# NVlabs/EdgeRunner

Hardware: AMD Instinct MI355X
Metric: mesh tokens/sec (whole node), ArAE greedy test_num_face=1000 (higher is better)
Workload: dtype f32; 1 GPU; BASELINE configs[1]: ArAE random-init (seeded synthetic checkpoint), batch 1 per GPU, greedy, test_num_face=1000, 4000 new tokens (EOS suppressed until T), 4096-point synthetic cloud; step = the whole LMM.generate(): encode_cond + 2050-token prefill + 4000-token decode + detokenise to a mesh (native meto engine, clean=True); layers=24, hidden=1536, heads=16, batch_per_gpu=1, precision=fp32, parallelism=dp1 (independent samples, full replica per GPU)

## Files before the change

### edgerunner_amd/csrc/er_api.hip

```cpp
#include "../../include/edgerunner_hip.h"

#include <hip/hip_runtime.h>

#include <algorithm>
#include <cstdarg>
#include <cstdio>
#include <cstdlib>
#include <cstring>
#include <map>
#include <memory>
#include <string>
#include <utility>
#include <vector>

#include "er_common.h"
#include "k_attn_decode.h"
#include "k_outproj_merge.h"
#include "k_flash_attn_f16s.h"
#include "k_gemm.h"
#include "k_gemm_stream.h"
#include "k_gemv.h"
#include "k_gemv_mfma.h"
#include "k_head.h"
#include "k_rowops.h"
#include "k_score.h"
#include "k_flash_attn.h"
#include "k_flash_attn_f32.h"
#include "k_fps.h"
#include "k_fidelity.h"
#include "meto_decode.h"
#include "meto_encode.h"
#include "er_queue_host.h"
#include "er_decode_plan.h"
#include "er_decode_proj.h"

using namespace er;

static thread_local char g_err[1024] = "";

static int fail(int code, const char* fmt, ...) {
    va_list ap;
    va_start(ap, fmt);
    vsnprintf(g_err, sizeof(g_err), fmt, ap);
    va_end(ap);
    return code;
}

#define HIPCHK(expr)                                                                          \
    do {                                                                                      \
        hipError_t e_ = (expr);                                                               \
        if (e_ != hipSuccess)                                                                 \
            return fail(ER_ERR_HIP, "%s:%d %s -> %s", __FILE__, __LINE__, #expr, hipGetErrorString(e_)); \
    } while (0)
#define ERCHK(expr)                 \
    do {                            \
        int r_ = (expr);            \
        if (r_ < 0) return r_;      \
    } while (0)

struct LayerW {
    _Float16 *wqkv_h = nullptr, *wo_h = nullptr, *w1_h = nullptr, *w2_h = nullptr;
    void *wqkv_t = nullptr, *wo_t = nullptr, *w1_t = nullptr, *w2_t = nullptr;
    float *wqkv = nullptr, *bqkv = nullptr;
    float *wo = nullptr, *bo = nullptr, *ln1w = nullptr, *ln1b = nullptr;
    float *w1 = nullptr, *b1 = nullptr, *w2 = nullptr, *b2 = nullptr, *ln2w = nullptr, *ln2b = nullptr;
};

#include "er_devbuf.h"
#include "er_weights.h"

struct PointEnc {
    int PH = 0, heads = 0, Lq = 0, LD = 0, freq = 0;
    int mode = ER_PE_EMBED;
    float eps = 1e-5f;
    float *query = nullptr, *basis = nullptr, *mlp_w = nullptr, *mlp_b = nullptr, *ln_w = nullptr, *ln_b = nullptr;
    float *ca_ln1_w = nullptr, *ca_ln1_b = nullptr, *ca_ln2_w = nullptr, *ca_ln2_b = nullptr;
    float *ca_q_w = nullptr, *ca_q_b = nullptr, *ca_k_w = nullptr, *ca_k_b = nullptr, *ca_v_w = nullptr, *ca_v_b = nullptr,
          *ca_o_w = nullptr, *ca_o_b = nullptr;
    float *ff0_w = nullptr, *ff0_b = nullptr, *ff2_w = nullptr, *ff2_b = nullptr, *lin_w = nullptr, *lin_b = nullptr;
    int kpad = 0;
    DevBuf<float> a0, x, k, v, qln, q, sc, att, l, ln, u, g, lat;
    DevBuf<float> q0, fdist;
    DevBuf<int32_t> fidx;
};

static size_t gen_state_ints(size_t b) { return 7 * b + 8; }
static GenState gen_state_carve(int* sb, size_t b) {
    GenState s{};
    s.tok = sb; s.pos = sb + b; s.counter = sb + 2 * b; s.ngen = sb + 3 * b; s.unfinished = sb + 4 * b;
    s.eos_step = sb + 5 * b; s.base_pos = sb + 6 * b; s.n_unfinished = sb + 7 * b; s.error = sb + 7 * b + 1;
    return s;
}

constexpr int SK_SLICES_OUTPROJ = 4, SK_SLICES_FC2 = 16;
static_assert(1536 / (4 * GM_KW) == SK_SLICES_OUTPROJ && 6144 / (4 * GM_KW) == SK_SLICES_FC2 && 6144 / (GM_WAVES * GM_KW) == SK_SLICES_OUTPROJ, "k_gemv_mfma.h");

struct KvMem {
    DecodePlan plan;
    DevBuf<char> kc, vc;
    DevBuf<float> ypre, hbuf, ypre1, h1buf, qbuf, abuf, fbuf, logits;
    DevBuf<float> part, part_ml;
    DevBuf<float> skpart;
    DevBuf<char> xt_h, xt_att, xt_f;
    DevBuf<int> state_block;
    GenState st{};
    DevBuf<DecodeParamsDev> d_params;
    DevBuf<int> d_ids_tmp;
    DevBuf<unsigned int> d_row_stream;
    DevBuf<int> d_row_budget;
    DevBuf<long long> d_out_ids;
    hipGraphExec_t step_exec = nullptr;
    KvMem() = default;
    KvMem(const KvMem&) = delete;
    KvMem& operator=(const KvMem&) = delete;
    ~KvMem() { if (step_exec) hipGraphExecDestroy(step_exec); }
};

struct er_ctx {
    er_config cfg{};
    int device = 0;
    int D = 0;
    hipStream_t own_stream = nullptr;
    std::vector<LayerW> layers;
    float *embd = nullptr, *posemb = nullptr, *lm_head = nullptr, *embed_num_face = nullptr;
    _Float16* lm_head_h = nullptr;
    bool fast = false;
    float *proj_w = nullptr, *proj_b = nullptr, *normc_w = nullptr, *normc_b = nullptr;
    PointEnc pe;
    WeightTable w;
    std::unique_ptr<KvMem> kv = std::make_unique<KvMem>();
    int kv_esz = 4;
    int* h_pinned = nullptr;
    int base_pos = 0;
    bool have_hidden = false;
    DecodeKnobs knobs;
    bool tiled_valid = false;
    int prof_len = 0;
    hipEvent_t ev0 = nullptr, ev1 = nullptr;
    float last_decode_ms = 0.f;
    DevBuf<_Float16> p_hi, p_lo;
    DevBuf<float> p_h, p_q, p_a, p_y, p_f, p_qkv, p_ap, p_aml, e_tmp;
    DevBuf<int> e_ids;
    DevBuf<float> s_lg;
    erq::QueueHost q;
    DevBuf<int> q_stage, q_look;
    int* q_pinned = nullptr;
};

constexpr int ER_MAX_BATCH = 1023;

template <typename Ctx>
static hipStream_t pick(Ctx* c, void* s) { return s ? (hipStream_t)s : c->own_stream; }

static int env_int(const char* name, int dflt) { const char* v = getenv(name); return (v && v[0]) ? atoi(v) : dflt; }
static bool env_is(const char* name, char ch) { const char* v = getenv(name); return v && v[0] == ch; }

static DecodeKnobs read_knobs(bool fast) {
    DecodeKnobs k;
    k.use_graph = !env_is("ER_NO_GRAPH", '1');
    k.nw_qkv = env_int("ER_NW_QKV", fast ? 9 : 6);
    if (k.nw_qkv != 4 && k.nw_qkv != 9) k.nw_qkv = 6;
    k.nw_fc1 = env_int("ER_NW_FC1", fast ? 12 : 4) == 12 ? 12 : 4;
    k.prefill_attn_f16s = env_int("ER_PREFILL_ATTN_F16S", -1);
    if (k.prefill_attn_f16s != 0 && k.prefill_attn_f16s != 1) k.prefill_attn_f16s = -1;
    k.attn_v_batched = env_int("ER_ATTN_V_BATCHED", 0);
    if (k.attn_v_batched != 1 && k.attn_v_batched != 3) k.attn_v_batched = 0;
    k.decode_v = env_int("ER_DECODE_V", 3) == 2 ? 2 : 3;
    const char* rw = getenv("ER_RW_FC2");
    k.rw_fc2 = rw ? atoi(rw) : 6;
    if (fast && k.rw_fc2 != 2 && k.rw_fc2 != 4 && k.rw_fc2 != 6) fprintf(stderr, "[edgerunner_hip] ER_RW_FC2=%s is not 2 / 4 / 6: using 2 rows per fc2 workgroup\n", rw);
    return k;
}

static ReserveKnobs read_reserve_knobs() { return {env_is("ER_FORCE_BATCHED", '1'), env_is("ER_BATCHED_VALU", '1'), !env_is("ER_XT", '0')}; }

extern "C" int er_abi_version(void) { return ER_ABI_VERSION; }
extern "C" const char* er_last_error(void) { return g_err; }

static const char* kKindNames[ER_NUM_KERNEL_KINDS] = {"qkv_gemv", "attn_decode", "attn_combine", "out_proj_gemv",
                                                      "fc1_gemv", "fc2_gemv", "lm_head_gemv", "sample_head"};
extern "C" const char* er_kernel_kind_name(int k) { return (k >= 0 && k < ER_NUM_KERNEL_KINDS) ? kKindNames[k] : "?"; }

static int pe_attach(WeightTable& t, PointEnc& p, int mode, const char* who, const char* before) {
    if (mode != ER_PE_EMBED && mode != ER_PE_DOWNSAMPLE)
        return fail(ER_ERR_INVALID, "%s: %d is neither ER_PE_EMBED nor ER_PE_DOWNSAMPLE", who, mode);
    for (auto& kv : t.keys)
        if (kv.second.loaded && kv.first.rfind(before, 0) == 0)
            return fail(ER_ERR_INVALID, "%s: call it before any '%s*' tensor is loaded", who, before);
    const size_t PH = p.PH, kin = 2 * p.freq + 3;
    p.mode = mode;
    p.kpad = (int)((kin + 15) / 16 * 16);
    const std::string pe = "point_encoder.";
    if (mode == ER_PE_EMBED) t.add(pe + "query_embed", &p.query, (size_t)p.Lq * PH);
    else t.keys.erase(pe + "query_embed");
    t.add(pe + "point_embed.basis", &p.basis, (size_t)3 * p.freq);
    t.lin(pe + "point_embed.mlp", &p.mlp_w, &p.mlp_b, PH, kin).pad(kin, p.kpad);
    t.lin(pe + "ln", &p.ln_w, &p.ln_b, PH, 1);
    t.lin(pe + "cross_att.ln1", &p.ca_ln1_w, &p.ca_ln1_b, PH, 1);
    t.lin(pe + "cross_att.ln2", &p.ca_ln2_w, &p.ca_ln2_b, PH, 1);
    t.lin(pe + "cross_att.att.q_proj", &p.ca_q_w, &p.ca_q_b, PH, PH);
    t.lin(pe + "cross_att.att.k_proj", &p.ca_k_w, &p.ca_k_b, PH, PH);
    t.lin(pe + "cross_att.att.v_proj", &p.ca_v_w, &p.ca_v_b, PH, PH);
    t.lin(pe + "cross_att.att.out_proj", &p.ca_o_w, &p.ca_o_b, PH, PH);
    t.lin(pe + "cross_att.mlp.net.0", &p.ff0_w, &p.ff0_b, 8 * PH, PH);
    t.lin(pe + "cross_att.mlp.net.2", &p.ff2_w, &p.ff2_b, PH, 4 * PH);
    t.lin(pe + "linear", &p.lin_w, &p.lin_b, p.LD, PH);
    return 0;
}

static void register_weights(er_ctx* c) {
    WeightTable& t = c->w;
    const er_config& g = c->cfg;
    const size_t H = g.hidden_dim, I = g.intermediate_dim, V = g.vocab_size;
    t.fp16 = c->fast;
    if (g.cond_mode == ER_COND_POINT) pe_attach(t, c->pe, ER_PE_EMBED, "er_create", "");
    if (g.cond_mode != ER_COND_NONE) {
        t.lin("proj_cond", &c->proj_w, &c->proj_b, H, g.point_latent_dim);
        t.lin("norm_cond", &c->normc_w, &c->normc_b, H, 1);
    }
    if (g.num_face_buckets > 0) t.add("embed_num_face.weight", &c->embed_num_face, (size_t)g.num_face_buckets * H);
    t.add("mesh_decoder.model.embd.weight", &c->embd, V * H);
    t.add("mesh_decoder.model.embed_positions.weight", &c->posemb, (size_t)g.max_positions * H);
    for (int i = 0; i < g.num_layers; ++i) {
        LayerW& L = c->layers[i];
        const std::string p = "mesh_decoder.model.layers." + std::to_string(i) + ".";
        const char* qkv[3] = {"q_proj", "k_proj", "v_proj"};
        for (size_t j = 0; j < 3; ++j) {
            const std::string q = p + "self_attn." + qkv[j];
            t.add(q + ".weight", &L.wqkv, H * H).slice(3 * H * H, j * H * H).half(&L.wqkv_h);
            t.add(q + ".bias", &L.bqkv, H).slice(3 * H, j * H);
        }
        t.lin(p + "self_attn.out_proj", &L.wo, &L.bo, H, H).half(&L.wo_h);
        t.lin(p + "self_attn_layer_norm", &L.ln1w, &L.ln1b, H, 1);
        t.lin(p + "fc1", &L.w1, &L.b1, I, H).half(&L.w1_h);
        t.lin(p + "fc2", &L.w2, &L.b2, H, I).half(&L.w2_h);
        t.lin(p + "final_layer_norm", &L.ln2w, &L.ln2b, H, 1);
    }
    t.add("mesh_decoder.lm_head.weight", &c->lm_head, V * H).half(&c->lm_head_h);
}

extern "C" int er_create(const er_config* cfg, int device, er_ctx** out) {
    if (!cfg || !out) return fail(ER_ERR_INVALID, "er_create: null argument");
    if (cfg->hidden_dim != 1536 || cfg->intermediate_dim != 6144)
        return fail(ER_ERR_UNSUPPORTED, "this build streams hidden_dim=1536 / intermediate_dim=6144 (ArAE, DiT presets); got %d/%d",
                    cfg->hidden_dim, cfg->intermediate_dim);
    if (cfg->num_heads <= 0 || cfg->hidden_dim % cfg->num_heads) return fail(ER_ERR_INVALID, "hidden_dim %% num_heads != 0");
    const int D = cfg->hidden_dim / cfg->num_heads;
    if (D != 96 && D != 64) return fail(ER_ERR_UNSUPPORTED, "head_dim %d not built (96, 64)", D);
    const bool exact = cfg->weight_dtype == ER_F32 && cfg->kv_dtype == ER_F32;
    const bool fast = cfg->weight_dtype == ER_F16 && cfg->kv_dtype == ER_F16;
    if (!exact && !fast)
        return fail(ER_ERR_UNSUPPORTED, "built modes: fp32 weights + fp32 KV (exact) or fp16 weights + fp16 KV (fast)");
    if (cfg->vocab_size > ER_HEAD_MAX_VOCAB) return fail(ER_ERR_UNSUPPORTED, "vocab_size > %d", ER_HEAD_MAX_VOCAB);
    if (cfg->cond_mode == ER_COND_POINT && (cfg->point_hidden_dim != 1024 || cfg->point_hidden_dim % cfg->point_num_heads))
        return fail(ER_ERR_UNSUPPORTED, "point encoder width %d not built (1024)", cfg->point_hidden_dim);
    HIPCHK(hipSetDevice(device));
    er_ctx* c = new er_ctx();
    c->cfg = *cfg;
    c->device = device;
    c->D = D;
    c->fast = fast;
    c->kv_esz = fast ? 2 : 4;
    c->layers.resize(cfg->num_layers);
    c->pe.PH = cfg->point_hidden_dim; c->pe.heads = cfg->point_num_heads; c->pe.Lq = cfg->point_latent_size;
    c->pe.LD = cfg->point_latent_dim; c->pe.freq = cfg->point_freq_dim; c->pe.eps = cfg->ln_eps;
    c->knobs = read_knobs(fast);
    HIPCHK(hipStreamCreateWithFlags(&c->own_stream, hipStreamDefault));
    HIPCHK(hipEventCreate(&c->ev0));
    HIPCHK(hipEventCreate(&c->ev1));
    HIPCHK(hipHostMalloc((void**)&c->h_pinned, 4096, hipHostMallocDefault));
    register_weights(c);
    *out = c;
    return ER_OK;
}

extern "C" int er_destroy(er_ctx* c) {
    if (!c) return ER_OK;
    hipSetDevice(c->device);
    hipDeviceSynchronize();
    if (c->ev0) hipEventDestroy(c->ev0);
    if (c->ev1) hipEventDestroy(c->ev1);
    if (c->h_pinned) hipHostFree(c->h_pinned);
    if (c->q_pinned) hipHostFree(c->q_pinned);
    if (c->own_stream) hipStreamDestroy(c->own_stream);
    delete c;
    return ER_OK;
}

extern "C" int er_load_tensor(er_ctx* c, const char* key, const void* data, int dtype, int ndim, const int64_t* shape,
                              int on_device) {
    if (!c || !key) return fail(ER_ERR_INVALID, "er_load_tensor: bad argument");
    HIPCHK(hipSetDevice(c->device));
    const int rc = weights_load(c->w, c->own_stream, "er_load_tensor", key, data, dtype, ndim, shape, on_device);
    if (rc != 1) c->tiled_valid = false;
    return rc;
}

extern "C" int er_finalize_weights(er_ctx* c) {
    if (!c) return fail(ER_ERR_INVALID, "null ctx");
    return weights_finalize(c->w);
}

template <typename WT>
static int make_tiled(er_ctx* c, const void* src, void** dst, int N, int K) {
    if (!*dst) {
        char* blk = nullptr;
        ERCHK(c->w.alloc(&blk, tiled_weight_bytes<WT>(N, K)));
        *dst = blk;
    }
    hipLaunchKernelGGL((tile_weights_kernel<WT>), dim3(2048), dim3(ER_WG), 0, c->own_stream, reinterpret_cast<const WT*>(src),
                       reinterpret_cast<f32x4*>(*dst), N, K);
    HIPCHK(hipGetLastError());
    return 0;
}
static int make_tiled_weights(er_ctx* c) {
    if (c->tiled_valid || weights_missing(c->w)) return 0;
    const int H = c->cfg.hidden_dim, I = c->cfg.intermediate_dim;
    for (LayerW& L : c->layers) {
        if (c->fast) {
            ERCHK(make_tiled<_Float16>(c, L.wqkv_h, &L.wqkv_t, 3 * H, H));
            ERCHK(make_tiled<_Float16>(c, L.wo_h, &L.wo_t, H, H));
            ERCHK(make_tiled<_Float16>(c, L.w1_h, &L.w1_t, I, H));
            ERCHK(make_tiled<_Float16>(c, L.w2_h, &L.w2_t, H, I));
        } else {
            ERCHK(make_tiled<float>(c, L.wqkv, &L.wqkv_t, 3 * H, H));
            ERCHK(make_tiled<float>(c, L.wo, &L.wo_t, H, H));
            ERCHK(make_tiled<float>(c, L.w1, &L.w1_t, I, H));
            ERCHK(make_tiled<float>(c, L.w2, &L.w2_t, H, I));
        }
    }
    HIPCHK(hipStreamSynchronize(c->own_stream));
    c->tiled_valid = true;
    return 0;
}

static AttnChunking attn_chunking(int heads, bool fast) {
    return {attn3_num_chunks(heads), attn3_num_chunks(heads) * ATTN3_CAP, attn_chunk(ATTN_STEPS_DEFAULT, fast)};
}

extern "C" int er_plan_decode(int batch, int heads, int head_dim, int hidden, int l_cap, er_decode_plan* out) {
    if (!out || batch <= 0 || heads <= 0 || head_dim <= 0 || l_cap <= 0) return fail(ER_ERR_INVALID, "er_plan_decode: bad argument");
    const DecodeKnobs k = read_knobs(false);
    plan_decode(k.decode_v, k.attn_v_batched, read_reserve_knobs().force_batched, batch, heads, head_dim, hidden, (l_cap + 31) / 32 * 32, attn_chunking(heads, false), out);
    return ER_OK;
}

extern "C" int er_ctx_plan(er_ctx* c, er_decode_plan* out) {
    if (!c || !out) return fail(ER_ERR_INVALID, "er_ctx_plan: null argument");
    if (c->kv->plan.B <= 0) return fail(ER_ERR_INVALID, "er_ctx_plan: no cache reserved (call er_kv_reserve)");
    *out = c->kv->plan.sel;
    return ER_OK;
}

extern "C" int er_plan_gemm_tile(int m, int n, int batch) {
    if (m <= 0 || n <= 0 || batch <= 0) return fail(ER_ERR_INVALID, "er_plan_gemm_tile: bad argument");
    return gemm_pick_tile(m, n, batch);
}

static int kv_alloc(er_ctx* c, KvMem& m, int batch, int Lcap);

extern "C" int er_kv_reserve(er_ctx* c, int batch, int max_len) {
    if (!c || batch <= 0 || max_len <= 0) return fail(ER_ERR_INVALID, "er_kv_reserve: bad argument");
    if (batch > ER_MAX_BATCH) return fail(ER_ERR_UNSUPPORTED, "er_kv_reserve: batch %d > %d (host staging buffers are sized for %d rows)", batch, ER_MAX_BATCH, ER_MAX_BATCH);
    HIPCHK(hipSetDevice(c->device));
    const er_config& g = c->cfg;
    if (max_len > g.max_positions)
        return fail(ER_ERR_CAPACITY, "max_len %d exceeds the position table (%d)", max_len, g.max_positions);
    const int Lcap = (max_len + 31) / 32 * 32;
    if (c->kv->plan.B == batch && c->kv->plan.Lcap == Lcap) return ER_OK;
    HIPCHK(hipDeviceSynchronize());
    c->kv = std::make_unique<KvMem>();
    c->have_hidden = false;
    c->q.end();
    auto m = std::make_unique<KvMem>();
    ERCHK(kv_alloc(c, *m, batch, Lcap));
    c->kv = std::move(m);
    return ER_OK;
}

static int kv_alloc(er_ctx* c, KvMem& m, int batch, int Lcap) {
    const er_config& g = c->cfg;
    const int H = g.num_heads, D = c->D, hid = g.hidden_dim;
    m.plan = make_decode_plan(c->knobs, read_reserve_knobs(), c->fast, batch, Lcap, g.num_layers, H, D, hid, attn_chunking(H, c->fast));
    const DecodePlan& p = m.plan;
    const size_t kv_bytes = (size_t)p.kv_lstride * g.num_layers * c->kv_esz;
    ERCHK(m.kc.ensure(kv_bytes));
    ERCHK(m.vc.ensure(kv_bytes));
    const size_t b = (size_t)batch;
    for (DevBuf<float>* w : {&m.ypre, &m.hbuf, &m.ypre1, &m.h1buf, &m.qbuf, &m.abuf}) ERCHK(w->ensure(b * hid));
    ERCHK(m.fbuf.ensure(b * g.intermediate_dim));
    ERCHK(m.logits.ensure(b * g.vocab_size));
    ERCHK(m.part.ensure(b * H * (size_t)std::max(p.S_splits * (D + 2), p.nch3 * D)));
    ERCHK(m.part_ml.ensure(b * H * (size_t)p.nch3 * 2));
    ERCHK(m.state_block.ensure(gen_state_ints(b)));
    m.st = gen_state_carve(m.state_block.p, b);
    ERCHK(m.d_params.ensure(1));
    ERCHK(m.d_ids_tmp.ensure(b));
    ERCHK(m.d_row_stream.ensure(b));
    {
        std::vector<unsigned int> ident(b);
        for (size_t i = 0; i < b; ++i) ident[i] = (unsigned int)i;
        HIPCHK(hipMemcpy(m.d_row_stream.p, ident.data(), b * sizeof(unsigned int), hipMemcpyHostToDevice));
    }
    m.st.row_stream = m.d_row_stream.p;
    ERCHK(m.d_row_budget.ensure(b));
    {
        const std::vector<int> open(b, 0x7fffffff);
        HIPCHK(hipMemcpy(m.d_row_budget.p, open.data(), b * sizeof(int), hipMemcpyHostToDevice));
    }
    m.st.row_budget = m.d_row_budget.p;
    ERCHK(m.d_out_ids.ensure(b * (size_t)Lcap));
    if (p.mfma) ERCHK(make_tiled_weights(c));
    const size_t groups = (b + NBM - 1) / NBM;
    ERCHK(m.skpart.ensure(p.xt ? groups * SK_SLICES_FC2 * NBM * (size_t)hid : (size_t)SK_SLICES_OUTPROJ * NBM * (size_t)std::max(hid, g.vocab_size)));
    if (p.xt) {
        const size_t b_h = groups * (size_t)hid * 128, b_f = groups * (size_t)g.intermediate_dim * 128;
        ERCHK(m.xt_h.ensure(b_h));
        ERCHK(m.xt_att.ensure(b_h));
        ERCHK(m.xt_f.ensure(b_f));
        HIPCHK(hipMemset(m.xt_h.p, 0, b_h));
        HIPCHK(hipMemset(m.xt_att.p, 0, b_h));
        HIPCHK(hipMemset(m.xt_f.p, 0, b_f));
    }
    return ER_OK;
}

static AttnDecArgs attn_args(er_ctx* c, int layer) {
    const DecodePlan& p = c->kv->plan;
    AttnDecArgs a{};
    a.q = c->kv->qbuf.p;
    a.kcache = c->kv->kc.p + (long long)layer * p.kv_lstride * c->kv_esz;
    a.vcache = c->kv->vc.p + (long long)layer * p.kv_lstride * c->kv_esz;
    a.chunk = attn_chunk(ATTN_STEPS_DEFAULT, c->fast);
    a.pos = c->kv->st.pos;
    a.fixed_len = c->prof_len;
    a.len_dev = nullptr;
    a.part = c->kv->part.p;
    a.part_ml = c->kv->part_ml.p;
    a.out = c->kv->abuf.p;
    a.H = c->cfg.num_heads;
    a.l_cap = p.Lcap;
    a.S = p.S_splits;
    a.hidden = c->cfg.hidden_dim;
    a.kv_bstride = p.kv_bstride;
    a.sqrt_d = sqrtf((float)c->D);
    a.out_xt = p.outproj_partials ? c->kv->xt_att.p : nullptr;
    return a;
}

static hipError_t launch_attn_partial(const AttnDecArgs& a, int D, int steps, bool kv_half, int B, hipStream_t st, int ver = 2) {
    return D == 96 ? launch_attn_partial_d<96>(a, steps, kv_half, B, st, ver) : launch_attn_partial_d<64>(a, steps, kv_half, B, st, ver);
}
static hipError_t launch_attn_combine(const AttnDecArgs& a, int D, int B, hipStream_t st) {
    return D == 96 ? launch_attn_combine_d<96>(a, B, st) : launch_attn_combine_d<64>(a, B, st);
}

template <typename WT>
static hipError_t launch_kind_t(er_ctx* c, int kind, int layer, hipStream_t st, long long* out_ids, int out_ld) {
    constexpr bool HALF = sizeof(WT) == 2;
    const er_config& g = c->cfg;
    const DecodePlan& p = c->kv->plan;
    const KvMem& kv = *c->kv;
    const int H = g.hidden_dim, I = g.intermediate_dim, B = p.B;
    const SkPart sk{kv.skpart.p, kv.skpart.n};
    const auto form_of = [&](Proj proj, int l) { return proj_form(p, c->knobs, HALF, proj, l); };
    GemvArgs a{};
    a.eps = g.ln_eps;
    a.hidden = H; a.head_dim = c->D; a.l_cap = p.Lcap; a.kv_bstride = p.kv_bstride; a.kv_half = HALF ? 1 : 0;
    ProjIo io;
    switch (kind) {
        case 0: {
            const LayerW& L = c->layers[layer];
            a.W = HALF ? (const void*)L.wqkv_h : (const void*)L.wqkv; a.bias = L.bqkv; a.N = 3 * H;
            a.hout = kv.hbuf.p; a.pos = kv.st.pos;
            a.q = kv.qbuf.p;
            a.kcache = kv.kc.p + (long long)layer * p.kv_lstride * c->kv_esz;
            a.vcache = kv.vc.p + (long long)layer * p.kv_lstride * c->kv_esz;
            if (layer == 0) {
                io.pro = PRO_EMBED; a.embd = c->embd; a.posemb = c->posemb; a.tok = kv.st.tok;
            } else {
                io.pro = PRO_LN; a.xin = kv.ypre.p; a.ln_w = c->layers[layer - 1].ln2w; a.ln_b = c->layers[layer - 1].ln2b;
                if (form_of(PROJ_FC2, layer - 1).defer) io.rd = {sk.p, c->layers[layer - 1].b2, kv.h1buf.p, SK_SLICES_FC2};
            }
            io.w_tiled = L.wqkv_t; io.x_image = kv.xt_h.p; io.pro_image = p.xt ? kv.xt_h.p : nullptr;
            return run_proj<WT>(PROJ_QKV, form_of(PROJ_QKV, layer), io, a, B, H, sk, st);
        }
        case 1:
            if (p.v3) return launch_attn_partial3_d<96>(attn_args(c, layer), HALF, p.nch3, B, st);
            if (p.stream_attn) return launch_attn_stream_d<96>(attn_args(c, layer), HALF, B, st);
            return launch_attn_partial(attn_args(c, layer), c->D, ATTN_STEPS_DEFAULT, HALF, B, st, p.batched ? 1 : 2);
        case 2:
            if (!p.sel.merge_launch) return hipSuccess;
            return launch_attn_combine(attn_args(c, layer), c->D, B, st);
        case 3: {
            const LayerW& L = c->layers[layer];
            if (p.v3) {
                OutMergeArgs m{};
                m.W = HALF ? (const void*)L.wo_h : (const void*)L.wo; m.bias = L.bo; m.resid = c->kv->hbuf.p; m.out = c->kv->ypre1.p;
                m.part_o = c->kv->part.p; m.part_ml = c->kv->part_ml.p; m.N = H;
                return launch_outproj_merge<WT, 96>(m, p.nch3, st);
            }
            a.W = HALF ? (const void*)L.wo_h : (const void*)L.wo; a.bias = L.bo; a.N = H; a.xin = kv.abuf.p; a.out = kv.ypre1.p; a.resid = kv.hbuf.p;
            io.w_tiled = L.wo_t; io.x_image = kv.xt_att.p;
            return run_proj<WT>(PROJ_OUT, form_of(PROJ_OUT, layer), io, a, B, H, sk, st);
        }
        case 4: {
            const LayerW& L = c->layers[layer];
            a.W = HALF ? (const void*)L.w1_h : (const void*)L.w1; a.bias = L.b1; a.N = I; a.xin = kv.ypre1.p; a.ln_w = L.ln1w; a.ln_b = L.ln1b;
            a.hout = kv.h1buf.p; a.out = kv.fbuf.p;
            io.pro = PRO_LN;
            if (form_of(PROJ_OUT, layer).defer) io.rd = {sk.p, L.bo, kv.hbuf.p, SK_SLICES_OUTPROJ};
            io.w_tiled = L.w1_t; io.x_image = kv.xt_h.p; io.pro_image = p.xt ? kv.xt_h.p : nullptr; io.out_image = kv.xt_f.p;
            return run_proj<WT>(PROJ_FC1, form_of(PROJ_FC1, layer), io, a, B, H, sk, st);
        }
        case 5: {
            const LayerW& L = c->layers[layer];
            a.W = HALF ? (const void*)L.w2_h : (const void*)L.w2; a.bias = L.b2; a.N = H; a.xin = kv.fbuf.p; a.out = kv.ypre.p; a.resid = kv.h1buf.p;
            io.w_tiled = L.w2_t; io.x_image = kv.xt_f.p;
            return run_proj<WT>(PROJ_FC2, form_of(PROJ_FC2, layer), io, a, B, I, sk, st);
        }
        case 6: {
            a.W = HALF ? (const void*)c->lm_head_h : (const void*)c->lm_head; a.bias = nullptr; a.N = g.vocab_size; a.xin = kv.ypre.p;
            a.ln_w = c->layers[p.layers - 1].ln2w; a.ln_b = c->layers[p.layers - 1].ln2b; a.hout = p.batched ? kv.hbuf.p : nullptr; a.out = kv.logits.p;
            io.pro = PRO_LN;
            return run_proj<WT>(PROJ_HEAD, form_of(PROJ_HEAD, layer), io, a, B, H, sk, st);
        }
        case 7:
            hipLaunchKernelGGL(sample_head_kernel, dim3(B), dim3(ER_WG), sample_head_lds(g.vocab_size), st, c->kv->logits.p,
                               c->kv->d_params.p, c->kv->st, out_ids, out_ld);
            return hipGetLastError();
    }
    return hipErrorInvalidValue;
}

static hipError_t launch_kind(er_ctx* c, int kind, int layer, hipStream_t st, long long* out_ids, int out_ld) {
    return c->fast ? launch_kind_t<_Float16>(c, kind, layer, st, out_ids, out_ld)
                   : launch_kind_t<float>(c, kind, layer, st, out_ids, out_ld);
}

static hipError_t enqueue_layers(er_ctx* c, hipStream_t st) {
    for (int l = 0; l < c->cfg.num_layers; ++l)
        for (int k = 0; k <= 5; ++k) {
            hipError_t e = launch_kind(c, k, l, st, nullptr, 0);
            if (e != hipSuccess) return e;
        }
    return hipSuccess;
}

static hipError_t enqueue_step(er_ctx* c, hipStream_t st, long long* out_ids, int out_ld) {
    hipError_t e = launch_kind(c, 6, 0, st, nullptr, 0);
    if (e != hipSuccess) return e;
    e = launch_kind(c, 7, 0, st, out_ids, out_ld);
    if (e != hipSuccess) return e;
    return enqueue_layers(c, st);
}

static hipError_t linear(const float* A, int lda, const float* W, const float* bias, float* C, int ldc, int M, int N, int K,
                         bool relu, const float* resid, int ldr, hipStream_t st) {
    GemmArgs g = gemm_args_default();
    g.A = A; g.B = W; g.C = C; g.bias = bias; g.resid = resid;
    g.M = M; g.N = N; g.K = K; g.lda = lda; g.ldb = K; g.ldc = ldc; g.ldr = ldr;
    g.relu = relu ? 1 : 0;
    return launch_gemm(g, 1, st);
}

static hipError_t linear_h(const float* A, int lda, const _Float16* W, const float* bias, float* C, int ldc, int M, int N, int K,
                           bool relu, const float* resid, int ldr, hipStream_t st) {
    GemmArgs g = gemm_args_default();
    g.A = A; g.B = reinterpret_cast<const float*>(W); g.C = C; g.bias = bias; g.resid = resid;
    g.M = M; g.N = N; g.K = K; g.lda = lda; g.ldb = K; g.ldc = ldc; g.ldr = ldr;
    g.relu = relu ? 1 : 0;
    return launch_gemm_f16s(g, st);
}

static int linear_hs(er_ctx* c, const float* A, int lda, const _Float16* W, const float* bias, float* C, int ldc, int M, int N, int K,
                     bool relu, const float* resid, int ldr, hipStream_t st);

#define HIPRET(expr)                                                                          \
    do {                                                                                      \
        hipError_t e_ = (expr);                                                               \
        if (e_ != hipSuccess)                                                                 \
            return fail(ER_ERR_HIP, "%s:%d %s -> %s", __FILE__, __LINE__, #expr, hipGetErrorString(e_)); \
    } while (0)

static int linear_hs(er_ctx* c, const float* A, int lda, const _Float16* W, const float* bias, float* C, int ldc, int M, int N, int K,
                     bool relu, const float* resid, int ldr, hipStream_t st) {
    constexpr int HS_MAX_ROWS = 4608;
    if (K % XBK != 0 || M > HS_MAX_ROWS) { HIPRET(linear_h(A, lda, W, bias, C, ldc, M, N, K, relu, resid, ldr, st)); return 0; }
    ERCHK(c->p_hi.ensure((size_t)M * K + F16_TAIL));
    ERCHK(c->p_lo.ensure((size_t)M * K + F16_TAIL));
    _Float16 *hi = c->p_hi.p, *lo = c->p_lo.p;
    hipLaunchKernelGGL(split_rows_f16_kernel, split_rows_grid(M, K), dim3(ER_WG), 0, st, A, hi, lo, (long long)M, K, lda);
    HIPRET(hipGetLastError());
    GemmArgs g = gemm_args_default();
    g.A = reinterpret_cast<const float*>(hi); g.a_lo = lo; g.B = reinterpret_cast<const float*>(W); g.C = C; g.bias = bias; g.resid = resid;
    g.M = M; g.N = N; g.K = K; g.lda = K; g.ldb = K; g.ldc = ldc; g.ldr = ldr;
    g.relu = relu ? 1 : 0;
    HIPRET(launch_gemm_hh_split(g, st));
    return 0;
}

static int attention_full(const float* Q, int ldq, const float* Kp, int ldk, long long k_hstride, const float* Vp, int ldv,
                          long long v_hstride, float* out, int ldo, float* sc, int H, int D, int N, int M, bool causal,
                          hipStream_t st) {
    const int ldS = (M + 15) / 16 * 16;
    GemmArgs g = gemm_args_default();
    g.A = Q; g.lda = ldq; g.sA2 = D;
    g.B = Kp; g.ldb = ldk; g.sB2 = k_hstride;
    g.C = sc; g.ldc = ldS; g.sC2 = (long long)N * ldS;
    g.Z2 = H; g.M = N; g.N = M; g.K = D; g.div = sqrtf((float)D);
    g.causal = causal ? 1 : 0; g.causal_off = M - N;
    HIPRET(launch_gemm(g, H, st));
    HIPRET(launch_softmax_rows(sc, N, M, (long long)ldS, ldS, (long long)N * ldS, H, causal ? 1 : 0, M - N, st));
    GemmArgs p = gemm_args_default();
    p.A = sc; p.lda = ldS; p.sA2 = (long long)N * ldS;
    p.B = Vp; p.ldb = ldv; p.sB2 = v_hstride; p.b_is_kn = 1; p.kb_valid = M;
    p.C = out; p.ldc = ldo; p.sC2 = D;
    p.Z2 = H; p.M = N; p.N = D; p.K = ldS;
    p.causal = causal ? 1 : 0; p.causal_off = M - N;
    HIPRET(launch_gemm(p, H, st));
    return 0;
}

constexpr int ENC_CHUNK = 32;
static int point_latent_chunk(PointEnc& p, const float* pts, int nb, int N, hipStream_t st) {
    const int PH = p.PH, Lq = p.Lq, LD = p.LD;
    const int PHh = p.heads > 0 ? p.heads : 1, PD = PH / PHh;
    const bool ds = p.mode == ER_PE_DOWNSAMPLE;
    if (N <= 0) return fail(ER_ERR_INVALID, "n_points must be > 0");
    if (ds && N < Lq)
        return fail(ER_ERR_INVALID, "point_encoder_mode downsample samples point_latent_size = %d points per cloud; the clouds have %d", Lq, N);
    const size_t R = (size_t)nb * N, RQ = (size_t)nb * Lq;
    const size_t QR = ds ? RQ : (size_t)Lq;
    ERCHK(p.a0.ensure(R * p.kpad));
    ERCHK(p.x.ensure(R * PH));
    ERCHK(p.k.ensure(R * PH));
    ERCHK(p.v.ensure(R * PH));
    ERCHK(p.qln.ensure(QR * PH));
    ERCHK(p.q.ensure(QR * PH));
    ERCHK(p.att.ensure(RQ * PH));
    ERCHK(p.l.ensure(RQ * PH));
    ERCHK(p.ln.ensure(RQ * PH));
    ERCHK(p.u.ensure(RQ * 8 * PH));
    ERCHK(p.g.ensure(RQ * 4 * PH));
    ERCHK(p.lat.ensure(RQ * LD));
    int32_t* fidx = nullptr;
    if (ds) {
        ERCHK(p.q0.ensure(RQ * PH));
        ERCHK(p.fidx.ensure(RQ));
        if (N > FPS_REG_MAX) ERCHK(p.fdist.ensure(R));
        fidx = p.fidx.p;
        HIPRET(launch_fps(pts, nb, N, Lq, fidx, p.fdist.p, st));
    }
    hipLaunchKernelGGL(point_embed_kernel, dim3(ew_grid((long long)R * p.kpad)), dim3(ER_WG), 0, st, pts,
                       p.basis, p.a0.p, (long long)R, p.freq, p.kpad);
    HIPRET(hipGetLastError());
    HIPRET(linear(p.a0.p, p.kpad, p.mlp_w, p.mlp_b, p.x.p, PH, (int)R, PH, p.kpad, false, nullptr, 0, st));
    if (ds) {
        hipLaunchKernelGGL(fps_gather_rows_kernel, dim3((unsigned)RQ), dim3(ER_WG), 0, st, p.x.p, fidx, N, Lq, PH, p.q0.p);
        HIPRET(hipGetLastError());
    }
    HIPRET(launch_layernorm(p.x.p, p.ln_w, p.ln_b, p.x.p, (int)R, PH, PH, PH, p.eps, st));
    const float* qsrc = ds ? p.q0.p : p.query;
    HIPRET(launch_layernorm(qsrc, p.ca_ln1_w, p.ca_ln1_b, p.qln.p, (int)QR, PH, PH, PH, p.eps, st));
    HIPRET(linear(p.qln.p, PH, p.ca_q_w, p.ca_q_b, p.q.p, PH, (int)QR, PH, PH, false, nullptr, 0, st));
    HIPRET(linear(p.x.p, PH, p.ca_k_w, p.ca_k_b, p.k.p, PH, (int)R, PH, PH, false, nullptr, 0, st));
    HIPRET(linear(p.x.p, PH, p.ca_v_w, p.ca_v_b, p.v.p, PH, (int)R, PH, PH, false, nullptr, 0, st));
    if (PD == 64 || PD == 96) {
        Flash32Args f{};
        f.Q = p.q.p; f.ldq = PH; f.qs_b = ds ? (long long)Lq * PH : 0; f.qs_h = PD;
        f.K = p.k.p; f.ldk = PH; f.ks_b = (long long)N * PH; f.ks_h = PD;
        f.V = p.v.p; f.ldv = PH; f.vs_b = (long long)N * PH; f.vs_h = PD;
        f.O = p.att.p; f.ldo = PH; f.os_b = (long long)Lq * PH; f.os_h = PD;
        f.N = Lq; f.M = N; f.sqrt_d = sqrtf((float)PD); f.causal_off = 0;
        HIPRET(launch_flash_attn_f32(f, PD, false, PHh, nb, st));
    } else {
        const int ldS = (N + 15) / 16 * 16;
        ERCHK(p.sc.ensure((size_t)PHh * Lq * ldS));
        for (int b = 0; b < nb; ++b)
            ERCHK(attention_full(p.q.p + (ds ? (size_t)b * Lq * PH : 0), PH, p.k.p + (size_t)b * N * PH, PH, PD,
                                 p.v.p + (size_t)b * N * PH, PH, PD, p.att.p + (size_t)b * Lq * PH, PH, p.sc.p, PHh, PD, Lq, N, false, st));
    }
    {
        GemmArgs ga = gemm_args_default();
        ga.A = p.att.p; ga.B = p.ca_o_w; ga.C = p.l.p; ga.bias = p.ca_o_b; ga.resid = qsrc; ga.resid_mod = ds ? 0 : Lq;
        ga.M = (int)RQ; ga.N = PH; ga.K = PH; ga.lda = PH; ga.ldb = PH; ga.ldc = PH; ga.ldr = PH;
        HIPRET(launch_gemm(ga, 1, st));
    }
    HIPRET(launch_layernorm(p.l.p, p.ca_ln2_w, p.ca_ln2_b, p.ln.p, (int)RQ, PH, PH, PH, p.eps, st));
    HIPRET(linear(p.ln.p, PH, p.ff0_w, p.ff0_b, p.u.p, 8 * PH, (int)RQ, 8 * PH, PH, false, nullptr, 0, st));
    hipLaunchKernelGGL(geglu_kernel, dim3(ew_grid((long long)RQ * 4 * PH)), dim3(ER_WG), 0, st, p.u.p, p.g.p,
                       (long long)RQ, 4 * PH);
    HIPRET(hipGetLastError());
    HIPRET(linear(p.g.p, 4 * PH, p.ff2_w, p.ff2_b, p.l.p, PH, (int)RQ, PH, 4 * PH, false, p.l.p, PH, st));
    HIPRET(linear(p.l.p, PH, p.lin_w, p.lin_b, p.lat.p, LD, (int)RQ, LD, PH, false, nullptr, 0, st));
    return 0;
}

static int pe_latent(PointEnc& p, const float* pts, int B, int N, float* latent_out, hipStream_t st, const char* who) {
    const size_t per = (size_t)p.Lq * p.LD;
    if ((long long)B * (long long)per > 0x7fffffffLL) return fail(ER_ERR_CAPACITY, "%s: batch %d too large", who, B);
    for (int b0 = 0; b0 < B; b0 += ENC_CHUNK) {
        const int nb = std::min(ENC_CHUNK, B - b0);
        ERCHK(point_latent_chunk(p, pts + (size_t)b0 * N * 3, nb, N, st));
        HIPCHK(hipMemcpyAsync(latent_out + (size_t)b0 * per, p.lat.p, (size_t)nb * per * 4, hipMemcpyDeviceToDevice, st));
    }
    return 0;
}

extern "C" int er_encode_cond(er_ctx* c, const float* conds, int B, int n_points, const int32_t* face_bucket,
                              float* cond_out, void* stream) {
    if (!c || !cond_out || B <= 0) return fail(ER_ERR_INVALID, "er_encode_cond: bad argument");
    ERCHK(er_finalize_weights(c));
    HIPCHK(hipSetDevice(c->device));
    hipStream_t st = pick(c, stream);
    const er_config& g = c->cfg;
    const int H = g.hidden_dim, C = g.num_cond_tokens, Lq = g.point_latent_size, LD = g.point_latent_dim;
    const int n_lat = (g.cond_mode == ER_COND_NONE) ? 0 : Lq;
    const int n_face = g.num_face_buckets > 0 ? 1 : 0;
    if (n_lat + n_face != C) return fail(ER_ERR_INVALID, "num_cond_tokens %d != latent tokens %d + face token %d", C, n_lat, n_face);
    if (g.cond_mode != ER_COND_NONE && !conds) return fail(ER_ERR_INVALID, "er_encode_cond: conds is null");
    if (LD % 16) return fail(ER_ERR_UNSUPPORTED, "point_latent_dim must be a multiple of 16");
    for (int b0 = 0; b0 < B; b0 += ENC_CHUNK) {
        const int nb = std::min(ENC_CHUNK, B - b0);
        const float* lat = nullptr;
        if (g.cond_mode == ER_COND_POINT) {
            ERCHK(point_latent_chunk(c->pe, conds + (size_t)b0 * n_points * 3, nb, n_points, st));
            lat = c->pe.lat.p;
        } else if (g.cond_mode == ER_COND_POINT_LATENT) {
            lat = conds + (size_t)b0 * Lq * LD;
        }
        if (lat) {
            ERCHK(c->e_tmp.ensure((size_t)nb * Lq * H));
            HIPRET(linear(lat, LD, c->proj_w, c->proj_b, c->e_tmp.p, H, nb * Lq, H, LD, false, nullptr, 0, st));
        }
        for (int b = 0; b < nb; ++b) {
            float* out_b = cond_out + (size_t)(b0 + b) * C * H;
            if (lat) HIPRET(launch_layernorm(c->e_tmp.p + (size_t)b * Lq * H, c->normc_w, c->normc_b, out_b, Lq, H, H, H, g.ln_eps, st));
            if (n_face) {
                const int bucket = face_bucket ? face_bucket[b0 + b] : 0;
                if (bucket < 0 || bucket >= g.num_face_buckets) return fail(ER_ERR_INVALID, "face bucket %d out of range", bucket);
                HIPCHK(hipMemcpyAsync(out_b + (size_t)n_lat * H, c->embed_num_face + (size_t)bucket * H, (size_t)H * 4,
                                      hipMemcpyDeviceToDevice, st));
            }
        }
    }
    return ER_OK;
}

extern "C" int er_embed_tokens(er_ctx* c, const int32_t* ids, int B, int R, float* out, void* stream) {
    if (!c || !ids || !out || B <= 0 || R <= 0) return fail(ER_ERR_INVALID, "er_embed_tokens: bad argument");
    ERCHK(er_finalize_weights(c));
    HIPCHK(hipSetDevice(c->device));
    hipStream_t st = pick(c, stream);
    const int H = c->cfg.hidden_dim;
    const int n = B * R;
    for (int i = 0; i < n; ++i)
        if (ids[i] < 0 || ids[i] >= c->cfg.vocab_size) return fail(ER_ERR_INVALID, "token id %d out of range", ids[i]);
    ERCHK(c->e_ids.ensure((size_t)n));
    int* d_ids = c->e_ids.p;
    HIPCHK(hipMemcpyAsync(d_ids, ids, (size_t)n * sizeof(int), hipMemcpyHostToDevice, st));
    hipLaunchKernelGGL(gather_rows_kernel, dim3(n), dim3(ER_WG), 0, st, c->embd, d_ids, out, n, H, (long long)H);
    HIPRET(hipGetLastError());
    HIPCHK(hipStreamSynchronize(st));
    return ER_OK;
}

static int prefill_tail_rows(const er_ctx* c, int M) {
    const char* v = getenv("ER_PREFILL_TAIL");
    if ((v && atoi(v) == 0) || c->fast) return 0;
    if (c->cfg.hidden_dim != 1536 || c->cfg.intermediate_dim != 6144) return 0;
    const int tail = M % 64;
    if (tail < 1 || tail > 8 || M < 1024) return 0;
    const long long nt = c->cfg.hidden_dim / 64;
    const long long r_all = ((long long)(M / 64 + 1) * nt + 255) / 256, r_main = ((long long)(M / 64) * nt + 255) / 256;
    return r_all > r_main ? tail : 0;
}
template <int KS, int RW, int EPI>
static hipError_t linear_tail(const float* A, const float* W, const float* bias, float* C, const float* resid, int rows, int N, int K,
                              hipStream_t st) {
    GemvArgs t{};
    t.W = W; t.bias = bias; t.N = N; t.xin = A; t.out = C; t.resid = resid;
    return gemv_groups<float, KS, RW, PRO_NONE, EPI>(t, rows, K, st);
}

static int forward_check(er_ctx* c, const char* who, const float* embeds, int B, int S) {
    if (!c || !embeds || B <= 0 || S <= 0) return fail(ER_ERR_INVALID, "%s: bad argument", who);
    if (c->q.active) return fail(ER_ERR_INVALID, "%s: a queue is open on this context (er_queue_end first)", who);
    ERCHK(er_finalize_weights(c));
    if (c->kv->plan.B != B) return fail(ER_ERR_INVALID, "%s: batch %d but KV cache reserved for %d (call er_kv_reserve)", who, B, c->kv->plan.B);
    if (S >= c->kv->plan.Lcap) return fail(ER_ERR_CAPACITY, "prefix length %d does not fit the reserved KV cache (%d)", S, c->kv->plan.Lcap);
    const long long width = std::max({(long long)c->cfg.intermediate_dim, 3LL * c->cfg.hidden_dim, (long long)c->cfg.vocab_size});
    if ((long long)B * S * width > 0x7fffffffLL)
        return fail(ER_ERR_CAPACITY, "%s: %d x %d positions x %lld columns overflows the 32-bit row indexing of the prefill (split the batch)",
                    who, B, S, width);
    return 0;
}

static int prefill_run(er_ctx* c, const float* embeds, int B, int S, hipStream_t st, int row0 = 0, bool in_queue = false) {
    HIPCHK(hipSetDevice(c->device));
    const DecodePlan& p = c->kv->plan;
    if (p.mfma) ERCHK(make_tiled_weights(c));
    const er_config& g = c->cfg;
    const int H = g.hidden_dim, I = g.intermediate_dim, NH = g.num_heads, D = c->D;
    const int M = B * S;
    ERCHK(c->p_h.ensure((size_t)M * H));
    ERCHK(c->p_q.ensure((size_t)M * H));
    ERCHK(c->p_a.ensure((size_t)M * H));
    ERCHK(c->p_y.ensure((size_t)M * H));
    ERCHK(c->p_f.ensure((size_t)M * I));
    float *h = c->p_h.p, *q = c->p_q.p, *a = c->p_a.p, *y = c->p_y.p, *f = c->p_f.p;
    const int tail = prefill_tail_rows(c, M), Mm = M - tail;
    bool attn_ksplit = false;
    if (!c->fast && flash32_ksplit(S, NH, B, D, true)) {
        ERCHK(c->p_ap.ensure(flash32_part_o_floats(B, NH, S, D)));
        ERCHK(c->p_aml.ensure(flash32_part_ml_floats(B, NH, S)));
        attn_ksplit = true;
    }

    hipLaunchKernelGGL(add_pos_kernel, dim3(ew_grid((long long)M * H / 4)), dim3(ER_WG), 0, st, embeds, c->posemb, h, B, S, H, 0);
    HIPRET(hipGetLastError());
    for (int l = 0; l < g.num_layers; ++l) {
        const LayerW& L = c->layers[l];
        char* kc = c->kv->kc.p + ((long long)l * p.kv_lstride + (long long)row0 * p.kv_bstride) * c->kv_esz;
        char* vc = c->kv->vc.p + ((long long)l * p.kv_lstride + (long long)row0 * p.kv_bstride) * c->kv_esz;
        if (!c->fast) {
            GemmArgs qa = gemm_args_default();
            qa.A = h; qa.lda = H; qa.B = L.wqkv; qa.ldb = H; qa.bias = L.bqkv; qa.C = q; qa.ldc = H;
            qa.M = M; qa.N = 3 * H; qa.K = H; qa.epi = GEPI_QKV;
            qa.q = q; qa.kcache = (float*)kc; qa.vcache = (float*)vc; qa.S = S; qa.hidden = H; qa.head_dim = D; qa.l_cap = p.Lcap;
            qa.kv_bstride = p.kv_bstride;
            HIPRET(launch_gemm(qa, 1, st));
            {
                Flash32Args f{};
                f.Q = q; f.ldq = H; f.qs_b = (long long)S * H; f.qs_h = D;
                f.K = (float*)kc; f.ldk = D; f.ks_b = p.kv_bstride; f.ks_h = (long long)p.Lcap * D;
                f.V = (float*)vc; f.ldv = D; f.vs_b = p.kv_bstride; f.vs_h = (long long)p.Lcap * D;
                f.O = a; f.ldo = H; f.os_b = (long long)S * H; f.os_h = D;
                f.N = S; f.M = S; f.sqrt_d = sqrtf((float)D); f.causal_off = 0;
                if (attn_ksplit) { f.part_o = c->p_ap.p; f.part_ml = c->p_aml.p; }
                HIPRET(launch_flash_attn_f32(f, D, true, NH, B, st));
            }
        } else {
            ERCHK(c->p_qkv.ensure((size_t)M * 3 * H));
            float* qkv = c->p_qkv.p;
            ERCHK(linear_hs(c, h, H, L.wqkv_h, L.bqkv, qkv, 3 * H, M, 3 * H, H, false, nullptr, 0, st));
            hipLaunchKernelGGL(kv_scatter_half_kernel, kv_scatter_grid(M, H), dim3(ER_WG), 0, st, qkv,
                               (_Float16*)kc, (_Float16*)vc, M, S, H, D, p.Lcap, p.kv_bstride);
            HIPRET(hipGetLastError());
            {
                Flash32Args f{};
                f.Q = qkv; f.ldq = 3 * H; f.qs_b = (long long)S * 3 * H; f.qs_h = D;
                f.K = qkv + H; f.ldk = 3 * H; f.ks_b = f.qs_b; f.ks_h = D;
                f.V = qkv + 2 * H; f.ldv = 3 * H; f.vs_b = f.qs_b; f.vs_h = D;
                f.O = a; f.ldo = H; f.os_b = (long long)S * H; f.os_h = D;
                f.N = S; f.M = S; f.sqrt_d = sqrtf((float)D); f.causal_off = 0;
                const bool f16s = D == 96 && c->knobs.prefill_attn_f16s != 0;
                if (f16s) HIPRET(launch_flash_attn_f16s(f, D, true, NH, B, st));
                else HIPRET(launch_flash_attn_f32(f, D, true, NH, B, st));
            }
        }
        const bool hs = c->fast;
        if (hs) ERCHK(linear_hs(c, a, H, L.wo_h, L.bo, y, H, M, H, H, false, h, H, st));
        else {
            HIPRET(linear(a, H, L.wo, L.bo, y, H, Mm, H, H, false, h, H, st));
            if (tail) HIPRET((linear_tail<1, 1, EPI_RESID>(a + (size_t)Mm * H, L.wo, L.bo, y + (size_t)Mm * H, h + (size_t)Mm * H, tail, H, H, st)));
        }
        HIPRET(launch_layernorm(y, L.ln1w, L.ln1b, h, M, H, H, H, g.ln_eps, st));
        if (hs) {
            ERCHK(linear_hs(c, h, H, L.w1_h, L.b1, f, I, M, I, H, true, nullptr, 0, st));
            ERCHK(linear_hs(c, f, I, L.w2_h, L.b2, y, H, M, H, I, false, h, H, st));
        } else {
            HIPRET(linear(h, H, L.w1, L.b1, f, I, Mm, I, H, true, nullptr, 0, st));
            if (tail) HIPRET((linear_tail<1, 2, EPI_RELU>(h + (size_t)Mm * H, L.w1, L.b1, f + (size_t)Mm * I, nullptr, tail, I, H, st)));
            HIPRET(linear(f, I, L.w2, L.b2, y, H, Mm, H, I, false, h, H, st));
            if (tail) HIPRET((linear_tail<4, 2, EPI_RESID>(f + (size_t)Mm * I, L.w2, L.b2, y + (size_t)Mm * H, h + (size_t)Mm * H, tail, H, I, st)));
        }
        if (l + 1 < g.num_layers) HIPRET(launch_layernorm(y, L.ln2w, L.ln2b, h, M, H, H, H, g.ln_eps, st));
    }
    for (int b = 0; b < B; ++b)
        HIPCHK(hipMemcpyAsync(c->kv->ypre.p + (size_t)(row0 + b) * H, y + ((size_t)b * S + S - 1) * H, (size_t)H * 4, hipMemcpyDeviceToDevice, st));
    if (in_queue) return ER_OK;
    hipLaunchKernelGGL(init_state_kernel, dim3((B + 63) / 64), dim3(64), 0, st, c->kv->st, B, S);
    HIPRET(hipGetLastError());
    c->base_pos = S;
    c->have_hidden = true;
    return ER_OK;
}

extern "C" int er_prefill(er_ctx* c, const float* embeds, int B, int S, void* stream) {
    ERCHK(forward_check(c, "er_prefill", embeds, B, S));
    return prefill_run(c, embeds, B, S, pick(c, stream));
}

extern "C" int er_score(er_ctx* c, const float* embeds, const int32_t* labels, int B, int S, float* nll_out, int32_t* pred_out,
                        float* logits_out, float* loss_out, void* stream) {
    ERCHK(forward_check(c, "er_score", embeds, B, S));
    if (!labels || !nll_out || !loss_out) return fail(ER_ERR_INVALID, "er_score: labels, nll_out and loss_out are required");
    hipStream_t st = pick(c, stream);
    ERCHK(prefill_run(c, embeds, B, S, st));
    const er_config& g = c->cfg;
    const int H = g.hidden_dim, V = g.vocab_size, M = B * S;
    const LayerW& last = c->layers[g.num_layers - 1];
    HIPRET(launch_layernorm(c->p_y.p, last.ln2w, last.ln2b, c->p_h.p, M, H, H, H, g.ln_eps, st));
    float* lg = logits_out;
    if (!lg) {
        ERCHK(c->s_lg.ensure((size_t)M * V));
        lg = c->s_lg.p;
    }
    if (c->fast) ERCHK(linear_hs(c, c->p_h.p, H, c->lm_head_h, nullptr, lg, V, M, V, H, false, nullptr, 0, st));
    else HIPRET(linear(c->p_h.p, H, c->lm_head, nullptr, lg, V, M, V, H, false, nullptr, 0, st));
    HIPRET(launch_score_rows(lg, labels, M, S, V, nll_out, pred_out, st));
    HIPRET(launch_score_reduce(nll_out, labels, M, S, loss_out, st));
    return ER_OK;
}

extern "C" int er_point_latent(er_ctx* c, const float* conds, int B, int n_points, float* latent_out, float* kl_out, void* stream) {
    if (!c || !conds || !latent_out || B <= 0) return fail(ER_ERR_INVALID, "er_point_latent: bad argument");
    if (c->cfg.cond_mode != ER_COND_POINT) return fail(ER_ERR_UNSUPPORTED, "er_point_latent: the context has no point encoder (cond_mode %d)", c->cfg.cond_mode);
    ERCHK(er_finalize_weights(c));
    HIPCHK(hipSetDevice(c->device));
    hipStream_t st = pick(c, stream);
    ERCHK(pe_latent(c->pe, conds, B, n_points, latent_out, st, "er_point_latent"));
    const size_t n = (size_t)B * c->pe.Lq * c->pe.LD;
    if (kl_out) HIPRET(launch_score_reduce(latent_out, nullptr, (int)n, 0, kl_out, st));
    return ER_OK;
}

extern "C" int er_set_point_encoder_mode(er_ctx* c, int mode) {
    if (!c) return fail(ER_ERR_INVALID, "null ctx");
    if (c->cfg.cond_mode != ER_COND_POINT)
        return fail(ER_ERR_UNSUPPORTED, "er_set_point_encoder_mode: the context has no point encoder (cond_mode %d)", c->cfg.cond_mode);
    return pe_attach(c->w, c->pe, mode, "er_set_point_encoder_mode", "");
}

extern "C" int er_logits(er_ctx* c, float* out, void* stream) {
    if (!c || !out) return fail(ER_ERR_INVALID, "er_logits: bad argument");
    if (!c->have_hidden) return fail(ER_ERR_INVALID, "er_logits: no forward pass has run (call er_prefill)");
    HIPCHK(hipSetDevice(c->device));
    hipStream_t st = pick(c, stream);
    HIPRET(launch_kind(c, 6, 0, st, nullptr, 0));
    HIPCHK(hipMemcpyAsync(out, c->kv->logits.p, (size_t)c->kv->plan.B * c->cfg.vocab_size * 4, hipMemcpyDeviceToDevice, st));
    return ER_OK;
}

static int check_room(er_ctx* c, int extra) {
    HIPCHK(hipMemcpy(c->h_pinned, c->kv->st.ngen, sizeof(int), hipMemcpyDeviceToHost));
    const int used = c->base_pos + c->h_pinned[0];
    if (used + extra > c->kv->plan.Lcap) return fail(ER_ERR_CAPACITY, "KV cache full: %d + %d > %d", used, extra, c->kv->plan.Lcap);
    if (used + extra > c->cfg.max_positions) return fail(ER_ERR_CAPACITY, "position table exhausted (%d)", c->cfg.max_positions);
    return 0;
}

extern "C" int er_feed(er_ctx* c, const int32_t* ids, void* stream) {
    if (!c || !ids) return fail(ER_ERR_INVALID, "er_feed: bad argument");
// ... 13 lines not shown
    HIPRET(enqueue_layers(c, st));
    HIPCHK(hipStreamSynchronize(st));
    return ER_OK;
}

__global__ void fill_i64_kernel(long long* p, long long n, long long v) {
    for (long long i = (long long)blockIdx.x * blockDim.x + threadIdx.x; i < n; i += (long long)gridDim.x * blockDim.x) p[i] = v;
}
__global__ void reset_gen_kernel(GenState st, int B) {
    const int b = blockIdx.x * blockDim.x + threadIdx.x;
    if (b == 0) { *st.n_unfinished = B; *st.error = 0; }
    if (b >= B) return;
    st.counter[b] = 0; st.unfinished[b] = 1; st.eos_step[b] = -1;
}

static int ensure_step_graph(er_ctx* c) {
    if (!c->knobs.use_graph || c->kv->step_exec) return 0;
    const int Lcap = c->kv->plan.Lcap;
    hipGraph_t graph = nullptr;
    HIPCHK(hipStreamBeginCapture(c->own_stream, hipStreamCaptureModeRelaxed));
    hipError_t e = enqueue_step(c, c->own_stream, c->kv->d_out_ids.p, Lcap);
    hipError_t e2 = hipStreamEndCapture(c->own_stream, &graph);
    if (e != hipSuccess || e2 != hipSuccess) {
        if (graph) hipGraphDestroy(graph);
        return fail(ER_ERR_HIP, "graph capture failed: %s / %s", hipGetErrorString(e), hipGetErrorString(e2));
    }
    HIPCHK(hipGraphInstantiate(&c->kv->step_exec, graph, nullptr, nullptr, 0));
    hipGraphDestroy(graph);
    return 0;
}

extern "C" int er_decode(er_ctx* c, const er_decode_params* p, int64_t* out_ids, int32_t* n_steps, void* stream) {
    if (!c || !p || !out_ids || !n_steps) return fail(ER_ERR_INVALID, "er_decode: bad argument");
    if (!c->have_hidden) return fail(ER_ERR_INVALID, "er_decode: call er_prefill first");
    if (p->max_new_tokens <= 0) return fail(ER_ERR_INVALID, "max_new_tokens must be > 0");
    if (p->mode != ER_GREEDY && p->mode != ER_SAMPLE) return fail(ER_ERR_INVALID, "bad mode");
    if (p->grammar < 0 || p->grammar > 2) return fail(ER_ERR_INVALID, "bad grammar");
    if (p->mode == ER_SAMPLE && p->top_k <= 0) return fail(ER_ERR_INVALID, "top_k must be > 0 in sample mode");
    HIPCHK(hipSetDevice(c->device));
    hipStream_t st = pick(c, stream);
    const int B = c->kv->plan.B, Lcap = c->kv->plan.Lcap, T = p->max_new_tokens;
    HIPCHK(hipStreamSynchronize(st));
    ERCHK(check_room(c, T));
    if (c->h_pinned[0] != 0) return fail(ER_ERR_INVALID, "er_decode must directly follow er_prefill (%d tokens already fed)", c->h_pinned[0]);

    DecodeParamsDev dp{};
    dp.mode = p->mode; dp.top_k = p->top_k; dp.grammar = p->grammar; dp.max_new = T; dp.min_new = p->min_new_tokens;
    dp.eos = c->cfg.eos_token_id; dp.pad = c->cfg.pad_token_id; dp.vocab = c->cfg.vocab_size;
    dp.seed_lo = (unsigned int)(p->seed & 0xffffffffu); dp.seed_hi = (unsigned int)(p->seed >> 32);
    HIPCHK(hipMemcpy(c->kv->d_params.p, &dp, sizeof(dp), hipMemcpyHostToDevice));
    hipLaunchKernelGGL(reset_gen_kernel, dim3((B + 63) / 64), dim3(64), 0, st, c->kv->st, B);
    HIPRET(hipGetLastError());
    hipLaunchKernelGGL(fill_i64_kernel, dim3(ew_grid((long long)B * Lcap)), dim3(ER_WG), 0, st, c->kv->d_out_ids.p,
                       (long long)B * Lcap, (long long)dp.pad);
    HIPRET(hipGetLastError());

    ERCHK(ensure_step_graph(c));

    const int check_every = 32;
    int steps_run = 0;
    HIPCHK(hipEventRecord(c->ev0, st));
    for (int t = 0; t < T; ++t) {
        if (c->knobs.use_graph) HIPCHK(hipGraphLaunch(c->kv->step_exec, st));
        else HIPRET(enqueue_step(c, st, c->kv->d_out_ids.p, Lcap));
        steps_run = t + 1;
        if (steps_run >= p->min_new_tokens && steps_run < T && (steps_run % check_every) == 0) {
            HIPCHK(hipMemcpyAsync(c->h_pinned, c->kv->st.n_unfinished, sizeof(int), hipMemcpyDeviceToHost, st));
            HIPCHK(hipStreamSynchronize(st));
            if (c->h_pinned[0] <= 0) break;
        }
    }
    HIPCHK(hipEventRecord(c->ev1, st));
    HIPCHK(hipMemcpy2DAsync(out_ids, (size_t)T * sizeof(long long), c->kv->d_out_ids.p, (size_t)Lcap * sizeof(long long),
                            (size_t)T * sizeof(long long), B, hipMemcpyDeviceToDevice, st));
    HIPCHK(hipMemcpyAsync(c->h_pinned, c->kv->st.eos_step, B * sizeof(int), hipMemcpyDeviceToHost, st));
    HIPCHK(hipMemcpyAsync(c->h_pinned + B, c->kv->st.error, sizeof(int), hipMemcpyDeviceToHost, st));
    HIPCHK(hipStreamSynchronize(st));
    HIPCHK(hipEventElapsedTime(&c->last_decode_ms, c->ev0, c->ev1));
    if (c->h_pinned[B] != 0)
        return fail(ER_ERR_INVALID, "er_decode: a row had no finite candidate score (non-finite logits); HF would raise in multinomial/argmax");
    int last = -1;
    bool finished = true;
    for (int b = 0; b < B; ++b) {
        if (c->h_pinned[b] < 0) finished = false;
        else if (c->h_pinned[b] > last) last = c->h_pinned[b];
    }
    *n_steps = finished ? last + 1 : T;
    if (!finished && steps_run < T) return fail(ER_ERR_INVALID, "internal: stopped early with unfinished rows");
    return ER_OK;
}

extern "C" int er_set_row_streams(er_ctx* c, const uint32_t* ids, int n) {
    if (!c) return fail(ER_ERR_INVALID, "er_set_row_streams: null context");
    const int B = c->kv->plan.B;
    if (B <= 0) return fail(ER_ERR_INVALID, "er_set_row_streams: no cache reserved (call er_kv_reserve)");
    if (ids && n != B) return fail(ER_ERR_INVALID, "er_set_row_streams: %d ids for a batch of %d rows", n, B);
    HIPCHK(hipSetDevice(c->device));
    std::vector<unsigned int> h((size_t)B);
    for (int i = 0; i < B; ++i) h[i] = ids ? ids[i] : (unsigned int)i;
    HIPCHK(hipDeviceSynchronize());
    HIPCHK(hipMemcpy(c->kv->d_row_stream.p, h.data(), h.size() * sizeof(unsigned int), hipMemcpyHostToDevice));
    return ER_OK;
}

__global__ void queue_park_kernel(GenState st, int* budget, int row0, int n) {
    const int i = blockIdx.x * blockDim.x + threadIdx.x;
    if (i >= n) return;
    const int b = row0 + i;
    st.tok[b] = 0; st.pos[b] = 0; st.counter[b] = 0; st.ngen[b] = 0;
    st.unfinished[b] = 0; st.eos_step[b] = -1; st.base_pos[b] = 0;
    budget[b] = 0;
}
__global__ void queue_admit_kernel(GenState st, unsigned int* row_stream, int* budget, const int* stage, int row0, int n, int S) {
    const int i = blockIdx.x * blockDim.x + threadIdx.x;
    if (i >= n) return;
    const int b = row0 + i;
    st.tok[b] = 0; st.pos[b] = S; st.counter[b] = 0; st.ngen[b] = 0;
    st.unfinished[b] = 1; st.eos_step[b] = -1; st.base_pos[b] = S;
    row_stream[b] = (unsigned int)stage[i];
    budget[b] = stage[n + i];
}
__global__ void queue_look_kernel(GenState st, int B, int* look) {
    const int b = blockIdx.x * blockDim.x + threadIdx.x;
    if (b == 0) look[3 * B] = *st.error;
    if (b >= B) return;
    look[b] = st.ngen[b]; look[B + b] = st.unfinished[b]; look[2 * B + b] = st.eos_step[b];
}
__global__ void fill_i32_kernel(int* p, int n, int v) {
    const int i = blockIdx.x * blockDim.x + threadIdx.x;
    if (i < n) p[i] = v;
}

static int queue_open(er_ctx* c, const char* who) {
    if (!c) return fail(ER_ERR_INVALID, "%s: null context", who);
    if (!c->q.active) return fail(ER_ERR_INVALID, "%s: no queue is open (call er_queue_begin)", who);
    HIPCHK(hipSetDevice(c->device));
    return 0;
}

extern "C" int er_queue_begin(er_ctx* c, const er_decode_params* p, int check_every, void* stream) {
    if (!c || !p) return fail(ER_ERR_INVALID, "er_queue_begin: bad argument");
    if (c->q.active) return fail(ER_ERR_INVALID, "er_queue_begin: a queue is already open (er_queue_end first)");
    const int B = c->kv->plan.B, Lcap = c->kv->plan.Lcap;
    if (B <= 0) return fail(ER_ERR_INVALID, "er_queue_begin: no cache reserved (call er_kv_reserve)");
    if (p->max_new_tokens <= 0) return fail(ER_ERR_INVALID, "max_new_tokens must be > 0");
    if (p->mode != ER_GREEDY && p->mode != ER_SAMPLE) return fail(ER_ERR_INVALID, "bad mode");
    if (p->grammar < 0 || p->grammar > 2) return fail(ER_ERR_INVALID, "bad grammar");
    if (p->mode == ER_SAMPLE && p->top_k <= 0) return fail(ER_ERR_INVALID, "top_k must be > 0 in sample mode");
    if (check_every < 0) return fail(ER_ERR_INVALID, "er_queue_begin: check_every %d", check_every);
    ERCHK(er_finalize_weights(c));
    HIPCHK(hipSetDevice(c->device));
    hipStream_t st = pick(c, stream);
    if (c->kv->plan.mfma) ERCHK(make_tiled_weights(c));
    ERCHK(c->q_look.ensure((size_t)3 * B + 1));
    if (c->q_pinned) { hipHostFree(c->q_pinned); c->q_pinned = nullptr; }
    HIPCHK(hipHostMalloc((void**)&c->q_pinned, ((size_t)3 * B + 1) * sizeof(int), hipHostMallocDefault));
    HIPCHK(hipStreamSynchronize(st));

    DecodeParamsDev dp{};
    dp.mode = p->mode; dp.top_k = p->top_k; dp.grammar = p->grammar; dp.max_new = p->max_new_tokens; dp.min_new = p->min_new_tokens;
    dp.eos = c->cfg.eos_token_id; dp.pad = c->cfg.pad_token_id; dp.vocab = c->cfg.vocab_size;
    dp.seed_lo = (unsigned int)(p->seed & 0xffffffffu); dp.seed_hi = (unsigned int)(p->seed >> 32);
    HIPCHK(hipMemcpy(c->kv->d_params.p, &dp, sizeof(dp), hipMemcpyHostToDevice));
    hipLaunchKernelGGL(queue_park_kernel, dim3((B + 63) / 64), dim3(64), 0, st, c->kv->st, c->kv->d_row_budget.p, 0, B);
    HIPRET(hipGetLastError());
    HIPCHK(hipMemsetAsync(c->kv->st.n_unfinished, 0, 2 * sizeof(int), st));
    HIPCHK(hipMemsetAsync(c->kv->ypre.p, 0, (size_t)B * c->cfg.hidden_dim * sizeof(float), st));
    ERCHK(ensure_step_graph(c));
    HIPCHK(hipStreamSynchronize(st));
    c->have_hidden = false;
    c->q.begin(B, Lcap, c->cfg.max_positions, p->max_new_tokens, check_every);
    return ER_OK;
}

extern "C" int er_queue_admit(er_ctx* c, int row0, int n_rows, const float* embeds, int S, const uint32_t* stream_ids,
                              const int32_t* max_new, void* stream) {
    ERCHK(queue_open(c, "er_queue_admit"));
    if (!embeds) return fail(ER_ERR_INVALID, "er_queue_admit: embeds is null");
    const long long width = std::max({(long long)c->cfg.intermediate_dim, 3LL * c->cfg.hidden_dim, (long long)c->cfg.vocab_size});
    const int rc = c->q.check_admit(row0, n_rows, S, max_new, width);
    if (rc < 0) return fail(rc, "%s", c->q.why);
    hipStream_t st = pick(c, stream);
    std::vector<int> stage((size_t)2 * n_rows);
    for (int i = 0; i < n_rows; ++i) {
        stage[(size_t)i] = (int)(stream_ids ? stream_ids[i] : (uint32_t)(row0 + i));
        stage[(size_t)n_rows + i] = c->q.budget_of(max_new, i);
    }
    ERCHK(c->q_stage.ensure(stage.size()));
    HIPCHK(hipMemcpyAsync(c->q_stage.p, stage.data(), stage.size() * sizeof(int), hipMemcpyHostToDevice, st));
    HIPCHK(hipEventRecord(c->ev0, st));
    ERCHK(prefill_run(c, embeds, n_rows, S, st, row0, true));
    hipLaunchKernelGGL(queue_admit_kernel, dim3((n_rows + 63) / 64), dim3(64), 0, st, c->kv->st, c->kv->d_row_stream.p,
                       c->kv->d_row_budget.p, c->q_stage.p, row0, n_rows, S);
    HIPRET(hipGetLastError());
    HIPCHK(hipEventRecord(c->ev1, st));
    HIPCHK(hipStreamSynchronize(st));
    float ms = 0.f;
    HIPCHK(hipEventElapsedTime(&ms, c->ev0, c->ev1));
    c->q.stats.prefill_ms += ms;
    c->q.admit(row0, n_rows, S, max_new);
    return ER_OK;
}

extern "C" int er_queue_run(er_ctx* c, int32_t* done_rows, int32_t* n_done, void* stream) {
    ERCHK(queue_open(c, "er_queue_run"));
    if (!done_rows || !n_done) return fail(ER_ERR_INVALID, "er_queue_run: bad argument");
    *n_done = c->q.list_done(done_rows);
    if (*n_done > 0 || c->q.occupied() == 0) return ER_OK;
    hipStream_t st = pick(c, stream);
    const int B = c->q.slots, Lcap = c->kv->plan.Lcap;
    HIPCHK(hipEventRecord(c->ev0, st));
    while (*n_done == 0) {
        const int burst = c->q.next_burst();
        if (burst <= 0) return fail(ER_ERR_INVALID, "internal: er_queue_run has occupied rows but none is running");
        for (int t = 0; t < burst; ++t) {
            if (c->knobs.use_graph) HIPCHK(hipGraphLaunch(c->kv->step_exec, st));
            else HIPRET(enqueue_step(c, st, c->kv->d_out_ids.p, Lcap));
        }
        c->q.advance(burst);
        hipLaunchKernelGGL(queue_look_kernel, dim3((B + 63) / 64), dim3(64), 0, st, c->kv->st, B, c->q_look.p);
        HIPRET(hipGetLastError());
        HIPCHK(hipMemcpyAsync(c->q_pinned, c->q_look.p, ((size_t)3 * B + 1) * sizeof(int), hipMemcpyDeviceToHost, st));
        HIPCHK(hipStreamSynchronize(st));
        if (c->q_pinned[3 * B] != 0)
            return fail(ER_ERR_INVALID, "er_queue_run: a row had no finite candidate score (non-finite logits); HF would raise in multinomial/argmax");
        const int rc = c->q.collect(c->q_pinned, c->q_pinned + B, c->q_pinned + 2 * B, done_rows, n_done);
        if (rc < 0) return fail(rc, "%s", c->q.why);
    }
    HIPCHK(hipEventRecord(c->ev1, st));
    HIPCHK(hipStreamSynchronize(st));
    float ms = 0.f;
    HIPCHK(hipEventElapsedTime(&ms, c->ev0, c->ev1));
    c->q.stats.decode_ms += ms;
    return ER_OK;
}

extern "C" int er_queue_take(er_ctx* c, int row, int64_t* ids_out, int capacity, int32_t* n_tokens) {
    ERCHK(queue_open(c, "er_queue_take"));
    if (!ids_out || !n_tokens) return fail(ER_ERR_INVALID, "er_queue_take: bad argument");
    const int rc = c->q.check_take(row, capacity);
    if (rc < 0) return fail(rc, "%s", c->q.why);
    const int n = c->q.rows[(size_t)row].n_tokens;
    HIPCHK(hipMemcpy(ids_out, c->kv->d_out_ids.p + (size_t)row * c->kv->plan.Lcap, (size_t)n * sizeof(long long), hipMemcpyDeviceToHost));
    hipLaunchKernelGGL(queue_park_kernel, dim3(1), dim3(64), 0, c->own_stream, c->kv->st, c->kv->d_row_budget.p, row, 1);
    HIPRET(hipGetLastError());
    HIPCHK(hipStreamSynchronize(c->own_stream));
    *n_tokens = n;
    c->q.release(row);
    return ER_OK;
}

extern "C" int er_queue_stats(er_ctx* c, er_queue_counters* out) {
    if (!c || !out) return fail(ER_ERR_INVALID, "er_queue_stats: bad argument");
    if (!c->q.active) return fail(ER_ERR_INVALID, "er_queue_stats: no queue is open");
    *out = c->q.stats;
    return ER_OK;
}

extern "C" int er_queue_end(er_ctx* c) {
    ERCHK(queue_open(c, "er_queue_end"));
    const int B = c->q.slots;
    HIPCHK(hipDeviceSynchronize());
    hipLaunchKernelGGL(fill_i32_kernel, dim3((B + 63) / 64), dim3(64), 0, c->own_stream, c->kv->d_row_budget.p, B, 0x7fffffff);
    HIPRET(hipGetLastError());
    HIPCHK(hipStreamSynchronize(c->own_stream));
    c->q.end();
    c->have_hidden = false;
    if (c->q_pinned) { hipHostFree(c->q_pinned); c->q_pinned = nullptr; }
    return er_set_row_streams(c, nullptr, B);
}

extern "C" int er_last_decode_ms(er_ctx* c, float* ms) {
    if (!c || !ms) return fail(ER_ERR_INVALID, "null");
    *ms = c->last_decode_ms;
    return ER_OK;
}

static int profile_impl(er_ctx* c, int repeats, int use_graph, float* avg_us, double* bytes, void* stream);

extern "C" int er_profile_decode_kernels(er_ctx* c, int repeats, float* avg_us, double* bytes, void* stream) {
    return er_profile_decode_kernels_at(c, repeats, 0, 0, avg_us, bytes, stream);
}

extern "C" int er_profile_decode_kernels_at(er_ctx* c, int repeats, int context_len, int use_graph, float* avg_us, double* bytes,
                                            void* stream) {
    if (!c) return fail(ER_ERR_INVALID, "er_profile_decode_kernels: bad argument");
    if (context_len < 0 || context_len > c->kv->plan.Lcap) return fail(ER_ERR_CAPACITY, "profile: context_len %d outside the reserved cache (%d)", context_len, c->kv->plan.Lcap);
    c->prof_len = context_len;
    const int rc = profile_impl(c, repeats, use_graph, avg_us, bytes, stream);
    c->prof_len = 0;
    return rc;
}

static int profile_impl(er_ctx* c, int repeats, int use_graph, float* avg_us, double* bytes, void* stream) {
    if (!c || !avg_us || !bytes || repeats <= 0) return fail(ER_ERR_INVALID, "er_profile_decode_kernels: bad argument");
    if (!c->have_hidden) return fail(ER_ERR_INVALID, "profile: call er_prefill first");
    HIPCHK(hipSetDevice(c->device));
    hipStream_t st = pick(c, stream);
    const er_config& g = c->cfg;
    const DecodePlan& p = c->kv->plan;
    const int B = p.B, H = g.hidden_dim, I = g.intermediate_dim, nl = g.num_layers, V = g.vocab_size;
    HIPCHK(hipStreamSynchronize(st));
    HIPCHK(hipMemcpy(c->h_pinned, c->kv->st.pos, sizeof(int), hipMemcpyDeviceToHost));
    const double len = c->prof_len > 0 ? (double)c->prof_len : (double)c->h_pinned[0] + 1.0;
    std::vector<float> save_y((size_t)B * H);
    HIPCHK(hipMemcpy(save_y.data(), c->kv->ypre.p, save_y.size() * 4, hipMemcpyDeviceToHost));
    std::vector<int> save_state(gen_state_ints(B));
    HIPCHK(hipMemcpy(save_state.data(), c->kv->state_block.p, save_state.size() * sizeof(int), hipMemcpyDeviceToHost));
    std::vector<int> head_state = save_state;
    for (int b = 0; b < B; ++b) gen_state_carve(head_state.data(), B).ngen[b] = 0;
    DecodeParamsDev dp{};
    dp.mode = 0; dp.top_k = 10; dp.grammar = 2; dp.max_new = 1 << 30; dp.min_new = 0;
    dp.eos = g.eos_token_id; dp.pad = g.pad_token_id; dp.vocab = V;
    HIPCHK(hipMemcpy(c->kv->d_params.p, &dp, sizeof(dp), hipMemcpyHostToDevice));
    DevBuf<long long> dummy;
    ERCHK(dummy.ensure((size_t)B * 8));
    long long* dummy_ids = dummy.p;

    const double w = c->fast ? 2.0 : 4.0;
    bytes[0] = ((double)3 * H * H + 3 * H) * w + (double)B * (H + 3 * H) * w;
    bytes[1] = (double)B * 2.0 * len * H * w;
    bytes[2] = (double)B * g.num_heads * p.S_splits * (c->D + 2) * w + (double)B * H * w;
    bytes[3] = ((double)H * H + H) * w + (double)B * 3 * H * w;
    bytes[4] = ((double)I * H + I) * w + (double)B * (H + I) * w;
    bytes[5] = ((double)I * H + H) * w + (double)B * (I + 2 * H) * w;
    bytes[6] = ((double)V * H) * w + (double)B * (H + V) * w;
    bytes[7] = (double)B * V * w;

    if (p.v3) {
        bytes[3] += (double)g.num_heads * p.nch3 * (c->D + 2) * 4.0;
        bytes[2] = 0.0;
    }
    for (int kind = 0; kind < ER_NUM_KERNEL_KINDS; ++kind) {
        const bool per_layer = kind <= 5;
        if (!p.sel.merge_launch && kind == 2) { avg_us[kind] = 0.f; continue; }
        hipGraphExec_t gexec = nullptr;
        if (use_graph && per_layer) {
            hipGraph_t graph = nullptr;
            HIPCHK(hipStreamBeginCapture(c->own_stream, hipStreamCaptureModeRelaxed));
            hipError_t e = hipSuccess;
            for (int l = 0; l < nl && e == hipSuccess; ++l) e = launch_kind(c, kind, l, c->own_stream, dummy_ids, 8);
            hipError_t e2 = hipStreamEndCapture(c->own_stream, &graph);
            if (e != hipSuccess || e2 != hipSuccess) { if (graph) hipGraphDestroy(graph); return fail(ER_ERR_HIP, "profile: graph capture failed"); }
            HIPCHK(hipGraphInstantiate(&gexec, graph, nullptr, nullptr, 0));
            hipGraphDestroy(graph);
        }
        for (int pass = 0; pass < 2; ++pass) {
            const int reps = pass == 0 ? 1 : repeats;
            if (pass == 1) HIPCHK(hipEventRecord(c->ev0, st));
            int launches = 0;
            for (int r = 0; r < reps; ++r) {
                if (gexec) {
                    HIPCHK(hipGraphLaunch(gexec, st));
                    launches += nl;
                } else if (per_layer) {
                    for (int l = 0; l < nl; ++l) { HIPRET(launch_kind(c, kind, l, st, dummy_ids, 8)); ++launches; }
                } else {
                    for (int l = 0; l < nl; ++l) {
                        if (kind == 7) {
                            HIPCHK(hipMemcpyAsync(c->kv->state_block.p, head_state.data(), head_state.size() * sizeof(int), hipMemcpyHostToDevice, st));
                        }
                        HIPRET(launch_kind(c, kind, 0, st, dummy_ids, 8));
                        ++launches;
                    }
                }
            }
            if (pass == 1) {
                HIPCHK(hipEventRecord(c->ev1, st));
                HIPCHK(hipStreamSynchronize(st));
                float ms = 0.f;
                HIPCHK(hipEventElapsedTime(&ms, c->ev0, c->ev1));
                avg_us[kind] = ms * 1000.0f / (float)launches;
            }
        }
        if (gexec) hipGraphExecDestroy(gexec);
    }
    HIPCHK(hipStreamSynchronize(st));
    HIPCHK(hipMemcpy(c->kv->ypre.p, save_y.data(), save_y.size() * 4, hipMemcpyHostToDevice));
    HIPCHK(hipMemcpy(c->kv->state_block.p, save_state.data(), save_state.size() * sizeof(int), hipMemcpyHostToDevice));
    return ER_OK;
}

template <typename WT>
static int proj_entry(Proj proj, const ProjForm& f, ProjIo io, GemvArgs a, int B, int K, float* part_out, hipStream_t st) {
    const int form = f.form, n = a.N;
    const size_t groups = (size_t)(B + NBM - 1) / NBM;
    const int slices = form == ER_FORM_NARROW || form == ER_FORM_NARROW_DEFER ? K / (4 * GM_KW) : K / (GM_WAVES * GM_KW);
    DevBuf<float> tmp, part;
    DevBuf<char> wt, img;
    SkPart sk{nullptr, 0};
    hipError_t e = hipSuccess;
    if (form != ER_FORM_ROW && form != ER_FORM_ROWS8) {
        if (io.pro != PRO_NONE && !a.hout) { ERCHK(tmp.ensure((size_t)B * K)); a.hout = tmp.p; }
        if (form_mfma(form)) {
            ERCHK(wt.ensure(tiled_weight_bytes<WT>(n, K)));
            if (form != ER_FORM_NARROW_DEFER) ERCHK(part.ensure((size_t)slices * NBM * n));
            sk = form == ER_FORM_NARROW_DEFER ? SkPart{part_out, groups * slices * NBM * (size_t)n} : SkPart{part.p, part.n};
        }
        if (form == ER_FORM_MFMA_XT) {
            if (!io.pro_image) {
                ERCHK(img.ensure(groups * (size_t)K * 128));
                HIPCHK(hipMemsetAsync(img.p, 0, groups * (size_t)K * 128, st));
                io.pro_image = img.p;
            }
            io.x_image = io.pro_image;
        }
        if (form_mfma(form)) {
            hipLaunchKernelGGL((tile_weights_kernel<WT>), dim3(2048), dim3(ER_WG), 0, st, reinterpret_cast<const WT*>(a.W), reinterpret_cast<f32x4*>(wt.p), n, K);
            e = hipGetLastError();
            io.w_tiled = wt.p;
        }
    }
    if (e == hipSuccess) e = form == ER_FORM_PREP ? launch_prologue(io.pro, a, B, io.rd, io.pro_image, st) : run_proj<WT>(proj, f, io, a, B, K, sk, st);
    hipError_t e2 = hipStreamSynchronize(st);
    HIPRET(e);
    HIPRET(e2);
    return ER_OK;
}

extern "C" int er_k_gemv(const float* w, const float* bias, const float* x, const float* ln_w, const float* ln_b,
                         const float* resid, float* y, float* xnorm_out, int B, int n, int k, int relu, float eps, void* stream) {
    hipStream_t st = (hipStream_t)stream;
    GemvArgs a{};
    a.W = w; a.bias = bias; a.N = n; a.xin = x; a.ln_w = ln_w; a.ln_b = ln_b; a.eps = eps; a.hout = xnorm_out;
    a.out = y; a.resid = resid;
    const bool batched = B > 4;
    if (batched && ln_w && k != 1536) return fail(ER_ERR_UNSUPPORTED, "er_k_gemv: LayerNorm prologue needs k=1536");
    Proj proj = PROJ_FC2;
    bool built = k == 6144 && !relu && resid && !ln_w;
    if (k == 1536 && !(relu && resid)) {
        proj = relu ? PROJ_FC1 : resid ? PROJ_OUT : PROJ_HEAD;
        built = batched || (ln_w != nullptr) == (proj != PROJ_OUT);
    }
    if (!built) {
        if (batched) HIPRET(hipErrorInvalidValue);
        if (k != 1536 && k != 6144) return fail(ER_ERR_UNSUPPORTED, "er_k_gemv: k must be 1536 or 6144");
        return fail(ER_ERR_UNSUPPORTED, "er_k_gemv: combination not instantiated for k=%d", k);
    }
    const bool wide = proj == PROJ_FC1 || proj == PROJ_FC2;
    ProjIo io;
    io.pro = ln_w ? PRO_LN : PRO_NONE;
    if (batched) {
        const ProjForm f{wide && !env_is("ER_BATCHED_VALU", '1') ? ER_FORM_MFMA : ER_FORM_VALU, 0, 0, false};
        return proj_entry<float>(proj, f, io, a, B, k, nullptr, st);
    }
    HIPRET(run_proj<float>(proj, ProjForm{ER_FORM_ROW, ER_NWAVES, wide ? 2 : 1, false}, io, a, B, k, SkPart{nullptr, 0}, st));
    return ER_OK;
}

extern "C" int er_k_attn_decode(const float* q, const void* k, const void* v, const int32_t* len_host, float* out, int B,
                                int heads, int head_dim, int l_cap, int steps, int kv_half, int variant, void* stream) {
    if (variant != ER_ATTN_SPLIT1 && variant != ER_ATTN_SPLIT2 && variant != ER_ATTN_STREAM)
        return fail(ER_ERR_INVALID, "er_k_attn_decode: variant must be ER_ATTN_SPLIT1, ER_ATTN_SPLIT2 or ER_ATTN_STREAM");
    if (variant == ER_ATTN_STREAM && head_dim != 96) return fail(ER_ERR_UNSUPPORTED, "the streaming kernel is built for head_dim 96");
    if (head_dim != 96 && head_dim != 64) return fail(ER_ERR_UNSUPPORTED, "head_dim %d", head_dim);
    if (steps != 2 && steps != 4 && steps != 8) return fail(ER_ERR_INVALID, "steps must be 2, 4 or 8 (chunk = 32*steps keys)");
    hipStream_t st = (hipStream_t)stream;
    const int S = attn_num_chunks(l_cap, attn_chunk(steps, kv_half != 0));
    DevBuf<int> len_dev;
    DevBuf<float> part;
    ERCHK(len_dev.ensure(B));
    ERCHK(part.ensure((size_t)B * heads * S * (head_dim + 2)));
    HIPCHK(hipMemcpy(len_dev.p, len_host, B * sizeof(int), hipMemcpyHostToDevice));
    AttnDecArgs a{};
    a.q = q; a.kcache = k; a.vcache = v; a.len_dev = len_dev.p; a.part = part.p; a.out = out;
    a.H = heads; a.l_cap = l_cap; a.S = S; a.hidden = heads * head_dim; a.chunk = attn_chunk(steps, kv_half != 0);
    a.kv_bstride = (long long)heads * l_cap * head_dim; a.sqrt_d = sqrtf((float)head_dim);
    hipError_t e;
    if (variant == ER_ATTN_STREAM) {
        e = launch_attn_stream_d<96>(a, kv_half != 0, B, st);
    } else {
        e = launch_attn_partial(a, head_dim, steps, kv_half != 0, B, st, variant == ER_ATTN_SPLIT1 ? 1 : 2);
        if (e == hipSuccess) e = launch_attn_combine(a, head_dim, B, st);
    }
    hipError_t e2 = hipStreamSynchronize(st);
    HIPRET(e);
    HIPRET(e2);
    return ER_OK;
}

extern "C" int er_k_attn_stream_xt(const float* q, const void* k, const void* v, const int32_t* len_host, float* out, void* out_xt, int B,
                                   int heads, int l_cap, int kv_half, void* stream) {
    constexpr int D = 96;
    if (!q || !k || !v || !len_host || !out || B < 1 || heads < 1 || l_cap < 1) return fail(ER_ERR_INVALID, "er_k_attn_stream_xt: bad argument");
    for (int b = 0; b < B; ++b)
        if (len_host[b] < 1 || len_host[b] > l_cap) return fail(ER_ERR_CAPACITY, "er_k_attn_stream_xt: len[%d] = %d / l_cap %d", b, len_host[b], l_cap);
    hipStream_t st = (hipStream_t)stream;
    DevBuf<int> len_dev;
    ERCHK(len_dev.ensure(B));
    HIPCHK(hipMemcpy(len_dev.p, len_host, B * sizeof(int), hipMemcpyHostToDevice));
    AttnDecArgs a{};
    a.q = q; a.kcache = k; a.vcache = v; a.len_dev = len_dev.p; a.out = out; a.out_xt = out_xt;
    a.H = heads; a.l_cap = l_cap; a.hidden = heads * D; a.kv_bstride = (long long)heads * l_cap * D; a.sqrt_d = sqrtf((float)D);
    hipError_t e = launch_attn_stream_d<D>(a, kv_half != 0, B, st);
    hipError_t e2 = hipStreamSynchronize(st);
    HIPRET(e);
    HIPRET(e2);
    return ER_OK;
}

static int gemv_form_check(const er_k_gemv_form_args& f, Proj* proj_out) {
    const int B = f.batch, n = f.n, k = f.k, pro = f.prologue, epi = f.epilogue, form = f.form;
    const bool half = f.w_half != 0;
    if (B < 1 || B > ER_MAX_BATCH || n < 1) return fail(ER_ERR_INVALID, "er_k_gemv_form: batch %d, n %d", B, n);
    if (k != 1536 && k != 6144) return fail(ER_ERR_UNSUPPORTED, "er_k_gemv_form: k must be 1536 or 6144");
    Proj proj = PROJ_QKV;
    const bool prep = form == ER_FORM_PREP;
    if (prep) {
        if (k != 1536 || pro == ER_PRO_NONE) return fail(ER_ERR_UNSUPPORTED, "er_k_gemv_form: the prologue launch is built for k=1536 and LN / EMBED");
        if (!f.xnorm_out) return fail(ER_ERR_INVALID, "er_k_gemv_form: ER_FORM_PREP needs xnorm_out");
    } else {
        if (!f.w) return fail(ER_ERR_INVALID, "er_k_gemv_form: null weights");
        if (epi == ER_EPI_QKV && k == 1536 && pro != ER_PRO_NONE) proj = PROJ_QKV;
        else if (epi == ER_EPI_RELU && k == 1536 && (pro == ER_PRO_LN || pro == ER_PRO_LN_SK)) proj = PROJ_FC1;
        else if (epi == ER_EPI_RESID && pro == ER_PRO_NONE) proj = k == 1536 ? PROJ_OUT : PROJ_FC2;
        else if (epi == ER_EPI_STORE && k == 1536 && pro == ER_PRO_LN) proj = PROJ_HEAD;
        else return fail(ER_ERR_UNSUPPORTED, "er_k_gemv_form: no decode projection has k=%d, prologue %d, epilogue %d", k, pro, epi);
    }
    if (pro == ER_PRO_NONE && !f.x) return fail(ER_ERR_INVALID, "er_k_gemv_form: null x");
    if (pro == ER_PRO_LN && (!f.x || !f.ln_w || !f.ln_b)) return fail(ER_ERR_INVALID, "er_k_gemv_form: PRO_LN needs x, ln_w, ln_b");
    if (pro == ER_PRO_EMBED && (!f.embd || !f.posemb || !f.tok || !f.pos)) return fail(ER_ERR_INVALID, "er_k_gemv_form: PRO_EMBED needs embd, posemb, tok, pos");
    if (pro == ER_PRO_LN_SK) {
        if (!f.sk_part || !f.sk_bias || !f.sk_resid || !f.ln_w || !f.ln_b) return fail(ER_ERR_INVALID, "er_k_gemv_form: PRO_LN_SK needs sk_part, sk_bias, sk_resid, ln_w, ln_b");
        if (!half || form == ER_FORM_ROW || form == ER_FORM_ROWS8) return fail(ER_ERR_UNSUPPORTED, "er_k_gemv_form: a deferred finish is read by the fast-mode batched prologue only");
        const int want = prep ? f.sk_slices : proj == PROJ_QKV ? SK_SLICES_FC2 : proj == PROJ_FC1 ? SK_SLICES_OUTPROJ : f.sk_slices;
        if ((f.sk_slices != SK_SLICES_OUTPROJ && f.sk_slices != SK_SLICES_FC2) || f.sk_slices != want)
            return fail(ER_ERR_UNSUPPORTED, "er_k_gemv_form: sk_slices %d (qkv reads 16, fc1 reads 4)", f.sk_slices);
    }
    if (!prep && proj == PROJ_QKV) {
        if (!f.q_out || !f.kcache || !f.vcache || !f.pos) return fail(ER_ERR_INVALID, "er_k_gemv_form: EPI_QKV needs q_out, kcache, vcache, pos");
        if (f.heads < 1 || f.head_dim < 1 || f.l_cap < 1 || f.heads * f.head_dim != k || n != 3 * k)
            return fail(ER_ERR_INVALID, "er_k_gemv_form: EPI_QKV needs heads * head_dim == k and n == 3 k");
    } else if (!prep) {
        if (!f.y && !(form == ER_FORM_MFMA_XT && proj == PROJ_FC1) && form != ER_FORM_NARROW_DEFER) return fail(ER_ERR_INVALID, "er_k_gemv_form: null y");
        if (epi == ER_EPI_RESID && !f.resid && form != ER_FORM_NARROW_DEFER) return fail(ER_ERR_INVALID, "er_k_gemv_form: EPI_RESID needs resid");
    }
    if (f.prep_xt_out && !(half && pro != ER_PRO_NONE && (form == ER_FORM_MFMA_XT || form == ER_FORM_PREP)))
        return fail(ER_ERR_UNSUPPORTED, "er_k_gemv_form: prep_xt_out is written in front of the tiled fp16 forms only");
    if (form != ER_FORM_ROW && form != ER_FORM_ROWS8 && B <= 4) return fail(ER_ERR_UNSUPPORTED, "er_k_gemv_form: the batched forms run at batch > 4");
    if (form < ER_FORM_ROW || form > ER_FORM_PREP) return fail(ER_ERR_INVALID, "er_k_gemv_form: form %d", form);
    if (!prep && !proj_form_legal(proj, ProjForm{form, f.nw, f.rw, form == ER_FORM_NARROW_DEFER}, half, B))
        return fail(ER_ERR_UNSUPPORTED, "er_k_gemv_form: the decode step never launches projection %d in form %d (%d waves x %d rows) with %s weights at batch %d",
                    (int)proj, form, f.nw, f.rw, half ? "fp16" : "fp32", B);
    if (form == ER_FORM_MFMA_XT && proj == PROJ_FC1 && (!f.xt_out || n % 4)) return fail(ER_ERR_INVALID, "er_k_gemv_form: the tiled fc1 writes xt_out (n a multiple of 4)");
    if (form == ER_FORM_NARROW_DEFER && !f.part_out) return fail(ER_ERR_INVALID, "er_k_gemv_form: ER_FORM_NARROW_DEFER needs part_out");
    *proj_out = proj;
    return ER_OK;
}

template <typename WT>
static int gemv_form_t(const er_k_gemv_form_args& f, Proj proj, hipStream_t st) {
    GemvArgs a{};
    a.W = f.w; a.bias = f.bias; a.N = f.n; a.xin = f.x; a.ln_w = f.ln_w; a.ln_b = f.ln_b; a.eps = f.eps; a.hout = f.xnorm_out;
    a.embd = f.embd; a.posemb = f.posemb; a.tok = f.tok; a.pos = f.pos;
    a.out = f.y; a.resid = f.resid; a.q = f.q_out; a.kcache = f.kcache; a.vcache = f.vcache; a.kv_half = f.kv_half ? 1 : 0;
    a.hidden = f.form != ER_FORM_PREP && proj == PROJ_QKV ? f.heads * f.head_dim : 1536; a.head_dim = f.head_dim; a.l_cap = f.l_cap;
    a.kv_bstride = (long long)f.heads * f.l_cap * f.head_dim;
    ProjIo io;
    io.pro = f.prologue == ER_PRO_NONE ? PRO_NONE : f.prologue == ER_PRO_EMBED ? PRO_EMBED : PRO_LN;
    if (f.prologue == ER_PRO_LN_SK) io.rd = {f.sk_part, f.sk_bias, f.sk_resid, f.sk_slices};
    io.pro_image = f.prep_xt_out; io.x_image = f.x; io.out_image = f.xt_out;
    return proj_entry<WT>(proj, ProjForm{f.form, f.nw, f.rw, f.form == ER_FORM_NARROW_DEFER}, io, a, f.batch, f.k, f.part_out, st);
}

extern "C" int er_k_gemv_form(const er_k_gemv_form_args* f, void* stream) {
    if (!f) return fail(ER_ERR_INVALID, "er_k_gemv_form: null args");
    Proj proj = PROJ_QKV;
    ERCHK(gemv_form_check(*f, &proj));
    return f->w_half ? gemv_form_t<_Float16>(*f, proj, (hipStream_t)stream) : gemv_form_t<float>(*f, proj, (hipStream_t)stream);
}

extern "C" int er_k_attn_outproj3(const float* q, const void* k, const void* v, int len, const void* wo, const float* bo,
                                  const float* resid, float* y, int l_cap, int kv_half, int w_half, void* stream) {
    constexpr int H = 16, D = 96;
    if (len <= 0 || len > l_cap || !attn3_fits(l_cap, H)) return fail(ER_ERR_CAPACITY, "er_k_attn_outproj3: len %d / l_cap %d (<= %d)", len, l_cap, attn3_num_chunks(H) * ATTN3_CAP);
    hipStream_t st = (hipStream_t)stream;
    const int nch = attn3_num_chunks(H);
    DevBuf<float> blk;
    ERCHK(blk.ensure((size_t)H * nch * (D + 2)));
    float *part = blk.p, *part_ml = part + (size_t)H * nch * D;
    AttnDecArgs a{};
    a.q = q; a.kcache = k; a.vcache = v; a.fixed_len = len; a.part = part; a.part_ml = part_ml;
    a.H = H; a.l_cap = l_cap; a.hidden = H * D; a.kv_bstride = (long long)H * l_cap * D; a.sqrt_d = sqrtf((float)D);
    hipError_t e = launch_attn_partial3_d<D>(a, kv_half != 0, nch, 1, st);
    OutMergeArgs m{};
    m.W = wo; m.bias = bo; m.resid = resid; m.out = y; m.part_o = part; m.part_ml = part_ml; m.N = H * D;
    if (e == hipSuccess) e = w_half ? launch_outproj_merge<_Float16, D>(m, nch, st) : launch_outproj_merge<float, D>(m, nch, st);
    hipError_t e2 = hipStreamSynchronize(st);
    HIPRET(e);
    HIPRET(e2);
    return ER_OK;
}

extern "C" int er_k_gemm(const float* a, const float* b, const float* bias, const float* resid, float* cc, int m, int n, int k,
                         int lda, int ldb, int ldc, int b_is_kn, int relu, float div, void* stream) {
    if (k % 16) return fail(ER_ERR_INVALID, "er_k_gemm: k must be a multiple of 16");
    GemmArgs g = gemm_args_default();
    g.A = a; g.B = b; g.C = cc; g.bias = bias; g.resid = resid; g.M = m; g.N = n; g.K = k;
    g.lda = lda; g.ldb = ldb; g.ldc = ldc; g.ldr = ldc; g.b_is_kn = b_is_kn; g.kb_valid = k; g.relu = relu; g.div = div;
    HIPRET(launch_gemm(g, 1, (hipStream_t)stream));
    return ER_OK;
}

extern "C" int er_k_gemm_f16(const float* a, const void* w, const float* bias, const float* resid, float* cc, int m, int n, int k,
                             int lda, int ldb, int ldc, int relu, void* stream) {
    if (k % 32) return fail(ER_ERR_INVALID, "er_k_gemm_f16: k must be a multiple of 32");
    GemmArgs g = gemm_args_default();
    g.A = a; g.B = reinterpret_cast<const float*>(w); g.C = cc; g.bias = bias; g.resid = resid; g.M = m; g.N = n; g.K = k;
    g.lda = lda; g.ldb = ldb; g.ldc = ldc; g.ldr = ldc; g.relu = relu;
    HIPRET(launch_gemm_f16(g, (hipStream_t)stream));
    return ER_OK;
}

extern "C" int er_k_gemm_hh(const float* a, const void* w, const float* bias, const float* resid, float* cc, void* c16_out, int m,
                            int n, int k, int lda, int ldb, int ldc, int relu, void* stream) {
    if (k % 64 || (ldb & 7)) return fail(ER_ERR_INVALID, "er_k_gemm_hh: k must be a multiple of 64, ldb of 8");
    hipStream_t st = (hipStream_t)stream;
    DevBuf<_Float16> a16b;
    ERCHK(a16b.ensure((size_t)m * k));
    _Float16* a16 = a16b.p;
    hipLaunchKernelGGL(cvt_rows_f16_kernel, dim3(ew_grid((long long)m * k)), dim3(ER_WG), 0, st, a, a16, (long long)m, k, lda, k);
    GemmArgs g = gemm_args_default();
    g.A = reinterpret_cast<const float*>(a16); g.B = reinterpret_cast<const float*>(w); g.C = cc; g.bias = bias; g.resid = resid;
    g.M = m; g.N = n; g.K = k; g.lda = k; g.ldb = ldb; g.ldc = ldc; g.ldr = ldc; g.relu = relu;
    g.c16 = reinterpret_cast<_Float16*>(c16_out); g.ldc16 = n;
    hipError_t e = launch_gemm_hh(g, st);
    hipError_t e2 = hipStreamSynchronize(st);
    HIPRET(e);
    HIPRET(e2);
    return ER_OK;
}

extern "C" int er_k_gemm_hh_qkv(const float* a, const void* w, const float* bias, void* qk16_out, void* vt_out, int m, int n, int k,
                                int rows_per_batch, int force_tile, void* stream) {
    if (k % 64 || n % 192 || m % 64 || rows_per_batch <= 0 || rows_per_batch % 64 || m % rows_per_batch)
        return fail(ER_ERR_INVALID, "er_k_gemm_hh_qkv: k, m, rows_per_batch multiples of 64, n of 192");
    hipStream_t st = (hipStream_t)stream;
    DevBuf<_Float16> a16b;
    ERCHK(a16b.ensure((size_t)m * k));
    _Float16* a16 = a16b.p;
    hipLaunchKernelGGL(cvt_rows_f16_kernel, dim3(ew_grid((long long)m * k)), dim3(ER_WG), 0, st, a, a16, (long long)m, k, k, k);
    GemmArgs g = gemm_args_default();
    g.A = reinterpret_cast<const float*>(a16); g.B = reinterpret_cast<const float*>(w); g.bias = bias;
    g.M = m; g.N = n; g.K = k; g.lda = k; g.ldb = k; g.ldc = n; g.ldr = n;
    g.c16 = reinterpret_cast<_Float16*>(qk16_out); g.ldc16 = n;
    g.vt16 = reinterpret_cast<_Float16*>(vt_out); g.vt_col0 = 2 * (n / 3); g.vt_rows = rows_per_batch; g.vt_ld = rows_per_batch;
    hipError_t e = launch_gemm_hh(g, st, force_tile);
    hipError_t e2 = hipStreamSynchronize(st);
    HIPRET(e);
    HIPRET(e2);
    return ER_OK;
}

extern "C" int er_k_gemm_hh_geglu(const float* a, const void* w, const float* bias, void* out16, int m, int f, int k, int force_tile,
                                  void* stream) {
    if (!a || !w || !bias || !out16) return fail(ER_ERR_INVALID, "er_k_gemm_hh_geglu: a, w, bias and out16 are required (the permute pass reads the bias)");
    if (k % 64 || f % 64 || m <= 0) return fail(ER_ERR_INVALID, "er_k_gemm_hh_geglu: k and f must be multiples of 64");
    if (force_tile != 0 && force_tile != 1 && force_tile != 2 && force_tile != 4) return fail(ER_ERR_INVALID, "er_k_gemm_hh_geglu: force_tile 0 / 1 / 2 / 4");
    hipStream_t st = (hipStream_t)stream;
    DevBuf<_Float16> a16b, wpb;
    DevBuf<float> bpb;
    ERCHK(a16b.ensure((size_t)m * k));
    ERCHK(wpb.ensure((size_t)2 * f * k));
    ERCHK(bpb.ensure((size_t)2 * f));
    _Float16 *a16 = a16b.p, *wp = wpb.p;
    float* bp = bpb.p;
    hipLaunchKernelGGL(cvt_rows_f16_kernel, dim3(ew_grid((long long)m * k)), dim3(ER_WG), 0, st, a, a16, (long long)m, k, k, k);
    hipLaunchKernelGGL(geglu_permute_kernel, dim3(2 * f), dim3(ER_WG), 0, st, reinterpret_cast<const _Float16*>(w), bias, wp, bp, f, k);
    GemmArgs g = gemm_args_default();
    g.A = reinterpret_cast<const float*>(a16); g.B = reinterpret_cast<const float*>(wp); g.bias = bp;
    g.M = m; g.N = 2 * f; g.K = k; g.lda = k; g.ldb = k; g.ldc = 2 * f; g.ldr = 2 * f;
    g.c16 = reinterpret_cast<_Float16*>(out16); g.ldc16 = f;
    hipError_t e = launch_gemm_hh_geglu(g, st, force_tile);
    hipError_t e2 = hipStreamSynchronize(st);
    HIPRET(e);
    HIPRET(e2);
    return ER_OK;
}

extern "C" int er_k_gemm_f16s(const float* a, const void* w, const float* bias, const float* resid, float* cc, int m, int n, int k,
                              int lda, int ldb, int ldc, int relu, void* stream) {
    if (k % 32) return fail(ER_ERR_INVALID, "er_k_gemm_f16s: k must be a multiple of 32");
    hipStream_t st = (hipStream_t)stream;
    GemmArgs g = gemm_args_default();
    g.A = a; g.B = reinterpret_cast<const float*>(w); g.C = cc; g.bias = bias; g.resid = resid; g.M = m; g.N = n; g.K = k;
    g.lda = lda; g.ldb = ldb; g.ldc = ldc; g.ldr = ldc; g.relu = relu;
    const bool force_reg = env_is("ER_K_GEMM_F16S_FORM", 'r');
    if (k % XBK == 0 && !(ldb & 7) && !force_reg) {
        DevBuf<_Float16> hi, lo;
        ERCHK(hi.ensure((size_t)m * k));
        ERCHK(lo.ensure((size_t)m * k));
        hipLaunchKernelGGL(split_rows_f16_kernel, split_rows_grid(m, k), dim3(ER_WG), 0, st, a, hi.p, lo.p, (long long)m, k, lda);
        g.A = reinterpret_cast<const float*>(hi.p); g.a_lo = lo.p; g.lda = k;
        hipError_t e = launch_gemm_hh_split(g, st);
        hipError_t e2 = hipStreamSynchronize(st);
        HIPRET(e);
        HIPRET(e2);
        return ER_OK;
    }
    HIPRET(launch_gemm_f16s(g, st));
    return ER_OK;
}

extern "C" int er_k_flash_attn_f16(const float* q, const float* k, const float* v, float* o, int B, int H, int N, int M,
                                   void* stream) {
    FlashArgs a{};
    a.Q = q; a.K = k; a.V = v; a.O = o; a.N = N; a.M = M;
    a.ldq = a.ldk = a.ldv = a.ldo = H * FA_D;
    a.qs_b = (long long)N * H * FA_D; a.os_b = a.qs_b; a.ks_b = (long long)M * H * FA_D; a.vs_b = a.ks_b;
    a.head_stride = FA_D; a.scale = 1.0f / sqrtf((float)FA_D);
    HIPRET(launch_flash_attn_f16(a, H, B, (hipStream_t)stream));
    return ER_OK;
}

extern "C" int er_k_flash_attn_hh(const float* q, const float* k, const float* v, float* o, int B, int H, int N, int M, void* stream) {
    hipStream_t st = (hipStream_t)stream;
    const int C = H * FA_D, Mp = (M + 63) / 64 * 64;
    DevBuf<_Float16> q16b, k16b, v16b, vtb, o16b;
    ERCHK(q16b.ensure((size_t)B * N * C));
    ERCHK(k16b.ensure((size_t)B * M * C));
    ERCHK(v16b.ensure((size_t)B * M * C));
    ERCHK(vtb.ensure((size_t)B * H * 64 * Mp));
    ERCHK(o16b.ensure((size_t)B * N * C));
    _Float16 *q16 = q16b.p, *k16 = k16b.p, *v16 = v16b.p, *vt = vtb.p, *o16 = o16b.p;
// ... 224 lines not shown
```

### edgerunner_amd/csrc/er_decode_plan.h

```cpp
#pragma once
#include "../../include/edgerunner_hip.h"

namespace er {

struct DecodeKnobs {
    bool use_graph = true;
    int nw_qkv = 6, nw_fc1 = 4;
    int prefill_attn_f16s = -1;
    int attn_v_batched = 0;
    int decode_v = 3;
    int rw_fc2 = 6;
};

struct ReserveKnobs { bool force_batched, batched_valu, xt; };

struct AttnChunking {
    int nch3;
    int cap3;
    int chunk;
};

struct DecodePlan {
    int B = 0, Lcap = 0, layers = 0;
    long long kv_bstride = 0, kv_lstride = 0;
    int S_splits = 0, nch3 = 0;
    er_decode_plan sel{};
    bool force_batched = false;
    bool batched = false;
    bool valu = false;
    bool mfma = false;
    bool xt = false;
    bool stream_attn = false;
    bool v3 = false;
    bool outproj_rows8 = false;
    bool outproj_partials = false;
    bool fc2_defers(int layer) const { return xt && layer >= 0 && layer + 1 < layers; }
};

inline void plan_decode(int decode_v, int attn_v_batched, bool force_batched, int batch, int H, int D, int hid, int Lcap,
                        const AttnChunking& ch, er_decode_plan* p) {
    p->batched = (batch > 4 || force_batched) ? 1 : 0;
    p->attn_chunks = ch.nch3;
    const bool v3 = decode_v == 3 && batch == 1 && !p->batched && D == 96 && H == 16 && hid == 1536 && Lcap <= ch.cap3;
    p->decode_version = v3 ? 3 : 2;
    const bool stream = p->batched && D == 96 && (attn_v_batched == 3 || (attn_v_batched == 0 && batch * H >= 256));
    p->attn_kernel = !p->batched ? (v3 ? ER_ATTN_BALANCED : ER_ATTN_SPLIT2)
                                 : (stream ? ER_ATTN_STREAM : ER_ATTN_SPLIT1);
    p->merge_launch = (p->attn_kernel == ER_ATTN_SPLIT1 || p->attn_kernel == ER_ATTN_SPLIT2) ? 1 : 0;
    p->launches_per_layer = p->batched ? 0 : 5 + p->merge_launch;
}

inline DecodePlan make_decode_plan(const DecodeKnobs& k, const ReserveKnobs& rk, bool fast, int batch, int Lcap, int layers, int H, int D,
                                   int hid, const AttnChunking& ch) {
    DecodePlan p;
    p.B = batch; p.Lcap = Lcap; p.layers = layers;
    p.kv_bstride = (long long)H * Lcap * D; p.kv_lstride = p.kv_bstride * batch;
    p.S_splits = (Lcap + ch.chunk - 1) / ch.chunk;
    p.nch3 = ch.nch3;
    p.force_batched = rk.force_batched; p.valu = rk.batched_valu;
    plan_decode(k.decode_v, k.attn_v_batched, p.force_batched, batch, H, D, hid, Lcap, ch, &p.sel);
    p.batched = p.sel.batched != 0; p.mfma = p.batched && !p.valu; p.xt = fast && p.mfma && rk.xt;
    p.stream_attn = p.sel.attn_kernel == ER_ATTN_STREAM; p.v3 = p.sel.decode_version == 3;
    p.outproj_rows8 = p.mfma && batch >= 5 && batch <= 8;
    p.outproj_partials = p.xt && p.stream_attn && batch > 8;
    return p;
}

enum Proj { PROJ_QKV = 0, PROJ_OUT, PROJ_FC1, PROJ_FC2, PROJ_HEAD };

struct ProjForm {
    int form = ER_FORM_ROW;
    int nw = 0, rw = 0;
    bool defer = false;
};

inline bool form_batched(int form) { return form == ER_FORM_VALU || form == ER_FORM_MFMA || form == ER_FORM_MFMA_XT || form == ER_FORM_NARROW || form == ER_FORM_NARROW_DEFER; }
inline bool form_tiled_in(int form) { return form == ER_FORM_MFMA_XT || form == ER_FORM_NARROW || form == ER_FORM_NARROW_DEFER; }
inline bool form_mfma(int form) { return form == ER_FORM_MFMA || form_tiled_in(form); }

inline ProjForm proj_form(const DecodePlan& p, const DecodeKnobs& k, bool half, Proj proj, int layer) {
    const auto batched = [&](int tiled) { return ProjForm{p.xt && half ? tiled : p.mfma ? ER_FORM_MFMA : ER_FORM_VALU, 0, 0, false}; };
    switch (proj) {
        case PROJ_QKV:
            if (p.batched) return batched(ER_FORM_MFMA_XT);
            return ProjForm{ER_FORM_ROW, k.nw_qkv, k.nw_qkv == 9 ? 2 : 1, false};
        case PROJ_OUT:
            if (p.outproj_rows8) return ProjForm{ER_FORM_ROWS8, 3, 1, false};
            if (p.outproj_partials && half) return ProjForm{ER_FORM_NARROW_DEFER, 0, 0, true};
            if (p.mfma) return ProjForm{ER_FORM_MFMA, 0, 0, false};
            if (p.batched) return ProjForm{ER_FORM_VALU, 0, 0, false};
            return ProjForm{ER_FORM_ROW, 3, 1, false};
        case PROJ_FC1:
            if (p.batched) return batched(ER_FORM_MFMA_XT);
            return ProjForm{ER_FORM_ROW, k.nw_fc1, 2, false};
        case PROJ_FC2:
            if (p.xt && half) return p.fc2_defers(layer) ? ProjForm{ER_FORM_NARROW_DEFER, 0, 0, true} : ProjForm{ER_FORM_NARROW, 0, 0, false};
            if (p.mfma) return ProjForm{ER_FORM_MFMA, 0, 0, false};
            if (p.batched) return ProjForm{ER_FORM_VALU, 0, 0, false};
            if (half && p.B == 1 && (k.rw_fc2 == 6 || k.rw_fc2 == 4)) return ProjForm{ER_FORM_ROW, 4, k.rw_fc2, false};
            return ProjForm{ER_FORM_ROW, 4, 2, false};
        case PROJ_HEAD:
            return p.batched ? ProjForm{ER_FORM_VALU, 0, 0, false} : ProjForm{ER_FORM_ROW, 4, 1, false};
    }
    return ProjForm{};
}

inline bool proj_form_legal(Proj proj, const ProjForm& f, bool half, int B) {
    if (B < 1 || f.defer != (f.form == ER_FORM_NARROW_DEFER)) return false;
    switch (f.form) {
        case ER_FORM_ROW:
            if (B > 4) return false;
            switch (proj) {
                case PROJ_QKV: return (f.nw == 4 && f.rw == 1) || (f.nw == 6 && f.rw == 1) || (f.nw == 9 && f.rw == 2);
                case PROJ_OUT: return f.nw == 3 && f.rw == 1;
                case PROJ_FC1: return (f.nw == 4 || f.nw == 12) && f.rw == 2;
                case PROJ_FC2: return f.nw == 4 && (f.rw == 2 || (half && B == 1 && (f.rw == 4 || f.rw == 6)));
                case PROJ_HEAD: return f.nw == 4 && f.rw == 1;
            }
            return false;
        case ER_FORM_ROWS8: return proj == PROJ_OUT && B >= 5 && B <= 8;
        case ER_FORM_VALU: return true;
        case ER_FORM_MFMA: return proj != PROJ_HEAD;
        case ER_FORM_MFMA_XT: return half && (proj == PROJ_QKV || proj == PROJ_FC1);
        case ER_FORM_NARROW: return half && proj == PROJ_FC2;
        case ER_FORM_NARROW_DEFER: return half && (proj == PROJ_OUT || proj == PROJ_FC2);
    }
    return false;
}

}
```

### edgerunner_amd/kernels.py

```python
from __future__ import annotations

import ctypes as C

import torch

from . import native


def _st():
    return C.c_void_p(torch.cuda.current_stream().cuda_stream)


def gemv(w, x, bias=None, ln_w=None, ln_b=None, resid=None, relu=False, eps=1e-5, return_xnorm=False):
    lib = native.load_library()
    B, K = x.shape
    N = w.shape[0]
    y = torch.empty((B, N), dtype=torch.float32, device=x.device)
    xn = torch.empty_like(x) if return_xnorm else None
    native.check(lib.er_k_gemv(native.ptr(w), native.ptr(bias), native.ptr(x), native.ptr(ln_w), native.ptr(ln_b),
                               native.ptr(resid), native.ptr(y), native.ptr(xn), B, N, K, int(relu), float(eps), _st()),
                 "er_k_gemv")
    return (y, xn) if return_xnorm else y


def attn_decode(q, k_cache, v_cache, lens, steps=4, variant=native.ER_ATTN_SPLIT2):
    lib = native.load_library()
    B, H, Lcap, D = k_cache.shape
    out = torch.empty((B, H * D), dtype=torch.float32, device=q.device)
    native.check(lib.er_k_attn_decode(native.ptr(q), native.ptr(k_cache), native.ptr(v_cache), native.i32_array(lens),
                                      native.ptr(out), B, H, D, Lcap, steps, int(k_cache.dtype == torch.float16), int(variant), _st()),
                 "er_k_attn_decode")
    return out


def xt_pack_image(x):
    B, K = x.shape
    assert x.dtype == torch.float32 and K % 4 == 0
    G = (B + 31) // 32
    xp = torch.zeros((G * 32, K), dtype=torch.float32, device=x.device)
    xp[:B] = x
    hi = xp.half()
    lo = (xp - hi.float()).half()
    hi, lo = (t.view(G, 32, K // 4, 4).permute(0, 2, 1, 3) for t in (hi, lo))
    return torch.cat((hi, lo), dim=3).contiguous()


def xt_unpack_image(img, B=None):
    G, K4, _, _ = img.shape
    hi, lo = (img[..., s].permute(0, 2, 1, 3).reshape(G * 32, K4 * 4) for s in (slice(0, 4), slice(4, 8)))
    n = G * 32 if B is None else B
    return hi[:n].contiguous(), lo[:n].contiguous()


def _i32_dev(values, device, hi, what):
    v = [int(t) for t in (values.tolist() if torch.is_tensor(values) else values)]
    assert all(0 <= t < hi for t in v), f"{what} outside [0, {hi})"
    return torch.tensor(v, dtype=torch.int32, device=device)


def gemv_form(form, epilogue, w, B, *, x=None, bias=None, ln=None, embed=None, sk=None, resid=None, qkv=None, nw=4, rw=1, eps=1e-5,
              n=None, k=None, w_half=None, return_xnorm=False, prep_xt=False, prep_xt_image=None, xt_out_image=None):
    lib = native.load_library()
    dev = (x if x is not None else (embed[0] if embed is not None else sk[0])).device
    if w is not None:
        n, k = w.shape
        w_half = w.dtype == torch.float16
    a = native.ErKGemvFormArgs()
    keep = [w, x, bias, resid]
    a.w, a.bias, a.x, a.resid = (native.ptr(t).value for t in (w, bias, x, resid))
    a.w_half, a.batch, a.n, a.k, a.epilogue, a.form, a.nw, a.rw, a.eps = int(bool(w_half)), B, n, k, epilogue, form, nw, rw, eps
    pro = native.ER_PRO_NONE
    if ln is not None:
        pro = native.ER_PRO_LN
        a.ln_w, a.ln_b = native.ptr(ln[0]).value, native.ptr(ln[1]).value
    if embed is not None:
        pro = native.ER_PRO_EMBED
        embd, posemb, tok, pos = embed
        tok_d, pos_d = _i32_dev(tok, dev, embd.shape[0], "token"), _i32_dev(pos, dev, posemb.shape[0], "position")
        assert len(tok_d) == B and len(pos_d) == B and embd.shape[1] == k and posemb.shape[1] == k
        keep += [tok_d, pos_d]
        a.embd, a.posemb, a.tok, a.pos = (native.ptr(t).value for t in (embd, posemb, tok_d, pos_d))
    if sk is not None:
        pro = native.ER_PRO_LN_SK
        part, sk_bias, sk_resid, slices = sk
        groups = (B + 31) // 32
        assert part.numel() >= groups * slices * 32 * k and sk_resid.shape == (B, k) and sk_bias.numel() == k
        a.sk_part, a.sk_bias, a.sk_resid, a.sk_slices = native.ptr(part).value, native.ptr(sk_bias).value, native.ptr(sk_resid).value, slices
    a.prologue = pro
    if x is not None and pro in (native.ER_PRO_NONE, native.ER_PRO_LN):
        tiled = form in (native.ER_FORM_NARROW, native.ER_FORM_NARROW_DEFER)
        assert x.numel() * x.element_size() == ((B + 31) // 32 * 32 if tiled else B) * k * 4, "x does not hold B rows of k (tiled: whole groups)"
    out = {}
    if pro != native.ER_PRO_NONE and (return_xnorm or form == native.ER_FORM_PREP):
        out["xnorm"] = torch.empty((B, k), dtype=torch.float32, device=dev)
        a.xnorm_out = native.ptr(out["xnorm"]).value
    if prep_xt or prep_xt_image is not None:
        out["prep_xt"] = prep_xt_image if prep_xt_image is not None else torch.zeros(((B + 31) // 32, k // 4, 32, 8), dtype=torch.float16, device=dev)
        assert out["prep_xt"].numel() == (B + 31) // 32 * k * 64
        a.prep_xt_out = native.ptr(out["prep_xt"]).value
    if epilogue == native.ER_EPI_QKV and form != native.ER_FORM_PREP:
        kc, vc, pos = qkv[:3]
        _, heads, l_cap, hd = kc.shape
        assert kc.shape == vc.shape and kc.shape[0] == B and kc.dtype == vc.dtype and kc.dtype in (torch.float32, torch.float16)
        pos_d = _i32_dev(pos, dev, l_cap, "cache position")
        assert len(pos_d) == B
        out["q"] = qkv[3] if len(qkv) > 3 else torch.empty((B, heads * hd), dtype=torch.float32, device=dev)
        assert out["q"].shape == (B, heads * hd) and out["q"].dtype == torch.float32
        keep += [pos_d]
        a.pos = native.ptr(pos_d).value
        a.q_out, a.kcache, a.vcache = native.ptr(out["q"]).value, native.ptr(kc).value, native.ptr(vc).value
        a.kv_half, a.heads, a.head_dim, a.l_cap = int(kc.dtype == torch.float16), heads, hd, l_cap
    elif form == native.ER_FORM_NARROW_DEFER:
        out["part"] = torch.empty(((B + 31) // 32, (k // 384) * 32 * n), dtype=torch.float32, device=dev)
        a.part_out = native.ptr(out["part"]).value
    elif form == native.ER_FORM_MFMA_XT and epilogue == native.ER_EPI_RELU:
        out["xt_out"] = xt_out_image if xt_out_image is not None else torch.zeros(((B + 31) // 32, n // 4, 32, 8), dtype=torch.float16, device=dev)
        assert out["xt_out"].numel() == (B + 31) // 32 * n * 64
        a.xt_out = native.ptr(out["xt_out"]).value
    elif form != native.ER_FORM_PREP:
        out["y"] = torch.empty((B, n), dtype=torch.float32, device=dev)
        a.y = native.ptr(out["y"]).value
    native.check(lib.er_k_gemv_form(C.byref(a), _st()), "er_k_gemv_form")
    del keep
    return out


def attn_stream_xt(q, k_cache, v_cache, lens, out_xt):
    lib = native.load_library()
    B, H, Lcap, D = k_cache.shape
    assert D == 96 and out_xt.dtype == torch.float16 and out_xt.numel() == (B + 31) // 32 * H * D * 64
    out = torch.empty((B, H * D), dtype=torch.float32, device=q.device)
    native.check(lib.er_k_attn_stream_xt(native.ptr(q), native.ptr(k_cache), native.ptr(v_cache), native.i32_array(lens), native.ptr(out),
                                         native.ptr(out_xt), B, H, Lcap, int(k_cache.dtype == torch.float16), _st()), "er_k_attn_stream_xt")
    return out


def attn_outproj3(q, k_cache, v_cache, length, wo, bo, resid):
    lib = native.load_library()
    H, Lcap, D = k_cache.shape
    assert (H, D) == (16, 96)
    y = torch.empty((H * D,), dtype=torch.float32, device=q.device)
    native.check(lib.er_k_attn_outproj3(native.ptr(q), native.ptr(k_cache), native.ptr(v_cache), int(length), native.ptr(wo),
                                        native.ptr(bo), native.ptr(resid), native.ptr(y), Lcap,
                                        int(k_cache.dtype == torch.float16), int(wo.dtype == torch.float16), _st()),
                 "er_k_attn_outproj3")
    return y


def gemm(a, b, bias=None, resid=None, b_is_kn=False, relu=False, div=0.0, m=None, n=None, k=None):
    lib = native.load_library()
    M = a.shape[0] if m is None else m
    K = a.shape[1] if k is None else k
    N = (b.shape[1] if b_is_kn else b.shape[0]) if n is None else n
    c = torch.empty((M, N), dtype=torch.float32, device=a.device)
    native.check(lib.er_k_gemm(native.ptr(a), native.ptr(b), native.ptr(bias), native.ptr(resid), native.ptr(c), M, N, K,
                               a.stride(0), b.stride(0), c.stride(0), int(b_is_kn), int(relu), float(div), _st()),
                 "er_k_gemm")
    return c


def gemm_f16(a, w_half, bias=None, resid=None, relu=False):
    lib = native.load_library()
    M, K = a.shape
    N = w_half.shape[0]
    c = torch.empty((M, N), dtype=torch.float32, device=a.device)
    native.check(lib.er_k_gemm_f16(native.ptr(a), native.ptr(w_half), native.ptr(bias), native.ptr(resid), native.ptr(c), M, N, K,
                                   a.stride(0), w_half.stride(0), c.stride(0), int(relu), _st()), "er_k_gemm_f16")
    return c


def gemm_hh(a, w_half, bias=None, resid=None, relu=False, return_half=False):
    lib = native.load_library()
    M, K = a.shape
    N = w_half.shape[0]
    c = torch.empty((M, N), dtype=torch.float32, device=a.device)
    c16 = torch.empty((M, N), dtype=torch.float16, device=a.device) if return_half else None
    native.check(lib.er_k_gemm_hh(native.ptr(a), native.ptr(w_half), native.ptr(bias), native.ptr(resid), native.ptr(c), native.ptr(c16),
                                  M, N, K, a.stride(0), w_half.stride(0), c.stride(0), int(relu), _st()), "er_k_gemm_hh")
    return (c, c16) if return_half else c


def gemm_hh_qkv(a, w_half, bias, rows_per_batch, force_tile=0):
    lib = native.load_library()
    M, K = a.shape
    N = w_half.shape[0]
    heads = N // 192
    qk16 = torch.zeros((M, N), dtype=torch.float16, device=a.device)
    vt = torch.zeros((M // rows_per_batch, heads, 64, rows_per_batch), dtype=torch.float16, device=a.device)
    native.check(lib.er_k_gemm_hh_qkv(native.ptr(a.contiguous()), native.ptr(w_half.contiguous()), native.ptr(bias), native.ptr(qk16), native.ptr(vt),
                                      M, N, K, rows_per_batch, force_tile, _st()), "er_k_gemm_hh_qkv")
    return qk16, vt


def gemm_hh_geglu(a, w_half, bias, force_tile=0):
    lib = native.load_library()
    M, K = a.shape
    F = w_half.shape[0] // 2
    out = torch.empty((M, F), dtype=torch.float16, device=a.device)
    native.check(lib.er_k_gemm_hh_geglu(native.ptr(a.contiguous()), native.ptr(w_half.contiguous()), native.ptr(bias), native.ptr(out), M, F, K,
                                        force_tile, _st()), "er_k_gemm_hh_geglu")
    return out


def gemm_f16s(a, w_half, bias=None, resid=None, relu=False):
    lib = native.load_library()
    M, K = a.shape
    N = w_half.shape[0]
    c = torch.empty((M, N), dtype=torch.float32, device=a.device)
    native.check(lib.er_k_gemm_f16s(native.ptr(a), native.ptr(w_half), native.ptr(bias), native.ptr(resid), native.ptr(c), M, N, K,
                                   a.stride(0), w_half.stride(0), c.stride(0), int(relu), _st()), "er_k_gemm_f16s")
    return c


def flash_attn_f16(q, k, v, heads):
    lib = native.load_library()
    B, N, _ = q.shape
    M = k.shape[1]
    o = torch.empty_like(q)
    native.check(lib.er_k_flash_attn_f16(native.ptr(q), native.ptr(k), native.ptr(v), native.ptr(o), B, heads, N, M, _st()),
                 "er_k_flash_attn_f16")
    return o


def flash_attn_hh(q, k, v, heads):
    lib = native.load_library()
    B, N, _ = q.shape
    M = k.shape[1]
    o = torch.empty_like(q)
    native.check(lib.er_k_flash_attn_hh(native.ptr(q), native.ptr(k), native.ptr(v), native.ptr(o), B, heads, N, M, _st()),
                 "er_k_flash_attn_hh")
    return o


def flash_attn_f32(q, k, v, heads, causal=False):
    lib = native.load_library()
    B, N, HD = q.shape
    M = k.shape[1]
    o = torch.empty_like(q)
    native.check(lib.er_k_flash_attn_f32(native.ptr(q), native.ptr(k), native.ptr(v), native.ptr(o), B, heads, N, M, HD // heads,
                                         int(causal), _st()), "er_k_flash_attn_f32")
    return o



def flash_attn_f16s(q, k, v, heads, causal=False):
    lib = native.load_library()
    B, N, HD = q.shape
    assert HD // heads == 96
    M = k.shape[1]
    o = torch.empty_like(q)
    native.check(lib.er_k_flash_attn_f16s(native.ptr(q), native.ptr(k), native.ptr(v), native.ptr(o), B, heads, N, M,
                                          int(causal), _st()), "er_k_flash_attn_f16s")
    return o

def layernorm(x, w, b, eps=1e-5):
    lib = native.load_library()
    y = torch.empty_like(x)
    native.check(lib.er_k_layernorm(native.ptr(x), native.ptr(w), native.ptr(b), native.ptr(y), x.shape[0], x.shape[1],
                                    float(eps), _st()), "er_k_layernorm")
    return y


def softmax_(s, cols, causal=False):
    lib = native.load_library()
    native.check(lib.er_k_softmax(native.ptr(s), s.shape[0], cols, s.stride(0), int(causal), _st()), "er_k_softmax")
    return s


def score_rows(logits, labels):
    lib = native.load_library()
    B, S, V = logits.shape
    lab = labels.to(logits.device, torch.int32).contiguous()
    nll = torch.empty((B, S), dtype=torch.float32, device=logits.device)
    pred = torch.empty((B, S), dtype=torch.int32, device=logits.device)
    loss = torch.empty((2,), dtype=torch.float32, device=logits.device)
    native.check(lib.er_k_score_rows(native.ptr(logits), native.ptr(lab), B, S, V, native.ptr(nll), native.ptr(pred),
                                     native.ptr(loss), _st()), "er_k_score_rows")
    return nll, pred, loss

# ... 92 lines not shown
```

### edgerunner_amd/native.py

```python
from __future__ import annotations

import ctypes as C
import os
from typing import Optional, Sequence

PKG = os.path.dirname(os.path.abspath(__file__))
LIB_PATH = os.environ.get("ER_LIB_PATH") or os.path.join(PKG, "libedgerunner_hip.so")

ER_F32, ER_F16, ER_BF16 = 0, 1, 2
ER_COND_NONE, ER_COND_POINT, ER_COND_POINT_LATENT = 0, 1, 2
ER_GREEDY, ER_SAMPLE = 0, 1
ER_GRAMMAR_NONE, ER_GRAMMAR_NAIVE9, ER_GRAMMAR_LR_ABSCO = 0, 1, 2
ER_METO_LR_ABSCO, ER_METO_LR = 0, 1
ER_NUM_KERNEL_KINDS = 8
ER_PRED_V_PREDICTION, ER_PRED_EPSILON = 0, 1
ER_PE_EMBED, ER_PE_DOWNSAMPLE = 0, 1

EXPORTS = [
    "er_abi_version", "er_last_error", "er_create", "er_destroy", "er_load_tensor", "er_finalize_weights",
    "er_kv_reserve", "er_encode_cond", "er_embed_tokens", "er_prefill", "er_score", "er_point_latent", "er_set_point_encoder_mode", "er_logits", "er_feed", "er_decode",
    "er_meto_decode", "er_meto_encode", "er_dit_create", "er_dit_destroy", "er_dit_load_tensor",
    "er_dit_finalize_weights", "er_dit_project_cond", "er_dit_encode_image", "er_dit_forward", "er_dit_sample",
    "er_dit_set_prediction_type", "er_dit_attach_point_encoder", "er_dit_point_latent", "er_dit_set_point_encoder_mode", "er_dit_loss", "er_k_dit_loss",
    "er_set_row_streams", "er_plan_decode", "er_ctx_plan", "er_plan_gemm_tile", "er_kernel_kind_name", "er_profile_decode_kernels", "er_profile_decode_kernels_at", "er_last_decode_ms",
    "er_k_gemv", "er_k_gemv_form", "er_k_attn_decode", "er_k_attn_stream_xt", "er_k_attn_outproj3", "er_k_gemm", "er_k_gemm_f16", "er_k_gemm_hh", "er_k_gemm_hh_qkv", "er_k_gemm_hh_geglu", "er_k_gemm_f16s", "er_k_flash_attn_f16", "er_k_flash_attn_hh", "er_k_flash_attn_f32", "er_k_flash_attn_f16s", "er_k_layernorm", "er_k_softmax", "er_k_score_rows", "er_k_fps", "er_k_sample_head",
    "er_k_nn_dist2", "er_k_surface_sample", "er_k_fidelity_metrics",
    "er_queue_begin", "er_queue_admit", "er_queue_run", "er_queue_take", "er_queue_stats", "er_queue_end",
]


ER_ATTN_SPLIT1, ER_ATTN_SPLIT2, ER_ATTN_BALANCED, ER_ATTN_STREAM = 1, 2, 3, 4


class ErDecodePlan(C.Structure):
    _fields_ = [(n, C.c_int32) for n in ("batched", "decode_version", "attn_kernel", "attn_chunks", "merge_launch",
                                         "launches_per_layer")]


ER_PRO_NONE, ER_PRO_LN, ER_PRO_EMBED, ER_PRO_LN_SK = 0, 1, 2, 3
ER_EPI_STORE, ER_EPI_RELU, ER_EPI_RESID, ER_EPI_QKV = 0, 1, 2, 3
ER_FORM_ROW, ER_FORM_ROWS8, ER_FORM_VALU, ER_FORM_MFMA, ER_FORM_MFMA_XT, ER_FORM_NARROW, ER_FORM_NARROW_DEFER, ER_FORM_PREP = range(8)


class ErKGemvFormArgs(C.Structure):
    _fields_ = [(n, C.c_void_p) for n in (
        "w", "bias", "x", "ln_w", "ln_b", "xnorm_out", "embd", "posemb", "tok", "pos", "sk_part", "sk_bias", "sk_resid", "y", "resid",
        "q_out", "kcache", "vcache", "prep_xt_out", "xt_out", "part_out")] + [(n, C.c_int32) for n in (
        "w_half", "kv_half", "batch", "n", "k", "prologue", "epilogue", "form", "nw", "rw", "sk_slices", "heads", "head_dim",
        "l_cap")] + [("eps", C.c_float)]


class ErConfig(C.Structure):
    _fields_ = [(n, C.c_int32) for n in (
        "hidden_dim", "num_heads", "num_layers", "intermediate_dim", "vocab_size", "max_positions",
        "num_cond_tokens", "point_hidden_dim", "point_num_heads", "point_latent_size", "point_latent_dim",
        "point_freq_dim", "num_face_buckets", "cond_mode", "pad_token_id", "bos_token_id", "eos_token_id",
        "weight_dtype", "kv_dtype")] + [("ln_eps", C.c_float)]


class ErDitConfig(C.Structure):
    _fields_ = [(n, C.c_int32) for n in ("hidden_dim", "num_heads", "num_layers", "latent_size", "latent_dim", "clip_dim",
                                         "clip_layers", "clip_heads", "clip_mlp_dim", "clip_image_size", "clip_patch", "weight_dtype")]


class ErDecodeParams(C.Structure):
    _fields_ = [("mode", C.c_int32), ("top_k", C.c_int32), ("grammar", C.c_int32),
                ("max_new_tokens", C.c_int32), ("min_new_tokens", C.c_int32), ("seed", C.c_uint64)]


class ErQueueCounters(C.Structure):
    _fields_ = [(n, C.c_int64) for n in ("steps", "admissions", "occupied_row_steps", "wait_row_steps", "parked_row_steps")] + \
               [("prefill_ms", C.c_float), ("decode_ms", C.c_float)]


class NativeError(RuntimeError):
    pass


_lib = None


def load_library(path: Optional[str] = None) -> C.CDLL:
    global _lib
    if _lib is not None and path is None:
        return _lib
    p = path or LIB_PATH
    if not os.path.exists(p):
        raise NativeError(
            f"HIP extension not built: {p} is missing. Run `python -m edgerunner_amd.build` "
            "(hipcc --offload-arch=gfx950). There is no CPU/eager fallback for this path.")
    lib = C.CDLL(p)
    vp, ci, cf = C.c_void_p, C.c_int, C.c_float
    lib.er_abi_version.restype = ci
    lib.er_last_error.restype = C.c_char_p
    lib.er_kernel_kind_name.restype = C.c_char_p
    lib.er_kernel_kind_name.argtypes = [ci]
    lib.er_create.argtypes = [C.POINTER(ErConfig), ci, C.POINTER(vp)]
    lib.er_destroy.argtypes = [vp]
    lib.er_load_tensor.argtypes = [vp, C.c_char_p, vp, ci, ci, C.POINTER(C.c_int64), ci]
    lib.er_finalize_weights.argtypes = [vp]
    lib.er_kv_reserve.argtypes = [vp, ci, ci]
    lib.er_encode_cond.argtypes = [vp, vp, ci, ci, C.POINTER(C.c_int32), vp, vp]
    lib.er_embed_tokens.argtypes = [vp, C.POINTER(C.c_int32), ci, ci, vp, vp]
    lib.er_prefill.argtypes = [vp, vp, ci, ci, vp]
    lib.er_logits.argtypes = [vp, vp, vp]
    lib.er_score.argtypes = [vp, vp, vp, ci, ci, vp, vp, vp, vp, vp]
    lib.er_point_latent.argtypes = [vp, vp, ci, ci, vp, vp, vp]
    lib.er_set_point_encoder_mode.argtypes = [vp, ci]
    lib.er_feed.argtypes = [vp, C.POINTER(C.c_int32), vp]
    lib.er_decode.argtypes = [vp, C.POINTER(ErDecodeParams), vp, C.POINTER(C.c_int32), vp]
    lib.er_profile_decode_kernels.argtypes = [vp, ci, C.POINTER(C.c_float), C.POINTER(C.c_double), vp]
    lib.er_profile_decode_kernels_at.argtypes = [vp, ci, ci, ci, C.POINTER(C.c_float), C.POINTER(C.c_double), vp]
    lib.er_last_decode_ms.argtypes = [vp, C.POINTER(C.c_float)]
    i32p = C.POINTER(C.c_int32)
    lib.er_meto_decode.argtypes = [i32p, ci, ci, ci, C.POINTER(C.c_float), i32p, i32p, i32p, i32p, i32p]
    lib.er_meto_encode.argtypes = [C.POINTER(C.c_float), ci, i32p, ci, ci, ci, i32p, i32p, i32p, i32p, i32p]
    lib.er_dit_create.argtypes = [C.POINTER(ErDitConfig), ci, C.POINTER(vp)]
    lib.er_dit_destroy.argtypes = [vp]
    lib.er_dit_load_tensor.argtypes = [vp, C.c_char_p, vp, ci, ci, C.POINTER(C.c_int64), ci]
    lib.er_dit_finalize_weights.argtypes = [vp]
    lib.er_dit_project_cond.argtypes = [vp, vp, ci, ci, vp, vp]
    lib.er_dit_encode_image.argtypes = [vp, vp, ci, ci, ci, vp, vp]
    lib.er_dit_forward.argtypes = [vp, vp, vp, C.POINTER(C.c_float), ci, ci, vp, vp]
    lib.er_dit_sample.argtypes = [vp, vp, ci, ci, vp, ci, cf, ci, vp]
    lib.er_dit_set_prediction_type.argtypes = [vp, ci]
    lib.er_dit_attach_point_encoder.argtypes = [vp, ci, ci, ci]
    lib.er_dit_point_latent.argtypes = [vp, vp, ci, ci, vp, vp]
    lib.er_dit_set_point_encoder_mode.argtypes = [vp, ci]
    lib.er_k_fps.argtypes = [vp, ci, ci, ci, vp, vp]
    lib.er_k_nn_dist2.argtypes = [vp, vp, ci, ci, ci, vp, vp, vp]
    lib.er_k_surface_sample.argtypes = [vp, vp, C.POINTER(C.c_int32), C.POINTER(C.c_int32), ci, ci, C.c_uint64, C.POINTER(C.c_uint32),
                                        vp, vp, vp]
    lib.er_k_fidelity_metrics.argtypes = [vp, vp, ci, ci, ci, cf, vp, vp]
    lib.er_dit_loss.argtypes = [vp, vp, vp, vp, C.POINTER(C.c_int32), ci, ci, cf, vp, vp, vp, vp]
    lib.er_k_dit_loss.argtypes = [vp, vp, vp, C.POINTER(C.c_int32), ci, ci, ci, cf, vp, vp, vp]
    lib.er_plan_decode.argtypes = [ci, ci, ci, ci, ci, C.POINTER(ErDecodePlan)]
    lib.er_ctx_plan.argtypes = [vp, C.POINTER(ErDecodePlan)]
    lib.er_set_row_streams.argtypes = [vp, C.POINTER(C.c_uint32), ci]
    lib.er_plan_gemm_tile.argtypes = [ci, ci, ci]
    lib.er_queue_begin.argtypes = [vp, C.POINTER(ErDecodeParams), ci, vp]
    lib.er_queue_admit.argtypes = [vp, ci, ci, vp, ci, C.POINTER(C.c_uint32), C.POINTER(C.c_int32), vp]
    lib.er_queue_run.argtypes = [vp, C.POINTER(C.c_int32), C.POINTER(C.c_int32), vp]
    lib.er_queue_take.argtypes = [vp, ci, C.POINTER(C.c_int64), ci, C.POINTER(C.c_int32)]
    lib.er_queue_stats.argtypes = [vp, C.POINTER(ErQueueCounters)]
    lib.er_queue_end.argtypes = [vp]
    lib.er_k_gemv.argtypes = [vp, vp, vp, vp, vp, vp, vp, vp, ci, ci, ci, ci, cf, vp]
    lib.er_k_gemv_form.argtypes = [C.POINTER(ErKGemvFormArgs), vp]
    lib.er_k_attn_stream_xt.argtypes = [vp, vp, vp, C.POINTER(C.c_int32), vp, vp, ci, ci, ci, ci, vp]
    lib.er_k_attn_decode.argtypes = [vp, vp, vp, C.POINTER(C.c_int32), vp, ci, ci, ci, ci, ci, ci, ci, vp]
    lib.er_k_attn_outproj3.argtypes = [vp, vp, vp, ci, vp, vp, vp, vp, ci, ci, ci, vp]
    lib.er_k_gemm.argtypes = [vp, vp, vp, vp, vp, ci, ci, ci, ci, ci, ci, ci, ci, cf, vp]
    lib.er_k_gemm_f16.argtypes = [vp, vp, vp, vp, vp, ci, ci, ci, ci, ci, ci, ci, vp]
    lib.er_k_gemm_f16s.argtypes = [vp, vp, vp, vp, vp, ci, ci, ci, ci, ci, ci, ci, vp]
    lib.er_k_gemm_hh.argtypes = [vp, vp, vp, vp, vp, vp, ci, ci, ci, ci, ci, ci, ci, vp]
    lib.er_k_gemm_hh_qkv.argtypes = [vp, vp, vp, vp, vp, ci, ci, ci, ci, ci, vp]
    lib.er_k_gemm_hh_geglu.argtypes = [vp, vp, vp, vp, ci, ci, ci, ci, vp]
    lib.er_k_flash_attn_f16.argtypes = [vp, vp, vp, vp, ci, ci, ci, ci, vp]
    lib.er_k_flash_attn_hh.argtypes = [vp, vp, vp, vp, ci, ci, ci, ci, vp]
    lib.er_k_flash_attn_f32.argtypes = [vp, vp, vp, vp, ci, ci, ci, ci, ci, ci, vp]
    lib.er_k_flash_attn_f16s.argtypes = [vp, vp, vp, vp, ci, ci, ci, ci, ci, vp]
    lib.er_k_layernorm.argtypes = [vp, vp, vp, vp, ci, ci, cf, vp]
    lib.er_k_softmax.argtypes = [vp, ci, ci, ci, ci, vp]
    lib.er_k_score_rows.argtypes = [vp, vp, ci, ci, ci, vp, vp, vp, vp]
    lib.er_k_sample_head.argtypes = [vp, C.POINTER(ErDecodeParams), ci, ci, ci, ci, ci, C.POINTER(C.c_int32),
                                     C.POINTER(C.c_int32), C.POINTER(C.c_int32), C.POINTER(C.c_int32),
                                     C.POINTER(C.c_int32), C.POINTER(C.c_int32), vp]
    for name in EXPORTS:
        fn = getattr(lib, name)
        if name not in ("er_last_error", "er_kernel_kind_name"):
            fn.restype = ci
    if lib.er_abi_version() != 1:
        raise NativeError(f"ABI version mismatch: library {lib.er_abi_version()}, binding 1")
    if path is None:
        _lib = lib
    return lib


def check(rc: int, what: str = "") -> int:
    if rc < 0:
        msg = load_library().er_last_error().decode(errors="replace")
        raise NativeError(f"{what} failed ({rc}): {msg}")
    return rc


def i32_array(values: Sequence[int]):
    return (C.c_int32 * len(values))(*[int(v) for v in values])


def ptr(t) -> C.c_void_p:
    if t is None:
        return C.c_void_p(0)
    assert t.is_contiguous(), "tensor handed to the C ABI must be contiguous"
    return C.c_void_p(t.data_ptr())


def load_tensor(fn, ctx, key: str, t) -> int:
    import torch
    dtypes = {torch.float32: ER_F32, torch.float16: ER_F16, torch.bfloat16: ER_BF16}
    if t.dtype not in dtypes:
        t = t.float()
    t = t.detach().contiguous()
    shape = (C.c_int64 * max(1, t.dim()))(*(list(t.shape) or [1]))
    return check(fn(ctx, key.encode(), ptr(t), dtypes[t.dtype], max(1, t.dim()), shape, 1 if t.is_cuda else 0),
                 f"{fn.__name__}({key})")


def stream_ptr(stream) -> C.c_void_p:
    import torch
    s = stream if stream is not None else torch.cuda.current_stream()
    return C.c_void_p(s.cuda_stream)
```

### edgerunner_amd/shape_opt.py

```python
from __future__ import annotations

import ctypes as C
from typing import Callable, Dict, Optional

import torch

from . import native
from .weights import ModelDims

_COND = {"none": native.ER_COND_NONE, "point": native.ER_COND_POINT, "point_latent": native.ER_COND_POINT_LATENT}
_DT = {torch.float32: native.ER_F32, torch.float16: native.ER_F16, torch.bfloat16: native.ER_BF16}


class BuiltinGrammar:

    def __init__(self, er_grammar: int, vocab_size: int, eos_token_id: int = 2):
        from .grammar import as_callable
        self.er_grammar = er_grammar
        self._fn = as_callable(er_grammar, vocab_size, eos_token_id)

    def __call__(self, batch_id, input_ids):
        return self._fn(batch_id, input_ids) if self._fn is not None else None


# ... 163 lines not shown
        with self._enter():
            kw = dict(dtype=torch.float32, device=self.device)
            nll = nll_out if nll_out is not None else torch.empty((B, S), **kw)
            pred = pred_out if pred_out is not None else torch.empty((B, S), dtype=torch.int32, device=self.device)
            logits = None if logits_out is False else (logits_out if logits_out is not None
                                                        else torch.empty((B, S, self.dims.vocab_size), **kw))
            loss = torch.empty((2,), **kw)
            native.check(self.lib.er_score(self._ctx, native.ptr(x), native.ptr(lab), B, S, native.ptr(nll), native.ptr(pred),
                                           native.ptr(logits), native.ptr(loss), self._sp()), "er_score")
        self._exit()
        return {"nll": nll, "pred": pred, "logits": logits, "loss": loss}

    def point_latent(self, conds: torch.Tensor):
        d = self.dims
        x = conds.to(self.device, torch.float32).contiguous()
        B, N = x.shape[0], x.shape[1]
        check_clouds(x, d)
        with self._enter():
            lat = torch.empty((B, d.point_latent_size, d.point_latent_dim), dtype=torch.float32, device=self.device)
            kl = torch.empty((1,), dtype=torch.float32, device=self.device)
            native.check(self.lib.er_point_latent(self._ctx, native.ptr(x), B, N, native.ptr(lat), native.ptr(kl), self._sp()),
                         "er_point_latent")
        self._exit()
        return lat, kl[0]

    def feed(self, ids):
        ids = [int(v) for v in (ids.flatten().tolist() if isinstance(ids, torch.Tensor) else ids)]
        with self._enter():
            native.check(self.lib.er_feed(self._ctx, native.i32_array(ids), self._sp()), "er_feed")
        self._exit()

    @torch.no_grad()
    def generate(self, inputs_embeds: torch.Tensor, num_tokens=None, pad_token_id=None, bos_token_id=None,
                 eos_token_id=None, max_new_tokens: Optional[int] = None,
                 prefix_allowed_tokens_fn: Optional[Callable] = None, num_beams: int = 1, do_sample: bool = False,
                 top_k: int = 50, min_new_tokens: int = 0, seed: Optional[int] = None, row_streams=None,
                 **unused) -> torch.Tensor:
        if num_beams != 1:
            raise NotImplementedError("beam search is not part of the reference's call (num_beams=1)")
        for name, got, want in (("pad", pad_token_id, self.opt.pad_token_id), ("bos", bos_token_id, self.opt.bos_token_id),
                                ("eos", eos_token_id, self.opt.eos_token_id)):
            if got is not None and got != want:
                raise ValueError(f"{name}_token_id={got} differs from the context's {want}")
        if max_new_tokens is None:
            max_new_tokens = self.opt.max_seq_length
        B = inputs_embeds.shape[0]
        self.prefill(inputs_embeds, max_new_tokens)
        if row_streams is not None and len(row_streams) != B:
            raise ValueError(f"row_streams has {len(row_streams)} entries for a batch of {B}")
        arr = None if row_streams is None else (C.c_uint32 * B)(*[int(v) & 0xFFFFFFFF for v in row_streams])
        native.check(self.lib.er_set_row_streams(self._ctx, arr, B), "er_set_row_streams")
        if prefix_allowed_tokens_fn is None or isinstance(prefix_allowed_tokens_fn, BuiltinGrammar):
            grammar = native.ER_GRAMMAR_NONE if prefix_allowed_tokens_fn is None else prefix_allowed_tokens_fn.er_grammar
            return self._decode_device(B, max_new_tokens, min_new_tokens, do_sample, top_k, grammar, seed)
        return self._decode_stepwise(B, max_new_tokens, min_new_tokens, do_sample, top_k, prefix_allowed_tokens_fn)

    def _decode_device(self, B, T, min_new, do_sample, top_k, grammar, seed):
        if seed is None:
            seed = int(torch.randint(0, 2 ** 62, (1,)).item()) if do_sample else 0
        p = native.ErDecodeParams(mode=native.ER_SAMPLE if do_sample else native.ER_GREEDY, top_k=int(top_k),
                                  grammar=int(grammar), max_new_tokens=int(T), min_new_tokens=int(min_new),
                                  seed=int(seed) & 0xFFFFFFFFFFFFFFFF)
        n = C.c_int32(0)
        with self._enter():
            out = torch.empty((B, T), dtype=torch.int64, device=self.device)
            native.check(self.lib.er_decode(self._ctx, C.byref(p), native.ptr(out), C.byref(n), self._sp()), "er_decode")
        self._exit()
        ms = C.c_float(0)
        self.lib.er_last_decode_ms(self._ctx, C.byref(ms))
        self.last_decode_ms = float(ms.value)
        return out[:, : n.value]

    def _decode_stepwise(self, B, T, min_new, do_sample, top_k, fn):
        eos, pad = self.opt.eos_token_id, self.opt.pad_token_id
        ids = torch.empty((B, 0), dtype=torch.long)
        unfinished = torch.ones(B, dtype=torch.long)
        for t in range(T):
            s = self.logits().float().cpu()
            if t < min_new:
                s[:, eos] = -float("inf")
            mask = torch.full_like(s, -float("inf"))
            for b in range(B):
                allowed = fn(b, ids[b])
                if len(allowed) == 0:
                    raise ValueError(f"`prefix_allowed_tokens_fn` returned an empty list for batch ID {b}.")
                mask[b, allowed] = 0
            s = s + mask
            if do_sample:
                k = min(top_k, s.shape[-1])
                kth = torch.topk(s, k)[0][..., -1, None]
                s = s.masked_fill(s < kth, -float("inf"))
                nxt = torch.multinomial(torch.softmax(s, dim=-1), 1).squeeze(1)
            else:
                nxt = torch.argmax(s, dim=-1)
            nxt = nxt * unfinished + pad * (1 - unfinished)
            ids = torch.cat([ids, nxt[:, None]], dim=-1)
            unfinished = unfinished & (nxt != eos).long()
            if unfinished.max() == 0 or t == T - 1:
                break
            self.feed(nxt)
        return ids.to(self.device)

    def queue_begin(self, slots: int, l_cap: int, max_new_tokens: int, min_new_tokens: int = 0, do_sample: bool = False,
                    top_k: int = 10, grammar: int = native.ER_GRAMMAR_NONE, seed: int = 0, check_every: int = 0):
        if self._reserved[0] != slots or self._reserved[1] < l_cap:
            self.reserve(slots, l_cap)
        p = native.ErDecodeParams(mode=native.ER_SAMPLE if do_sample else native.ER_GREEDY, top_k=int(top_k), grammar=int(grammar),
                                  max_new_tokens=int(max_new_tokens), min_new_tokens=int(min_new_tokens),
                                  seed=int(seed) & 0xFFFFFFFFFFFFFFFF)
        with self._enter():
            native.check(self.lib.er_queue_begin(self._ctx, C.byref(p), int(check_every), self._sp()), "er_queue_begin")
        self._exit()

    def queue_admit(self, row0: int, inputs_embeds: torch.Tensor, stream_ids=None, budgets=None):
        x = inputs_embeds.to(self.device, torch.float32).contiguous()
        n, S, _ = x.shape
        ids = None if stream_ids is None else (C.c_uint32 * n)(*[int(v) & 0xFFFFFFFF for v in stream_ids])
        bud = None if budgets is None else native.i32_array(budgets)
        if (ids is not None and len(stream_ids) != n) or (bud is not None and len(budgets) != n):
            raise ValueError(f"queue_admit: {n} rows need {n} stream ids / budgets")
        with self._enter():
            native.check(self.lib.er_queue_admit(self._ctx, int(row0), n, native.ptr(x), S, ids, bud, self._sp()), "er_queue_admit")
        self._exit()

    def queue_run(self):
        rows = (C.c_int32 * max(1, self._reserved[0]))()
        n = C.c_int32(0)
        with self._enter():
            native.check(self.lib.er_queue_run(self._ctx, rows, C.byref(n), self._sp()), "er_queue_run")
        self._exit()
        return [int(rows[i]) for i in range(n.value)]

    def queue_take(self, row: int, capacity: int):
        import numpy as np
        buf = np.empty((max(1, int(capacity)),), dtype=np.int64)
        n = C.c_int32(0)
        native.check(self.lib.er_queue_take(self._ctx, int(row), buf.ctypes.data_as(C.POINTER(C.c_int64)), int(capacity), C.byref(n)),
                     "er_queue_take")
        return buf[: n.value].copy()

    def queue_stats(self) -> Dict[str, float]:
        s = native.ErQueueCounters()
        native.check(self.lib.er_queue_stats(self._ctx, C.byref(s)), "er_queue_stats")
        return {n: (float if n.endswith("_ms") else int)(getattr(s, n)) for n, _ in native.ErQueueCounters._fields_}

    def queue_end(self):
        native.check(self.lib.er_queue_end(self._ctx), "er_queue_end")

    def plan(self):
        p = native.ErDecodePlan()
        native.check(self.lib.er_ctx_plan(self._ctx, C.byref(p)), "er_ctx_plan")
        return {n: int(getattr(p, n)) for n, _ in native.ErDecodePlan._fields_}

    def profile_decode_kernels(self, repeats: int = 5, context_len: int = 0, use_graph: bool = False):
        us = (C.c_float * native.ER_NUM_KERNEL_KINDS)()
        by = (C.c_double * native.ER_NUM_KERNEL_KINDS)()
        with self._enter():
            native.check(self.lib.er_profile_decode_kernels_at(self._ctx, repeats, int(context_len), 1 if use_graph else 0, us, by,
                                                               self._sp()), "er_profile")
        self._exit()
        return {self.lib.er_kernel_kind_name(k).decode(): {"avg_us": float(us[k]), "bytes": float(by[k])}
                for k in range(native.ER_NUM_KERNEL_KINDS)}
```

### include/edgerunner_hip.h

```cpp
#ifndef EDGERUNNER_HIP_H
#define EDGERUNNER_HIP_H

#include <stdint.h>

#ifdef __cplusplus
extern "C" {
#endif

#define ER_ABI_VERSION 1

typedef enum {
    ER_OK = 0,
    ER_ERR_INVALID = -1,
    ER_ERR_HIP = -2,
    ER_ERR_MISSING = -3,
    ER_ERR_CAPACITY = -4,
    ER_ERR_UNSUPPORTED = -5
} er_status;

typedef enum { ER_F32 = 0, ER_F16 = 1, ER_BF16 = 2 } er_dtype;
typedef enum { ER_COND_NONE = 0, ER_COND_POINT = 1, ER_COND_POINT_LATENT = 2 } er_cond_mode;
typedef enum { ER_GREEDY = 0, ER_SAMPLE = 1 } er_gen_mode;
typedef enum {
    ER_GRAMMAR_NONE = 0,
// ... 37 lines not shown

int er_kv_reserve(er_ctx* ctx, int batch, int max_len);

int er_encode_cond(er_ctx* ctx, const float* conds_dev, int batch, int n_points,
                   const int32_t* face_bucket_host, float* cond_out_dev, void* stream);

int er_embed_tokens(er_ctx* ctx, const int32_t* ids_host, int batch, int n_tokens,
                    float* out_dev, void* stream);

int er_prefill(er_ctx* ctx, const float* embeds_dev, int batch, int seq_len, void* stream);

int er_score(er_ctx* ctx, const float* embeds_dev, const int32_t* labels_dev, int batch, int seq_len,
             float* nll_out_dev, int32_t* pred_out_dev, float* logits_out_dev, float* loss_out_dev, void* stream);

int er_point_latent(er_ctx* ctx, const float* conds_dev, int batch, int n_points, float* latent_out_dev,
                    float* kl_out_dev, void* stream);

typedef enum { ER_PE_EMBED = 0, ER_PE_DOWNSAMPLE = 1 } er_point_encoder_mode;
int er_set_point_encoder_mode(er_ctx* ctx, int mode);

int er_logits(er_ctx* ctx, float* logits_out_dev, void* stream);

int er_feed(er_ctx* ctx, const int32_t* ids_host, void* stream);

int er_decode(er_ctx* ctx, const er_decode_params* p, int64_t* out_ids_dev,
              int32_t* n_steps_host, void* stream);
int er_set_row_streams(er_ctx* ctx, const uint32_t* ids_host, int n);

typedef struct {
    int64_t steps;
    int64_t admissions;
    int64_t occupied_row_steps;
    int64_t wait_row_steps;
    int64_t parked_row_steps;
    float prefill_ms, decode_ms;
} er_queue_counters;
int er_queue_begin(er_ctx* ctx, const er_decode_params* p, int check_every, void* stream);
int er_queue_admit(er_ctx* ctx, int row0, int n_rows, const float* embeds_dev, int S, const uint32_t* stream_ids_host,
                   const int32_t* max_new_host, void* stream);
int er_queue_run(er_ctx* ctx, int32_t* done_rows_host, int32_t* n_done, void* stream);
int er_queue_take(er_ctx* ctx, int row, int64_t* ids_out_host, int capacity, int32_t* n_tokens);
int er_queue_stats(er_ctx* ctx, er_queue_counters* out);
int er_queue_end(er_ctx* ctx);

enum er_meto_backend { ER_METO_LR_ABSCO = 0, ER_METO_LR = 1 };

int er_meto_decode(const int32_t* tokens_host, int n_tokens, int discrete_bins, int backend, float* vertices_out,
                   int32_t* faces_out, int32_t* face_type_out, int32_t* n_vertices, int32_t* n_faces,
                   int32_t* n_face_types);

int er_meto_encode(const float* vertices_host, int n_vertices, const int32_t* faces_host, int n_faces,
                   int discrete_bins, int backend, int32_t* tokens_out, int32_t* n_tokens, int32_t* face_order_out,
                   int32_t* face_type_out, int32_t* n_faces_out);

typedef struct {
    int32_t hidden_dim, num_heads, num_layers;
    int32_t latent_size, latent_dim;
    int32_t clip_dim;
    int32_t clip_layers, clip_heads, clip_mlp_dim;
    int32_t clip_image_size, clip_patch;
    int32_t weight_dtype;
} er_dit_config;
typedef struct er_dit_ctx er_dit_ctx;
int er_dit_create(const er_dit_config* cfg, int device, er_dit_ctx** out);
int er_dit_destroy(er_dit_ctx* ctx);
int er_dit_load_tensor(er_dit_ctx* ctx, const char* key, const void* data, int dtype, int ndim,
                       const int64_t* shape, int on_device);
int er_dit_finalize_weights(er_dit_ctx* ctx);
int er_dit_project_cond(er_dit_ctx* ctx, const float* clip_hidden_dev, int batch, int m_tokens,
                        float* cond_out_dev, void* stream);
int er_dit_encode_image(er_dit_ctx* ctx, const float* images_dev, int batch, int height, int width,
                        float* clip_hidden_out_dev, void* stream);
int er_dit_forward(er_dit_ctx* ctx, const float* x_dev, const float* c_dev, const float* t_host, int batch,
                   int m_tokens, float* out_dev, void* stream);
int er_dit_sample(er_dit_ctx* ctx, const float* cond_dev, int batch, int m_tokens, float* latents_dev,
                  int num_inference_steps, float guidance_scale, int init_step, void* stream);

typedef enum { ER_PRED_V_PREDICTION = 0, ER_PRED_EPSILON = 1 } er_pred_type;
int er_dit_set_prediction_type(er_dit_ctx* ctx, int pred_type);
int er_dit_attach_point_encoder(er_dit_ctx* ctx, int point_hidden_dim, int point_num_heads, int point_freq_dim);
int er_dit_point_latent(er_dit_ctx* ctx, const float* points_dev, int batch, int n_points, float* latent_out_dev, void* stream);
int er_dit_set_point_encoder_mode(er_dit_ctx* ctx, int mode);
int er_dit_loss(er_dit_ctx* ctx, const float* latents_dev, const float* noise_dev, const float* cond_dev,
                const int32_t* timesteps_host, int batch, int m_tokens, float snr_gamma, float* pred_out_dev,
                float* mse_out_dev, float* loss_out_dev, void* stream);

typedef enum { ER_ATTN_SPLIT1 = 1, ER_ATTN_SPLIT2 = 2, ER_ATTN_BALANCED = 3, ER_ATTN_STREAM = 4 } er_attn_kernel;
typedef struct {
    int32_t batched;
    int32_t decode_version;
    int32_t attn_kernel;
    int32_t attn_chunks;
    int32_t merge_launch;
    int32_t launches_per_layer;
} er_decode_plan;
int er_plan_decode(int batch, int heads, int head_dim, int hidden, int l_cap, er_decode_plan* out);
int er_ctx_plan(er_ctx* ctx, er_decode_plan* out);
int er_plan_gemm_tile(int m, int n, int batch);

#define ER_NUM_KERNEL_KINDS 8
const char* er_kernel_kind_name(int kind);
int er_profile_decode_kernels(er_ctx* ctx, int repeats, float* avg_us_out, double* bytes_out, void* stream);
int er_profile_decode_kernels_at(er_ctx* ctx, int repeats, int context_len, int use_graph, float* avg_us_out,
                                 double* bytes_out, void* stream);
int er_last_decode_ms(er_ctx* ctx, float* ms_out);

int er_k_gemv(const float* w_dev, const float* bias_dev, const float* x_dev, const float* ln_w_dev,
              const float* ln_b_dev, const float* resid_dev, float* y_dev, float* xnorm_out_dev,
              int batch, int n, int k, int relu, float eps, void* stream);
int er_k_attn_decode(const float* q_dev, const void* k_dev, const void* v_dev, const int32_t* len_host,
                     float* out_dev, int batch, int heads, int head_dim, int l_cap, int steps, int kv_half,
                     int variant, void* stream);
typedef enum { ER_PRO_NONE = 0, ER_PRO_LN = 1, ER_PRO_EMBED = 2,
               ER_PRO_LN_SK = 3
} er_gemv_prologue;
typedef enum { ER_EPI_STORE = 0, ER_EPI_RELU = 1, ER_EPI_RESID = 2, ER_EPI_QKV = 3 } er_gemv_epilogue;
typedef enum {
    ER_FORM_ROW = 0,
    ER_FORM_ROWS8 = 1,
    ER_FORM_VALU = 2,
    ER_FORM_MFMA = 3,
    ER_FORM_MFMA_XT = 4,
    ER_FORM_NARROW = 5,
    ER_FORM_NARROW_DEFER = 6,
    ER_FORM_PREP = 7
} er_gemv_form;
typedef struct {
    const void* w;
    const float* bias;
    const float* x;
    const float *ln_w, *ln_b;
    float* xnorm_out;
    const float *embd, *posemb;
    const int32_t* tok;
    const int32_t* pos;
    const float* sk_part;
    const float *sk_bias, *sk_resid;
    float* y;
    const float* resid;
    float* q_out;
    void *kcache, *vcache;
    void* prep_xt_out;
    void* xt_out;
    float* part_out;
    int32_t w_half, kv_half;
    int32_t batch, n, k;
    int32_t prologue, epilogue, form;
    int32_t nw, rw;
    int32_t sk_slices;
    int32_t heads, head_dim, l_cap;
    float eps;
} er_k_gemv_form_args;
int er_k_gemv_form(const er_k_gemv_form_args* args, void* stream);
int er_k_attn_stream_xt(const float* q_dev, const void* k_dev, const void* v_dev, const int32_t* len_host, float* out_dev,
                        void* out_xt_dev, int batch, int heads, int l_cap, int kv_half, void* stream);
int er_k_attn_outproj3(const float* q_dev, const void* k_dev, const void* v_dev, int len, const void* wo_dev,
                       const float* bo_dev, const float* resid_dev, float* y_dev, int l_cap, int kv_half, int w_half,
                       void* stream);
int er_k_gemm(const float* a_dev, const float* b_dev, const float* bias_dev, const float* resid_dev,
              float* c_dev, int m, int n, int k, int lda, int ldb, int ldc, int b_is_kn, int relu,
              float div, void* stream);
int er_k_gemm_f16(const float* a_dev, const void* w_half_dev, const float* bias_dev, const float* resid_dev,
                  float* c_dev, int m, int n, int k, int lda, int ldb, int ldc, int relu, void* stream);
int er_k_gemm_hh(const float* a_dev, const void* w_half_dev, const float* bias_dev, const float* resid_dev, float* c_dev,
                 void* c16_out_dev, int m, int n, int k, int lda, int ldb, int ldc, int relu, void* stream);
int er_k_gemm_hh_qkv(const float* a_dev, const void* w_half_dev, const float* bias_dev, void* qk16_out_dev, void* vt_out_dev, int m,
                     int n, int k, int rows_per_batch, int force_tile, void* stream);
int er_k_gemm_hh_geglu(const float* a_dev, const void* w_half_dev, const float* bias_dev, void* out16_dev, int m, int f, int k,
                       int force_tile, void* stream);
int er_k_gemm_f16s(const float* a, const void* w_half, const float* bias, const float* resid, float* c, int m, int n, int k,
                   int lda, int ldb, int ldc, int relu, void* stream);
int er_k_flash_attn_f16(const float* q_dev, const float* k_dev, const float* v_dev, float* o_dev, int batch,
                        int heads, int n_queries, int m_keys, void* stream);
int er_k_flash_attn_f32(const float* q, const float* k, const float* v, float* o, int batch, int heads, int n, int m,
                        int head_dim, int causal, void* stream);
int er_k_flash_attn_hh(const float* q_dev, const float* k_dev, const float* v_dev, float* o_dev, int batch, int heads, int n, int m,
                       void* stream);
int er_k_flash_attn_f16s(const float* q_dev, const float* k_dev, const float* v_dev, float* o_dev, int batch, int heads,
                         int n_queries, int m_keys, int causal, void* stream);
int er_k_layernorm(const float* x_dev, const float* w_dev, const float* b_dev, float* y_dev,
                   int rows, int cols, float eps, void* stream);
int er_k_softmax(float* s_dev, int rows, int cols, int ld, int causal, void* stream);
int er_k_score_rows(const float* logits_dev, const int32_t* labels_dev, int batch, int seq_len, int vocab, float* nll_out_dev,
                    int32_t* pred_out_dev, float* loss_out_dev, void* stream);
int er_k_dit_loss(const float* pred_dev, const float* x0_dev, const float* eps_dev, const int32_t* timesteps_host, int batch, int n,
                  int pred_type, float snr_gamma, float* mse_out_dev, float* loss_out_dev, void* stream);
int er_k_fps(const float* points_dev, int batch, int n_points, int n_samples, int32_t* idx_out_dev, void* stream);
int er_k_nn_dist2(const float* a_dev, const float* b_dev, int batch, int n_a, int n_b, float* d2_out_dev, int32_t* idx_out_dev,
                  void* stream);
int er_k_surface_sample(const float* vertices_dev, const int32_t* faces_dev, const int32_t* vert_offset_host,
                        const int32_t* face_offset_host, int batch, int n_samples, uint64_t seed, const uint32_t* stream_ids_host,
                        float* points_out_dev, int32_t* face_out_dev, void* stream);
int er_k_fidelity_metrics(const float* d2_ab_dev, const float* d2_ba_dev, int batch, int n_a, int n_b, float tau,
                          double* metrics_out_dev, void* stream);
int er_k_sample_head(const float* logits_dev, const er_decode_params* p, int vocab, int eos, int pad,
                     int batch, int step, const int32_t* last_tok_host, const int32_t* counter_host,
                     const int32_t* unfinished_host, int32_t* next_tok_host, int32_t* counter_out_host,
                     int32_t* unfinished_out_host, void* stream);

#ifdef __cplusplus
}
#endif
#endif
```

Baseline: 1074 tokens/s.

## Fuse decode MLP into one kernel that skips fc2 rows of ReLU-zero neurons

Adds a fused batch-1 decode MLP kernel that computes LayerNorm, fc1 with ReLU, and partial fc2 products in one launch, followed by a small finish kernel that reduces the partials and adds bias and residual. fc2 weights are pre-transposed to K-major so each workgroup reads contiguous rows for its own neurons. When a neuron's activation is zero, the load is redirected to a shared zero row, which cuts fc2 weight traffic by exploiting ReLU sparsity. It is on by default for the fp32 non-batched hidden-1536 path. The cost is an extra copy of w2 in memory and a partials buffer that must be reduced.

```diff
diff --git a/edgerunner_amd/csrc/er_api.hip b/edgerunner_amd/csrc/er_api.hip
--- a/edgerunner_amd/csrc/er_api.hip
+++ b/edgerunner_amd/csrc/er_api.hip
@@ -33,6 +33,7 @@
 #include "er_queue_host.h"
 #include "er_decode_plan.h"
 #include "er_decode_proj.h"
+#include "k_mlp_sparse.h"
 
 using namespace er;
 
@@ -61,6 +62,7 @@
 struct LayerW {
     _Float16 *wqkv_h = nullptr, *wo_h = nullptr, *w1_h = nullptr, *w2_h = nullptr;
     void *wqkv_t = nullptr, *wo_t = nullptr, *w1_t = nullptr, *w2_t = nullptr;
+    void* w2_kt = nullptr;
     float *wqkv = nullptr, *bqkv = nullptr;
     float *wo = nullptr, *bo = nullptr, *ln1w = nullptr, *ln1b = nullptr;
     float *w1 = nullptr, *b1 = nullptr, *w2 = nullptr, *b2 = nullptr, *ln2w = nullptr, *ln2b = nullptr;
@@ -100,6 +102,8 @@
     DevBuf<char> kc, vc;
     DevBuf<float> ypre, hbuf, ypre1, h1buf, qbuf, abuf, fbuf, logits;
     DevBuf<float> part, part_ml;
+    DevBuf<float> mlp_part;
+    DevBuf<int> mlp_nnz;
     DevBuf<float> skpart;
     DevBuf<char> xt_h, xt_att, xt_f;
     DevBuf<int> state_block;
@@ -135,6 +139,8 @@
     bool have_hidden = false;
     DecodeKnobs knobs;
     bool tiled_valid = false;
+    bool kmajor_valid = false;
+    void* zero_row = nullptr;
     int prof_len = 0;
     hipEvent_t ev0 = nullptr, ev1 = nullptr;
     float last_decode_ms = 0.f;
@@ -169,6 +175,8 @@
     const char* rw = getenv("ER_RW_FC2");
     k.rw_fc2 = rw ? atoi(rw) : 6;
     if (fast && k.rw_fc2 != 2 && k.rw_fc2 != 4 && k.rw_fc2 != 6) fprintf(stderr, "[edgerunner_hip] ER_RW_FC2=%s is not 2 / 4 / 6: using 2 rows per fc2 workgroup\n", rw);
+    k.mlp_v = env_int("ER_MLP_V", fast ? 0 : 1);
+    if (k.mlp_v != 1) k.mlp_v = 0;
     return k;
 }
 
@@ -292,7 +300,7 @@
     if (!c || !key) return fail(ER_ERR_INVALID, "er_load_tensor: bad argument");
     HIPCHK(hipSetDevice(c->device));
     const int rc = weights_load(c->w, c->own_stream, "er_load_tensor", key, data, dtype, ndim, shape, on_device);
-    if (rc != 1) c->tiled_valid = false;
+    if (rc != 1) c->tiled_valid = c->kmajor_valid = false;
     return rc;
 }
 
@@ -331,6 +339,27 @@
     }
     HIPCHK(hipStreamSynchronize(c->own_stream));
     c->tiled_valid = true;
+    return 0;
+}
+
+static int make_kmajor_weights(er_ctx* c) {
+    if (c->kmajor_valid || weights_missing(c->w)) return 0;
+    const size_t H = c->cfg.hidden_dim, I = c->cfg.intermediate_dim, esz = c->fast ? 2 : 4;
+    if (!c->zero_row) {
+        char* z = nullptr;
+        ERCHK(weights_alloc(c->w, &z, H * 4));
+        c->zero_row = z;
+    }
+    for (LayerW& L : c->layers) {
+        if (!L.w2_kt) {
+            char* blk = nullptr;
+            ERCHK(c->w.alloc(&blk, I * H * esz));
+            L.w2_kt = blk;
+        }
+        HIPCHK(c->fast ? launch_transpose_w2<_Float16>(L.w2_h, L.w2_kt, c->own_stream) : launch_transpose_w2<float>(L.w2, L.w2_kt, c->own_stream));
+    }
+    HIPCHK(hipStreamSynchronize(c->own_stream));
+    c->kmajor_valid = true;
     return 0;
 }
 
@@ -411,6 +440,12 @@
     m.st.row_budget = m.d_row_budget.p;
     ERCHK(m.d_out_ids.ensure(b * (size_t)Lcap));
     if (p.mfma) ERCHK(make_tiled_weights(c));
+    if (p.mlp_fused) {
+        ERCHK(make_kmajor_weights(c));
+        ERCHK(m.mlp_part.ensure((size_t)MLP_WGS * hid));
+        ERCHK(m.mlp_nnz.ensure((size_t)g.num_layers * MLP_WGS));
+        HIPCHK(hipMemset(m.mlp_nnz.p, 0, m.mlp_nnz.n * sizeof(int)));
+    }
     const size_t groups = (b + NBM - 1) / NBM;
     ERCHK(m.skpart.ensure(p.xt ? groups * SK_SLICES_FC2 * NBM * (size_t)hid : (size_t)SK_SLICES_OUTPROJ * NBM * (size_t)std::max(hid, g.vocab_size)));
     if (p.xt) {
@@ -453,6 +488,17 @@
 }
 static hipError_t launch_attn_combine(const AttnDecArgs& a, int D, int B, hipStream_t st) {
     return D == 96 ? launch_attn_combine_d<96>(a, B, st) : launch_attn_combine_d<64>(a, B, st);
+}
+
+static MlpArgs mlp_args(er_ctx* c, int layer) {
+    const LayerW& L = c->layers[layer];
+    const KvMem& kv = *c->kv;
+    MlpArgs m{};
+    m.W1 = c->fast ? (const void*)L.w1_h : (const void*)L.w1; m.b1 = L.b1; m.W2T = L.w2_kt; m.zero_row = c->zero_row;
+    m.xin = kv.ypre1.p; m.ln_w = L.ln1w; m.ln_b = L.ln1b; m.eps = c->cfg.ln_eps; m.hout = kv.h1buf.p;
+    m.part = kv.mlp_part.p; m.nnz = kv.mlp_nnz.p + (size_t)layer * MLP_WGS;
+    m.b2 = L.b2; m.resid = kv.h1buf.p; m.out = kv.ypre.p;
+    return m;
 }
 
 template <typename WT>
@@ -506,6 +552,10 @@
         }
         case 4: {
             const LayerW& L = c->layers[layer];
+            if (p.mlp_fused) {
+                if (!c->kmajor_valid) return hipErrorInvalidValue;
+                return launch_mlp_fused<WT>(mlp_args(c, layer), st);
+            }
             a.W = HALF ? (const void*)L.w1_h : (const void*)L.w1; a.bias = L.b1; a.N = I; a.xin = kv.ypre1.p; a.ln_w = L.ln1w; a.ln_b = L.ln1b;
             a.hout = kv.h1buf.p; a.out = kv.fbuf.p;
             io.pro = PRO_LN;
@@ -515,6 +565,7 @@
         }
         case 5: {
             const LayerW& L = c->layers[layer];
+            if (p.mlp_fused) return launch_mlp_finish(mlp_args(c, layer), st);
             a.W = HALF ? (const void*)L.w2_h : (const void*)L.w2; a.bias = L.b2; a.N = H; a.xin = kv.fbuf.p; a.out = kv.ypre.p; a.resid = kv.h1buf.p;
             io.w_tiled = L.w2_t; io.x_image = kv.xt_f.p;
             return run_proj<WT>(PROJ_FC2, form_of(PROJ_FC2, layer), io, a, B, I, sk, st);
@@ -801,6 +852,7 @@
     HIPCHK(hipSetDevice(c->device));
     const DecodePlan& p = c->kv->plan;
     if (p.mfma) ERCHK(make_tiled_weights(c));
+    if (p.mlp_fused) ERCHK(make_kmajor_weights(c));
     const er_config& g = c->cfg;
     const int H = g.hidden_dim, I = g.intermediate_dim, NH = g.num_heads, D = c->D;
     const int M = B * S;
@@ -1120,6 +1172,7 @@
     HIPCHK(hipSetDevice(c->device));
     hipStream_t st = pick(c, stream);
     if (c->kv->plan.mfma) ERCHK(make_tiled_weights(c));
+    if (c->kv->plan.mlp_fused) ERCHK(make_kmajor_weights(c));
     ERCHK(c->q_look.ensure((size_t)3 * B + 1));
     if (c->q_pinned) { hipHostFree(c->q_pinned); c->q_pinned = nullptr; }
     HIPCHK(hipHostMalloc((void**)&c->q_pinned, ((size_t)3 * B + 1) * sizeof(int), hipHostMallocDefault));
@@ -1344,6 +1397,15 @@
         if (gexec) hipGraphExecDestroy(gexec);
     }
     HIPCHK(hipStreamSynchronize(st));
+    if (p.mlp_fused) {
+        std::vector<int> nnz((size_t)nl * MLP_WGS);
+        HIPCHK(hipMemcpy(nnz.data(), c->kv->mlp_nnz.p, nnz.size() * sizeof(int), hipMemcpyDeviceToHost));
+        double live = 0.0;
+        for (int n : nnz) live += n;
+        const double part = (double)MLP_WGS * H * 4.0;
+        bytes[4] = ((double)I * H + live / nl * H) * w + ((double)I + 4 * H) * 4.0 + part;
+        bytes[5] = part + (double)3 * H * 4.0;
+    }
     HIPCHK(hipMemcpy(c->kv->ypre.p, save_y.data(), save_y.size() * 4, hipMemcpyHostToDevice));
     HIPCHK(hipMemcpy(c->kv->state_block.p, save_state.data(), save_state.size() * sizeof(int), hipMemcpyHostToDevice));
     return ER_OK;
@@ -1538,6 +1600,36 @@
     return f->w_half ? gemv_form_t<_Float16>(*f, proj, (hipStream_t)stream) : gemv_form_t<float>(*f, proj, (hipStream_t)stream);
 }
 
+extern "C" int er_k_mlp_transpose(const void* w2, void* w2t, int w_half, void* stream) {
+    if (!w2 || !w2t) return fail(ER_ERR_INVALID, "er_k_mlp_transpose: null argument");
+    hipStream_t st = (hipStream_t)stream;
+    HIPRET(w_half ? launch_transpose_w2<_Float16>(w2, w2t, st) : launch_transpose_w2<float>(w2, w2t, st));
+    return ER_OK;
+}
+
+extern "C" int er_k_mlp_sparse(const er_k_mlp_sparse_args* f, void* stream) {
+    if (!f) return fail(ER_ERR_INVALID, "er_k_mlp_sparse: null args");
+    if (!f->w1 || !f->b1 || !f->w2t || !f->zero_row || !f->b2 || !f->x || !f->ln_w || !f->ln_b || !f->h1_out || !f->y || !f->part)
+        return fail(ER_ERR_INVALID, "er_k_mlp_sparse: null operand");
+    hipStream_t st = (hipStream_t)stream;
+    MlpArgs m{};
+    m.W1 = f->w1; m.b1 = f->b1; m.W2T = f->w2t; m.zero_row = f->zero_row; m.xin = f->x; m.ln_w = f->ln_w; m.ln_b = f->ln_b; m.eps = f->eps;
+    m.hout = f->h1_out; m.part = f->part; m.nnz = f->nnz; m.b2 = f->b2; m.resid = f->h1_out; m.out = f->y;
+    HIPRET(f->w_half ? launch_mlp_fused<_Float16>(m, st) : launch_mlp_fused<float>(m, st));
+    HIPRET(launch_mlp_finish(m, st));
+    return ER_OK;
+}
+
+extern "C" int er_mlp_nnz(er_ctx* c, int32_t* out, int n) {
+    if (!c || !out) return fail(ER_ERR_INVALID, "er_mlp_nnz: null argument");
+    if (!c->kv->plan.mlp_fused) return fail(ER_ERR_INVALID, "er_mlp_nnz: the reserved shape does not run the fused MLP");
+    if (n != (int)c->kv->mlp_nnz.n) return fail(ER_ERR_INVALID, "er_mlp_nnz: %d counts asked, the context holds %zu (layers * 256)", n, c->kv->mlp_nnz.n);
+    HIPCHK(hipSetDevice(c->device));
+    HIPCHK(hipDeviceSynchronize());
+    HIPCHK(hipMemcpy(out, c->kv->mlp_nnz.p, (size_t)n * sizeof(int), hipMemcpyDeviceToHost));
+    return ER_OK;
+}
+
 extern "C" int er_k_attn_outproj3(const float* q, const void* k, const void* v, int len, const void* wo, const float* bo,
                                   const float* resid, float* y, int l_cap, int kv_half, int w_half, void* stream) {
     constexpr int H = 16, D = 96;
diff --git a/edgerunner_amd/csrc/er_decode_plan.h b/edgerunner_amd/csrc/er_decode_plan.h
--- a/edgerunner_amd/csrc/er_decode_plan.h
+++ b/edgerunner_amd/csrc/er_decode_plan.h
@@ -10,6 +10,7 @@
     int attn_v_batched = 0;
     int decode_v = 3;
     int rw_fc2 = 6;
+    int mlp_v = 0;
 };
 
 struct ReserveKnobs { bool force_batched, batched_valu, xt; };
@@ -32,6 +33,7 @@
     bool xt = false;
     bool stream_attn = false;
     bool v3 = false;
+    bool mlp_fused = false;
     bool outproj_rows8 = false;
     bool outproj_partials = false;
     bool fc2_defers(int layer) const { return xt && layer >= 0 && layer + 1 < layers; }
@@ -61,6 +63,7 @@
     plan_decode(k.decode_v, k.attn_v_batched, p.force_batched, batch, H, D, hid, Lcap, ch, &p.sel);
     p.batched = p.sel.batched != 0; p.mfma = p.batched && !p.valu; p.xt = fast && p.mfma && rk.xt;
     p.stream_attn = p.sel.attn_kernel == ER_ATTN_STREAM; p.v3 = p.sel.decode_version == 3;
+    p.mlp_fused = k.mlp_v != 0 && batch == 1 && !p.batched && hid == 1536;
     p.outproj_rows8 = p.mfma && batch >= 5 && batch <= 8;
     p.outproj_partials = p.xt && p.stream_attn && batch > 8;
     return p;
diff --git a/edgerunner_amd/csrc/er_mlp_map.h b/edgerunner_amd/csrc/er_mlp_map.h
--- /dev/null
+++ b/edgerunner_amd/csrc/er_mlp_map.h
@@ -0,0 +1,20 @@
+#pragma once
+
+namespace er {
+
+constexpr int MLP_HIDDEN = 1536, MLP_INTER = 6144;
+constexpr int MLP_SLICES = MLP_INTER / MLP_HIDDEN;
+constexpr int MLP_WGS = MLP_SLICES * 64;
+constexpr int MLP_CHAIN = MLP_INTER / MLP_WGS;
+
+struct MlpSlot { int wg, i; };
+
+constexpr int mlp_neuron(int epl, int wg, int i) {
+    return (wg >> 6) * MLP_HIDDEN + ((i / epl) * 64 + (wg & 63)) * epl + i % epl;
+}
+constexpr MlpSlot mlp_slot(int epl, int k) {
+    const int s = k / MLP_HIDDEN, q = (k % MLP_HIDDEN) / epl, e = k % epl;
+    return MlpSlot{s * 64 + q % 64, (q / 64) * epl + e};
+}
+
+}
diff --git a/edgerunner_amd/csrc/k_mlp_sparse.h b/edgerunner_amd/csrc/k_mlp_sparse.h
--- /dev/null
+++ b/edgerunner_amd/csrc/k_mlp_sparse.h
@@ -0,0 +1,204 @@
+#pragma once
+#include "er_common.h"
+#include "er_mlp_map.h"
+#include "k_gemv.h"
+
+namespace er {
+
+struct MlpArgs {
+    const void* W1;
+    const float* b1;
+    const void* W2T;
+    const void* zero_row;
+    const float* xin;
+    const float* ln_w;
+    const float* ln_b;
+    float eps;
+    float* hout;
+    float* part;
+    int* nnz;
+    const float* b2;
+    const float* resid;
+    float* out;
+};
+
+template <typename WT>
+__global__ __launch_bounds__(ER_WG) void transpose_w2_kernel(const WT* __restrict__ src, WT* __restrict__ dst, int N, int K) {
+    __shared__ WT tile[64][65];
+    const int k0 = blockIdx.x * 64, n0 = blockIdx.y * 64, tx = threadIdx.x & 63, ty = threadIdx.x >> 6;
+    for (int r = ty; r < 64; r += 4) tile[r][tx] = src[(long long)(n0 + r) * K + k0 + tx];
+    __syncthreads();
+    for (int r = ty; r < 64; r += 4) dst[(long long)(k0 + r) * N + n0 + tx] = tile[tx][r];
+}
+
+template <typename WT>
+inline hipError_t launch_transpose_w2(const void* w2, void* w2t, hipStream_t st) {
+    hipLaunchKernelGGL((transpose_w2_kernel<WT>), dim3(MLP_INTER / 64, MLP_HIDDEN / 64), dim3(ER_WG), 0, st, reinterpret_cast<const WT*>(w2),
+                       reinterpret_cast<WT*>(w2t), MLP_HIDDEN, MLP_INTER);
+    return hipGetLastError();
+}
+
+typedef _Float16 f16x4 __attribute__((ext_vector_type(4)));
+template <typename WT> struct MlpCol;
+template <> struct MlpCol<float> { typedef f32x4 V; };
+template <> struct MlpCol<_Float16> { typedef f16x4 V; };
+
+constexpr int MLP_NW = 12, MLP_TPB = 64 * MLP_NW;
+constexpr int MLP_COLS = MLP_HIDDEN / 4;
+
+template <typename WT>
+__global__ __launch_bounds__(MLP_TPB) void mlp_sparse_kernel(const void* pW1, const float* pxin, const float* pln_w, const float* pln_b,
+                                                             const float* pb1, MlpArgs a_) {
+    MlpArgs a = a_;
+    a.W1 = pW1; a.xin = pxin; a.ln_w = pln_w; a.ln_b = pln_b; a.b1 = pb1;
+    constexpr int EPL = WTraits<WT>::EPL, XV = EPL / 4, K = MLP_HIDDEN, J = K / (64 * EPL), RW = 2;
+    constexpr int PW = 4, PTPB = 64 * PW, PT = K / PTPB;
+    static_assert(MLP_NW * RW == MLP_CHAIN && J * EPL == MLP_CHAIN, "one workgroup = one lane chain of fc2");
+    typedef typename MlpCol<WT>::V ColV;
+    __shared__ __attribute__((aligned(16))) float xs[K];
+    __shared__ float red[64];
+    __shared__ __attribute__((aligned(16))) float fs[MLP_CHAIN];
+    const int tid = threadIdx.x, lane = tid & 63, wid = tid >> 6, wg = blockIdx.x;
+    const bool pro = wid < PW;
+
+    float v[PT], lw[PT], lb[PT];
+    if (pro) {
+#pragma unroll
+        for (int i = 0; i < PT; ++i) v[i] = a.xin[tid + i * PTPB];
+#pragma unroll
+        for (int i = 0; i < PT; ++i) { lw[i] = a.ln_w[tid + i * PTPB]; lb[i] = a.ln_b[tid + i * PTPB]; }
+    }
+    int krow[RW];
+    float bias[RW];
+#pragma unroll
+    for (int r = 0; r < RW; ++r) {
+        krow[r] = mlp_neuron(EPL, wg, wid * RW + r);
+        bias[r] = a.b1[krow[r]];
+    }
+    f32x4 w[RW][J];
+#pragma unroll
+    for (int r = 0; r < RW; ++r) {
+        const f32x4* wr = reinterpret_cast<const f32x4*>(reinterpret_cast<const WT*>(a.W1) + (long long)krow[r] * K);
+#pragma unroll
+        for (int j = 0; j < J; ++j) w[r][j] = __builtin_nontemporal_load(wr + j * 64 + lane);
+    }
+    __builtin_amdgcn_sched_barrier(0);
+
+    {
+        float s[1], s2[1];
+        s[0] = 0.f;
+#pragma unroll
+        for (int i = 0; i < PT; ++i) s[0] += pro ? v[i] : 0.f;
+        block_sum_slots<PW, 1>(s, red, 8, pro);
+        const float mean = s[0] / (float)K;
+        s2[0] = 0.f;
+#pragma unroll
+        for (int i = 0; i < PT; ++i) { const float d = (pro ? v[i] : 0.f) - mean; s2[0] = fmaf(d, d, s2[0]); }
+        block_sum_slots<PW, 1>(s2, red + 4, 8, pro);
+        if (pro) {
+            const float rstd = 1.0f / sqrtf(s2[0] / (float)K + a.eps);
+#pragma unroll
+            for (int i = 0; i < PT; ++i) v[i] = (v[i] - mean) * rstd * lw[i] + lb[i];
+#pragma unroll
+            for (int i = 0; i < PT; ++i) xs[tid + i * PTPB] = v[i];
+            if (a.hout != nullptr && wg == 0) {
+#pragma unroll
+                for (int i = 0; i < PT; ++i) a.hout[tid + i * PTPB] = v[i];
+            }
+        }
+    }
+    __syncthreads();
+
+    {
+        f32x4 xr[J * XV];
+#pragma unroll
+        for (int j = 0; j < J; ++j)
+#pragma unroll
+            for (int u = 0; u < XV; ++u) xr[j * XV + u] = reinterpret_cast<const f32x4*>(xs)[(j * 64 + lane) * XV + u];
+#pragma unroll
+        for (int r = 0; r < RW; ++r) {
+            float s = 0.f;
+#pragma unroll
+            for (int j = 0; j < J; ++j) s = dot_w<WT>(w[r][j], &xr[j * XV], s);
+            float f = wave_sum(s);
+            f += bias[r];
+            f = fmaxf(f, 0.0f);
+            if (lane == 0) fs[wid * RW + r] = f;
+        }
+    }
+    __syncthreads();
+
+    constexpr int NCH = MLP_CHAIN;
+    if (wid >= MLP_NW / 2) return;
+    const int col = tid;
+    float f[NCH];
+    ColV wv[NCH];
+#pragma unroll
+    for (int u = 0; u < NCH; u += 4) {
+        const f32x4 t = reinterpret_cast<const f32x4*>(fs)[u / 4];
+        f[u] = t.x; f[u + 1] = t.y; f[u + 2] = t.z; f[u + 3] = t.w;
+    }
+#pragma unroll
+    for (int u = 0; u < NCH; ++u) {
+        f[u] = __uint_as_float(__builtin_amdgcn_readfirstlane(__float_as_uint(f[u])));
+        const char* row = f[u] != 0.f ? reinterpret_cast<const char*>(a.W2T) + (long long)mlp_neuron(EPL, wg, u) * K * (long long)sizeof(WT)
+                                      : reinterpret_cast<const char*>(a.zero_row);
+        wv[u] = __builtin_nontemporal_load(reinterpret_cast<const ColV*>(row) + col);
+    }
+    __builtin_amdgcn_sched_barrier(0);
+    if (tid == 0 && a.nnz != nullptr) {
+        int c = 0;
+#pragma unroll
+        for (int i = 0; i < MLP_CHAIN; ++i) c += fs[i] != 0.f ? 1 : 0;
+        a.nnz[wg] = c;
+    }
+    f32x4 s = {0.f, 0.f, 0.f, 0.f};
+#pragma unroll
+    for (int u = 0; u < NCH; ++u) {
+        s.x = fmaf((float)wv[u].x, f[u], s.x);
+        s.y = fmaf((float)wv[u].y, f[u], s.y);
+        s.z = fmaf((float)wv[u].z, f[u], s.z);
+        s.w = fmaf((float)wv[u].w, f[u], s.w);
+    }
+    reinterpret_cast<f32x4*>(a.part + (long long)wg * K)[col] = s;
+}
+
+constexpr int MLP_FIN_NC = 8;
+__global__ __launch_bounds__(ER_WG) void mlp_finish_kernel(MlpArgs a) {
+    constexpr int NC = MLP_FIN_NC;
+    static_assert(MLP_HIDDEN % NC == 0 && NC % 4 == 0 && MLP_SLICES == ER_NWAVES, "finish shape");
+    __shared__ float red[NC * MLP_SLICES];
+    const int tid = threadIdx.x, lane = tid & 63, wid = tid >> 6, n0 = blockIdx.x * NC;
+    float bias = 0.f, resid = 0.f;
+    if (tid < NC) { bias = a.b2[n0 + tid]; resid = a.resid[n0 + tid]; }
+    const f32x4* p = reinterpret_cast<const f32x4*>(a.part + (long long)(wid * 64 + lane) * MLP_HIDDEN + n0);
+    f32x4 pv[NC / 4];
+#pragma unroll
+    for (int c = 0; c < NC / 4; ++c) pv[c] = p[c];
+#pragma unroll
+    for (int c = 0; c < NC; ++c) {
+        const float t = wave_sum(pv[c / 4][c % 4]);
+        if (lane == 0) red[c * MLP_SLICES + wid] = t;
+    }
+    __syncthreads();
+    if (tid < NC) {
+        float s = 0.f;
+#pragma unroll
+        for (int k = 0; k < MLP_SLICES; ++k) s += red[tid * MLP_SLICES + k];
+        s += bias;
+        s += resid;
+        a.out[n0 + tid] = s;
+    }
+}
+
+template <typename WT>
+inline hipError_t launch_mlp_fused(const MlpArgs& a, hipStream_t st) {
+    hipLaunchKernelGGL((mlp_sparse_kernel<WT>), dim3(MLP_WGS), dim3(MLP_TPB), 0, st, a.W1, a.xin, a.ln_w, a.ln_b, a.b1, a);
+    return hipGetLastError();
+}
+inline hipError_t launch_mlp_finish(const MlpArgs& a, hipStream_t st) {
+    hipLaunchKernelGGL(mlp_finish_kernel, dim3(MLP_HIDDEN / MLP_FIN_NC), dim3(ER_WG), 0, st, a);
+    return hipGetLastError();
+}
+
+}
diff --git a/edgerunner_amd/kernels.py b/edgerunner_amd/kernels.py
--- a/edgerunner_amd/kernels.py
+++ b/edgerunner_amd/kernels.py
@@ -125,6 +125,33 @@
     return out
 
 
+def mlp_transpose(w2):
+    assert w2.shape == (1536, 6144) and w2.dtype in (torch.float32, torch.float16)
+    w2t = torch.empty((6144, 1536), dtype=w2.dtype, device=w2.device)
+    native.check(native.load_library().er_k_mlp_transpose(native.ptr(w2), native.ptr(w2t), int(w2.dtype == torch.float16), _st()), "er_k_mlp_transpose")
+    return w2t
+
+
+class MlpSparse:
+
+    def __init__(self, w1, b1, w2t, b2, x, ln_w, ln_b, eps=1e-5):
+        dev = x.device
+        assert w1.shape == (6144, 1536) and w2t.shape == (6144, 1536) and w1.dtype == w2t.dtype and x.numel() == 1536
+        self.keep = [w1, b1, w2t, b2, x, ln_w, ln_b]
+        self.zero_row = torch.zeros(1536, dtype=torch.float32, device=dev)
+        self.h1 = torch.empty(1536, dtype=torch.float32, device=dev)
+        self.y = torch.empty(1536, dtype=torch.float32, device=dev)
+        self.part = torch.empty((256, 1536), dtype=torch.float32, device=dev)
+        self.nnz = torch.zeros(256, dtype=torch.int32, device=dev)
+        a = self.args = native.ErKMlpSparseArgs()
+        a.w1, a.b1, a.w2t, a.zero_row, a.b2, a.x, a.ln_w, a.ln_b, a.h1_out, a.y, a.part, a.nnz = (
+            native.ptr(t).value for t in (w1, b1, w2t, self.zero_row, b2, x, ln_w, ln_b, self.h1, self.y, self.part, self.nnz))
+        a.w_half, a.eps = int(w1.dtype == torch.float16), eps
+
+    def launch(self):
+        native.check(native.load_library().er_k_mlp_sparse(C.byref(self.args), _st()), "er_k_mlp_sparse")
+
+
 def attn_stream_xt(q, k_cache, v_cache, lens, out_xt):
     lib = native.load_library()
     B, H, Lcap, D = k_cache.shape
diff --git a/edgerunner_amd/native.py b/edgerunner_amd/native.py
--- a/edgerunner_amd/native.py
+++ b/edgerunner_amd/native.py
@@ -23,7 +23,7 @@
     "er_dit_finalize_weights", "er_dit_project_cond", "er_dit_encode_image", "er_dit_forward", "er_dit_sample",
     "er_dit_set_prediction_type", "er_dit_attach_point_encoder", "er_dit_point_latent", "er_dit_set_point_encoder_mode", "er_dit_loss", "er_k_dit_loss",
     "er_set_row_streams", "er_plan_decode", "er_ctx_plan", "er_plan_gemm_tile", "er_kernel_kind_name", "er_profile_decode_kernels", "er_profile_decode_kernels_at", "er_last_decode_ms",
-    "er_k_gemv", "er_k_gemv_form", "er_k_attn_decode", "er_k_attn_stream_xt", "er_k_attn_outproj3", "er_k_gemm", "er_k_gemm_f16", "er_k_gemm_hh", "er_k_gemm_hh_qkv", "er_k_gemm_hh_geglu", "er_k_gemm_f16s", "er_k_flash_attn_f16", "er_k_flash_attn_hh", "er_k_flash_attn_f32", "er_k_flash_attn_f16s", "er_k_layernorm", "er_k_softmax", "er_k_score_rows", "er_k_fps", "er_k_sample_head",
+    "er_k_gemv", "er_k_gemv_form", "er_k_mlp_transpose", "er_k_mlp_sparse", "er_mlp_nnz", "er_k_attn_decode", "er_k_attn_stream_xt", "er_k_attn_outproj3", "er_k_gemm", "er_k_gemm_f16", "er_k_gemm_hh", "er_k_gemm_hh_qkv", "er_k_gemm_hh_geglu", "er_k_gemm_f16s", "er_k_flash_attn_f16", "er_k_flash_attn_hh", "er_k_flash_attn_f32", "er_k_flash_attn_f16s", "er_k_layernorm", "er_k_softmax", "er_k_score_rows", "er_k_fps", "er_k_sample_head",
     "er_k_nn_dist2", "er_k_surface_sample", "er_k_fidelity_metrics",
     "er_queue_begin", "er_queue_admit", "er_queue_run", "er_queue_take", "er_queue_stats", "er_queue_end",
 ]
@@ -48,6 +48,11 @@
         "q_out", "kcache", "vcache", "prep_xt_out", "xt_out", "part_out")] + [(n, C.c_int32) for n in (
         "w_half", "kv_half", "batch", "n", "k", "prologue", "epilogue", "form", "nw", "rw", "sk_slices", "heads", "head_dim",
         "l_cap")] + [("eps", C.c_float)]
+
+
+class ErKMlpSparseArgs(C.Structure):
+    _fields_ = [(n, C.c_void_p) for n in ("w1", "b1", "w2t", "zero_row", "b2", "x", "ln_w", "ln_b", "h1_out", "y", "part", "nnz")] + \
+               [("w_half", C.c_int32), ("eps", C.c_float)]
 
 
 class ErConfig(C.Structure):
@@ -146,6 +151,9 @@
     lib.er_queue_end.argtypes = [vp]
     lib.er_k_gemv.argtypes = [vp, vp, vp, vp, vp, vp, vp, vp, ci, ci, ci, ci, cf, vp]
     lib.er_k_gemv_form.argtypes = [C.POINTER(ErKGemvFormArgs), vp]
+    lib.er_k_mlp_transpose.argtypes = [vp, vp, ci, vp]
+    lib.er_k_mlp_sparse.argtypes = [C.POINTER(ErKMlpSparseArgs), vp]
+    lib.er_mlp_nnz.argtypes = [vp, C.POINTER(C.c_int32), ci]
     lib.er_k_attn_stream_xt.argtypes = [vp, vp, vp, C.POINTER(C.c_int32), vp, vp, ci, ci, ci, ci, vp]
     lib.er_k_attn_decode.argtypes = [vp, vp, vp, C.POINTER(C.c_int32), vp, ci, ci, ci, ci, ci, ci, ci, vp]
     lib.er_k_attn_outproj3.argtypes = [vp, vp, vp, ci, vp, vp, vp, vp, ci, ci, ci, vp]
diff --git a/edgerunner_amd/shape_opt.py b/edgerunner_amd/shape_opt.py
--- a/edgerunner_amd/shape_opt.py
+++ b/edgerunner_amd/shape_opt.py
@@ -339,6 +339,13 @@
         native.check(self.lib.er_ctx_plan(self._ctx, C.byref(p)), "er_ctx_plan")
         return {n: int(getattr(p, n)) for n, _ in native.ErDecodePlan._fields_}
 
+    def mlp_nnz(self):
+        import numpy as np
+        n = int(self.dims.num_layers) * 256
+        buf = np.empty((n,), dtype=np.int32)
+        native.check(self.lib.er_mlp_nnz(self._ctx, buf.ctypes.data_as(C.POINTER(C.c_int32)), n), "er_mlp_nnz")
+        return buf.reshape(-1, 256)
+
     def profile_decode_kernels(self, repeats: int = 5, context_len: int = 0, use_graph: bool = False):
         us = (C.c_float * native.ER_NUM_KERNEL_KINDS)()
         by = (C.c_double * native.ER_NUM_KERNEL_KINDS)()
diff --git a/include/edgerunner_hip.h b/include/edgerunner_hip.h
--- a/include/edgerunner_hip.h
+++ b/include/edgerunner_hip.h
@@ -213,6 +213,25 @@
     float eps;
 } er_k_gemv_form_args;
 int er_k_gemv_form(const er_k_gemv_form_args* args, void* stream);
+int er_k_mlp_transpose(const void* w2_dev, void* w2t_dev, int w_half, void* stream);
+typedef struct er_k_mlp_sparse_args {
+    const void* w1;
+    const float* b1;
+    const void* w2t;
+    const void* zero_row;
+    const float* b2;
+    const float* x;
+    const float* ln_w;
+    const float* ln_b;
+    float* h1_out;
+    float* y;
+    float* part;
+    int32_t* nnz;
+    int32_t w_half;
+    float eps;
+} er_k_mlp_sparse_args;
+int er_k_mlp_sparse(const er_k_mlp_sparse_args* args, void* stream);
+int er_mlp_nnz(er_ctx* ctx, int32_t* out, int n);
 int er_k_attn_stream_xt(const float* q_dev, const void* k_dev, const void* v_dev, const int32_t* len_host, float* out_dev,
                         void* out_xt_dev, int batch, int heads, int l_cap, int kv_half, void* stream);
 int er_k_attn_outproj3(const float* q_dev, const void* k_dev, const void* v_dev, int len, const void* wo_dev,
```

Result: faster. 1097 tokens/s, median of 6 (+2.1%).
